# jweyn/DLWP-CS

Measured on AMD Instinct MI355X. Metric: cubed-sphere samples/sec (fwd+bwd), higher is better.
Workload: dtype bf16; 1 GPU; unet2 C48: x (32,6,48,48,14) per GPU, 14 out channels, base 32, MSE + Adam, fwd+bwd+update, bf16 activations + bf16 MFMA, fp32 master weights / gradients / Adam; global_batch=32, parallelism=dp1, hip_graphs=True

## Files before the change

### dlwp-cs_amd/DLWP/_native.py

```python
import ctypes
import os
import threading

import numpy as np
import torch

_HERE = os.path.dirname(os.path.abspath(__file__))
_TAG = os.environ.get('DLWPCS_LIB_TAG', '')
LIB_PATH = os.path.join(os.path.dirname(_HERE), 'lib', 'libdlwpcs%s.so' % ('_' + _TAG if _TAG else ''))

F32 = 0
BF16 = 1
I16 = 2
MAP_RENORMALIZE = 1
MSE_TARGET_F32 = 0x100
MSE_OVERWRITE = 0x200
ADAM_ZERO_GRAD = 1
HEAD_DEFER_STAGE2 = 2
LOSS_MSE, LOSS_MAE, LOSS_ACC = 0, 1, 2
REG_NONE, REG_MSE, REG_MAE, REG_GLOBAL = 0, 1, 2, 3
NORM_ALL, NORM_VALID = 0, 1
E_UNSUPPORTED = -2
ACT_NONE = 0
ACT_LEAKY_CLIP = 1
CONV_ACCUMULATE_WGRAD = 1
CONV_PREPACKED = 2
CONV_REUSE_DZ = 4
CONV_DEFER_REDUCE = 8
CONV_DEFER_RING0 = 16
CONV_OUT_PADDED = 32
CONV_DGRAD_GATHER = 64
CONSTRAINT_MAX_NORM, CONSTRAINT_NON_NEG, CONSTRAINT_UNIT_NORM, CONSTRAINT_MIN_MAX_NORM = 1, 2, 3, 4
PACK_FWD, PACK_BWD, PACK_BIAS = 0, 1, 2
WGRAD_BATCH_MAX = 24

c_void_p, c_int, c_float, c_size_t = ctypes.c_void_p, ctypes.c_int, ctypes.c_float, ctypes.c_size_t
c_i32p = ctypes.POINTER(ctypes.c_int32)


class ConvDesc(ctypes.Structure):
    _fields_ = [('B', ctypes.c_int32), ('N', ctypes.c_int32), ('C0', ctypes.c_int32), ('C1', ctypes.c_int32),
                ('Cout', ctypes.c_int32), ('ksize', ctypes.c_int32), ('halo', ctypes.c_int32),
                ('up0', ctypes.c_int32), ('flip_north_pole', ctypes.c_int32), ('act', ctypes.c_int32),
                ('alpha', ctypes.c_float), ('vmax', ctypes.c_float), ('dtype', ctypes.c_int32),
                ('flags', ctypes.c_int32), ('c0_valid', ctypes.c_int32)]


class PackItem(ctypes.Structure):
    _fields_ = [(n, ctypes.c_void_p) for n in ('w_eq', 'w_pol', 'w_np', 'b_eq', 'b_pol', 'b_np', 'wpk_fwd', 'wpk_bwd',
                                                'bias_pk')] + \
               [(n, ctypes.c_int32) for n in ('ksize', 'Cin', 'Cout', 'flip_north_pole', 'dtype', 'reserved')]


class ReduceItem(ctypes.Structure):
    _fields_ = [(n, ctypes.c_void_p) for n in ('partial', 'bpartial', 'dw_eq', 'dw_pol', 'dw_np', 'db_eq', 'db_pol',
                                                'db_np')] + \
               [(n, ctypes.c_int32) for n in ('ksize', 'Cin', 'Cout', 'CinP', 'CoutP', 'n_eq', 'n_4', 'n_5',
                                              'flip_north_pole', 'accumulate', 'vec', 'nblocks')] + \
               [('reserved', ctypes.c_int32 * 4)]


class WgradItem(ctypes.Structure):
    _fields_ = [('d', ConvDesc)] + [(n, ctypes.c_void_p) for n in ('src0', 'src1', 'dz', 'y', 'table_dev', 'dw_eq', 'dw_pol',
                                                                    'dw_np', 'db_eq', 'db_pol', 'db_np')]


class LossTail(ctypes.Structure):
    _fields_ = [('partial', ctypes.c_void_p), ('loss_out', ctypes.c_void_p), ('nblocks', ctypes.c_int32), ('inv_n', ctypes.c_float),
                ('weight', ctypes.c_float), ('overwrite', ctypes.c_int32)]


class LossDesc(ctypes.Structure):
    _fields_ = [('kind', ctypes.c_int32), ('loss_weight', ctypes.c_float), ('weight', ctypes.c_void_p),
                ('weight_div', ctypes.c_int32), ('weight_period', ctypes.c_int32), ('clim', ctypes.c_void_p),
                ('clim_div', ctypes.c_int32), ('clim_period', ctypes.c_int32), ('regularize', ctypes.c_int32),
                ('reverse', ctypes.c_int32), ('overwrite', ctypes.c_int32)]


class GConvDesc(ctypes.Structure):
    _fields_ = [(n, ctypes.c_int32) for n in
                ('B', 'H', 'W', 'Cin', 'Cout', 'kh', 'kw', 'sh', 'sw', 'dh', 'dw', 'pad_t', 'pad_l', 'Ho', 'Wo',
                 'flip_north_pole', 'dtype')]


SCORE_MSE, SCORE_RMSE, SCORE_MAE, SCORE_ACC, SCORE_COS, SCORE_MEAN = 0, 1, 2, 3, 4, 5
SCORE_MAX_DIMS = 8


class ScoreDesc(ctypes.Structure):
    _fields_ = [(n, ctypes.c_int32) for n in ('method', 'n_lead', 't_len', 't_cap', 't_slope', 'n_keep', 'n_red', 'kc')] + \
               [('keep_ext', ctypes.c_int64 * SCORE_MAX_DIMS), ('red_ext', ctypes.c_int64 * SCORE_MAX_DIMS),
                ('lead_stride', ctypes.c_int64 * 4), ('t_stride', ctypes.c_int64 * 4), ('kc_stride', ctypes.c_int64 * 4),
                ('keep_stride', (ctypes.c_int64 * SCORE_MAX_DIMS) * 4), ('red_stride', (ctypes.c_int64 * SCORE_MAX_DIMS) * 4)]


class OverlapDesc(ctypes.Structure):
    _fields_ = [('N', ctypes.c_int32), ('n_lat', ctypes.c_int32), ('n_lon', ctypes.c_int32), ('reserved', ctypes.c_int32),
                ('frames', ((ctypes.c_double * 3) * 3) * 6), ('dust', ctypes.c_double)]


class CubeBilinearDesc(ctypes.Structure):
    _fields_ = [('N', ctypes.c_int32), ('reserved', ctypes.c_int32), ('n_points', ctypes.c_int64),
                ('frames', ((ctypes.c_double * 3) * 3) * 6), ('edge', ((ctypes.c_int32 * 3) * 4) * 6)]


class SparseMapDesc(ctypes.Structure):
    _fields_ = [('n_a', ctypes.c_int64), ('n_b', ctypes.c_int64), ('nnz', ctypes.c_int64), ('x_dtype', ctypes.c_int32),
                ('n_outer', ctypes.c_int32), ('outer_ext', ctypes.c_int64 * 3), ('x_outer_stride', ctypes.c_int64 * 3),
                ('y_outer_stride', ctypes.c_int64 * 3), ('x_space_stride', ctypes.c_int64), ('y_space_stride', ctypes.c_int64),
                ('inner_ext', ctypes.c_int64), ('x_inner_stride', ctypes.c_int64), ('y_inner_stride', ctypes.c_int64)]


GROUP_SLAB_ROWS = 512


class RowsDesc(ctypes.Structure):
    _fields_ = [('n_inner', ctypes.c_int32), ('reserved', ctypes.c_int32), ('src_row_stride', ctypes.c_int64),
                ('out_row_stride', ctypes.c_int64), ('inner_ext', ctypes.c_int64 * SCORE_MAX_DIMS),
                ('src_stride', ctypes.c_int64 * SCORE_MAX_DIMS), ('out_stride', ctypes.c_int64 * SCORE_MAX_DIMS)]


class ZonalSpectrumDesc(ctypes.Structure):
    _fields_ = [(n, ctypes.c_int32) for n in ('L', 'n_wave', 'n_dims', 'remove_mean')] + \
               [('ext', ctypes.c_int64 * SCORE_MAX_DIMS), ('kept', ctypes.c_int32 * SCORE_MAX_DIMS),
                ('stride', (ctypes.c_int64 * SCORE_MAX_DIMS) * 3)]


class ShtSpectrumDesc(ctypes.Structure):
    _fields_ = [(n, ctypes.c_int32) for n in ('nlat', 'L', 'T', 'n_dims')] + \
               [('lat_stride', ctypes.c_int64 * 2), ('ext', ctypes.c_int64 * SCORE_MAX_DIMS),
                ('stride', (ctypes.c_int64 * SCORE_MAX_DIMS) * 2)]


class ShtSynthesisDesc(ctypes.Structure):
    _fields_ = [(n, ctypes.c_int32) for n in ('nlat', 'L', 'T', 'n_dims')] + \
               [('lat_stride', ctypes.c_int64), ('ext', ctypes.c_int64 * SCORE_MAX_DIMS), ('stride', ctypes.c_int64 * SCORE_MAX_DIMS)]


SHT_MAX_NLAT = 8192
ENSEMBLE_MAX_M = 128


class EnsembleDesc(ctypes.Structure):
    _fields_ = [(n, ctypes.c_int32) for n in ('M', 'n_dims', 'fair', 'ddof', 'variance', 'reserved')] + \
               [('member_stride', ctypes.c_int64), ('ext', ctypes.c_int64 * SCORE_MAX_DIMS),
                ('stride', (ctypes.c_int64 * SCORE_MAX_DIMS) * 2)]


QUANTILE_MAX_PROBS = 16
TIME_FILTER_MAX_TAPS = 4096
REGRESSION_MAX_TERMS = 16
REGRESSION_SLAB_ROWS = 512
TIME_SPECTRUM_MAX_M = 1728
TIME_SPECTRUM_SLAB_SEGMENTS = 8
ROW_GRAM_SLAB_COLS = 512
ROW_GRAM_GROUP_SLABS = 16
TIME_LAG_MAX_LAGS = 1024
TIME_LAG_SLAB_ROWS = 512
LAG_AUTO, LAG_PAIR, LAG_INDEX = 0, 1, 2
RESAMPLE_STAGED_ROWS = 1280
RESAMPLE_MAX_ROWS = 2147483647
RESAMPLE_CHOOSE, RESAMPLE_STAGED, RESAMPLE_DIRECT = -1, 0, 1
CATEGORY_MAX_M = 1024
CATEGORY_MAX_Q = 16


class CategoryDesc(ctypes.Structure):
    _fields_ = [(n, ctypes.c_int32) for n in ('M', 'Q', 'n_dims', 'fair')] + \
               [('member_stride', ctypes.c_int64), ('thr_stride', ctypes.c_int64), ('ext', ctypes.c_int64 * SCORE_MAX_DIMS),
                ('stride', (ctypes.c_int64 * SCORE_MAX_DIMS) * 3), ('ref_prob', ctypes.c_float * CATEGORY_MAX_Q)]


AFFINE_MUL_ADD, AFFINE_SUB_DIV = 0, 1
AFFINE_MAX_CHANNELS = 1024


class ChanDesc(ctypes.Structure):
    _fields_ = [(n, ctypes.c_int64) for n in ('R', 'C', 'S', 'row_stride', 'chan_stride', 'inner_stride', 'dst_row_stride',
                                              'dst_chan_stride', 'dst_inner_stride')]


PROTOTYPES = {
    'dlwpcs_version': (c_int, []),
    'dlwpcs_last_error': (ctypes.c_char_p, []),
    'dlwpcs_halo_table': (c_int, [c_int, c_int, c_void_p]),
    'dlwpcs_halo_inverse_table': (c_int, [c_int, c_int, c_void_p]),
    'dlwpcs_dgrad_gather_plan_ints': (c_size_t, [c_int]),
    'dlwpcs_dgrad_gather_plan': (c_int, [c_int, c_void_p]),
    'dlwpcs_pad_fwd': (c_int, [c_void_p, c_void_p, c_int, c_int, c_int, c_int, c_int, c_void_p, c_void_p]),
    'dlwpcs_pad_bwd': (c_int, [c_void_p, c_void_p, c_int, c_int, c_int, c_int, c_int, c_void_p, c_void_p]),
    'dlwpcs_conv_workspace_bytes': (c_size_t, [ctypes.POINTER(ConvDesc)]),
    'dlwpcs_conv_packed_bytes': (c_size_t, [ctypes.POINTER(ConvDesc), c_int]),
    'dlwpcs_pack_batch': (c_int, [c_void_p, c_int, c_void_p]),
    'dlwpcs_conv_fwd': (c_int, [ctypes.POINTER(ConvDesc)] + [c_void_p] * 8 + [c_void_p, c_void_p, c_void_p, c_size_t,
                                                                                 c_void_p]),
    'dlwpcs_conv_fwd_pool': (c_int, [ctypes.POINTER(ConvDesc)] + [c_void_p] * 8 + [c_void_p, c_void_p, c_void_p, c_void_p, c_size_t,
                                                                                      c_void_p]),
    'dlwpcs_conv_fwd_head': (c_int, [ctypes.POINTER(ConvDesc)] + [c_void_p] * 4 + [ctypes.POINTER(ConvDesc)] + [c_void_p] * 6 +
                             [c_size_t, ctypes.POINTER(c_int), c_void_p]),
    'dlwpcs_conv_bwd_data': (c_int, [ctypes.POINTER(ConvDesc)] + [c_void_p] * 5 + [c_void_p, c_void_p, c_void_p,
                                                                                      c_void_p, c_size_t, c_void_p]),
    'dlwpcs_conv_bwd_data_masked': (c_int, [ctypes.POINTER(ConvDesc)] + [c_void_p] * 4 + [c_void_p] * 4 + [c_float, c_float] +
                                    [c_void_p, c_void_p, c_size_t, c_void_p]),
    'dlwpcs_conv_small_fwd': (c_int, [ctypes.POINTER(ConvDesc)] + [c_void_p] * 8 + [c_void_p, c_void_p, c_void_p, c_size_t,
                                                                                       c_void_p]),
    'dlwpcs_conv_small_bwd_data': (c_int, [ctypes.POINTER(ConvDesc)] + [c_void_p] * 4 + [c_void_p] * 4 + [c_float, c_float] +
                                   [c_void_p, c_void_p, c_size_t, c_void_p]),
    'dlwpcs_conv_bwd_weights': (c_int, [ctypes.POINTER(ConvDesc)] + [c_void_p] * 4 + [c_void_p] * 6 +
                                [c_void_p, c_void_p, c_size_t, c_void_p]),
    'dlwpcs_conv_wgrad_reduce_item': (c_int, [ctypes.POINTER(ConvDesc)] + [c_void_p] * 6 +
                                      [c_void_p, c_size_t, ctypes.POINTER(ReduceItem)]),
    'dlwpcs_wgrad_reduce_batch': (c_int, [c_void_p, c_void_p, c_int, c_void_p]),
    'dlwpcs_wgrad_batch_supported': (c_int, [ctypes.POINTER(ConvDesc)]),
    'dlwpcs_wgrad_batch_sizes': (c_int, [c_void_p, c_int, ctypes.POINTER(c_size_t), ctypes.POINTER(c_size_t)]),
    'dlwpcs_wgrad_batch_plan': (c_int, [c_void_p, c_int, c_void_p, c_size_t]),
    'dlwpcs_wgrad_batch': (c_int, [c_void_p, c_int, c_void_p, c_void_p, c_void_p, c_size_t, c_void_p]),
    'dlwpcs_wgrad_batch_adam': (c_int, [c_void_p, c_int, c_void_p, c_void_p, c_void_p, c_size_t, c_void_p, c_void_p, c_void_p,
                                        c_void_p, c_size_t, c_void_p, c_void_p, c_void_p]),
    'dlwpcs_wgrad_batch_adam_tail': (c_int, [c_void_p, c_int, c_void_p, c_void_p, c_void_p, c_size_t, c_void_p, c_void_p, c_void_p,
                                             c_void_p, c_size_t, c_void_p, c_void_p, c_void_p, c_void_p, c_void_p]),
    'dlwpcs_wgrad_batch_apply': (c_int, [c_void_p, c_int, c_void_p, c_void_p, c_void_p, c_void_p, c_void_p, c_void_p, c_size_t,
                                         c_void_p, c_void_p, c_void_p, c_void_p, c_void_p]),
    'dlwpcs_gconv_fwd': (c_int, [ctypes.POINTER(GConvDesc)] + [c_void_p] * 9),
    'dlwpcs_gconv_bwd_data': (c_int, [ctypes.POINTER(GConvDesc)] + [c_void_p] * 6),
    'dlwpcs_gconv_bwd_weights': (c_int, [ctypes.POINTER(GConvDesc)] + [c_void_p] * 9),
    'dlwpcs_act_fwd': (c_int, [c_void_p, c_void_p, c_size_t, c_int, c_float, c_float, c_int, c_void_p]),
    'dlwpcs_act_bwd': (c_int, [c_void_p, c_void_p, c_void_p, c_size_t, c_int, c_float, c_float, c_int, c_void_p]),
    'dlwpcs_avgpool2_fwd': (c_int, [c_void_p, c_void_p, c_int, c_int, c_int, c_int, c_void_p]),
    'dlwpcs_avgpool2_bwd': (c_int, [c_void_p, c_void_p, c_int, c_int, c_int, c_int, c_void_p]),
    'dlwpcs_avgpool2_bwd_add': (c_int, [c_void_p, c_void_p, c_void_p, c_int, c_int, c_int, c_int, c_void_p]),
    'dlwpcs_avgpool2_bwd_masked': (c_int, [c_void_p, c_void_p, c_void_p, c_void_p, c_int, c_int, c_int, c_float, c_float, c_int,
                                           c_void_p]),
    'dlwpcs_avgpool2_bwd_ring': (c_int, [c_void_p, c_void_p, c_void_p, c_void_p, c_int, c_int, c_int, c_float, c_float, c_int,
                                         c_void_p, c_void_p, c_int, c_int, c_void_p]),
    'dlwpcs_conv_ring_info': (c_int, [ctypes.POINTER(ConvDesc), ctypes.POINTER(c_size_t), ctypes.POINTER(c_int)]),
    'dlwpcs_upsample2_fwd': (c_int, [c_void_p, c_void_p, c_int, c_int, c_int, c_int, c_void_p]),
    'dlwpcs_upsample2_bwd': (c_int, [c_void_p, c_void_p, c_int, c_int, c_int, c_int, c_void_p]),
    'dlwpcs_concat2': (c_int, [c_void_p, c_void_p, c_void_p, c_size_t, c_int, c_int, c_int, c_void_p]),
    'dlwpcs_split2': (c_int, [c_void_p, c_void_p, c_void_p, c_size_t, c_int, c_int, c_int, c_void_p]),
    'dlwpcs_cf_to_cl': (c_int, [c_void_p, c_void_p, c_int, c_int, c_size_t, c_int, c_void_p]),
    'dlwpcs_cl_to_cf': (c_int, [c_void_p, c_void_p, c_int, c_int, c_size_t, c_int, c_void_p]),
    'dlwpcs_add': (c_int, [c_void_p, c_void_p, c_void_p, c_size_t, c_int, c_void_p]),
    'dlwpcs_l1l2_regularize': (c_int, [c_void_p, c_void_p, c_size_t, c_float, c_float, c_float, c_void_p, c_void_p]),
    'dlwpcs_weight_constraint': (c_int, [c_void_p, c_int, c_int, c_int, c_float, c_float, c_float, c_void_p]),
    'dlwpcs_mse_scratch_bytes': (c_size_t, []),
    'dlwpcs_mse_fwd_bwd': (c_int, [c_void_p, c_void_p, c_void_p, c_void_p, c_size_t, c_float, c_int, c_void_p,
                                   c_void_p]),
    'dlwpcs_loss_scratch_bytes': (c_size_t, []),
    'dlwpcs_loss_fwd_bwd': (c_int, [c_void_p, c_void_p, c_void_p, c_void_p, c_void_p, c_size_t, c_int, c_void_p, c_void_p]),
    'dlwpcs_loss_masked_fwd_bwd': (c_int, [c_void_p, c_void_p, c_void_p, c_int, c_void_p, c_void_p, c_void_p, c_size_t, c_int,
                                           c_void_p, c_void_p]),
    'dlwpcs_head_loss_step': (c_int, [c_void_p, c_void_p, c_void_p, c_void_p, c_void_p, c_void_p, c_void_p, c_void_p, c_void_p,
                                      c_void_p, c_void_p, c_int, c_float, c_float, c_void_p]),
    'dlwpcs_score_scratch_bytes': (c_size_t, [c_void_p]),
    'dlwpcs_score': (c_int, [c_void_p, c_void_p, c_void_p, c_void_p, c_void_p, c_void_p, c_int, c_void_p, c_size_t, c_void_p]),
    'dlwpcs_score_indexed': (c_int, [c_void_p, c_void_p, c_void_p, c_void_p, c_void_p, c_void_p, ctypes.c_int64, c_void_p, c_int,
                                     c_void_p, c_size_t, c_void_p]),
    'dlwpcs_score_plan_info': (c_int, [c_void_p, c_void_p, c_void_p, c_void_p, c_void_p, c_int, ctypes.c_int64, c_void_p]),
    'dlwpcs_group_mean_scratch_bytes': (c_size_t, [c_void_p, c_int, ctypes.c_int64, c_int]),
    'dlwpcs_group_mean': (c_int, [c_void_p, c_void_p, c_void_p, c_void_p, c_int, ctypes.c_int64, c_int, c_void_p, c_void_p,
                                  c_void_p, c_size_t, c_void_p]),
    'dlwpcs_rows_gather': (c_int, [c_void_p, c_void_p, c_void_p, ctypes.c_int64, c_void_p, c_void_p]),
    'dlwpcs_group_quantile': (c_int, [c_void_p, c_void_p, c_void_p, c_void_p, c_int, ctypes.c_int64, c_void_p, c_int, c_void_p,
                                      ctypes.c_int64, c_void_p, c_void_p]),
    'dlwpcs_group_quantile_plan_info': (c_int, [c_void_p, c_void_p, c_int, ctypes.c_int64, c_int, c_void_p]),
    'dlwpcs_time_filter': (c_int, [c_void_p, c_void_p, ctypes.c_int64, c_void_p, c_int, ctypes.c_int64, ctypes.c_int64, ctypes.c_int64,
                                   c_int, c_float, c_int, ctypes.c_int64, c_void_p, c_void_p, c_void_p]),
    'dlwpcs_time_filter_plan_info': (c_int, [c_void_p, c_void_p, c_void_p, ctypes.c_int64, c_int, ctypes.c_int64, ctypes.c_int64, c_int,
                                             c_int, ctypes.c_int64, c_void_p]),
    'dlwpcs_time_regression_scratch_bytes': (c_size_t, [c_void_p, ctypes.c_int64, c_int, ctypes.c_int64, c_int]),
    'dlwpcs_time_regression': (c_int, [c_void_p, c_void_p, ctypes.c_int64, c_void_p, c_int, c_int, ctypes.c_int64, ctypes.c_double,
                                       ctypes.c_int64, c_int, c_int, c_void_p, ctypes.c_int64, c_void_p, c_void_p, c_size_t, c_void_p]),
    'dlwpcs_time_regression_plan_info': (c_int, [c_void_p, c_void_p, c_void_p, ctypes.c_int64, c_int, c_int, ctypes.c_int64,
                                                 ctypes.c_int64, c_int, c_int, ctypes.c_int64, c_void_p]),
    'dlwpcs_time_regression_apply': (c_int, [c_void_p, c_void_p, ctypes.c_int64, c_void_p, c_int, c_void_p, ctypes.c_int64, c_void_p,
                                             c_int, c_void_p, c_void_p]),
    'dlwpcs_time_spectrum_scratch_bytes': (c_size_t, [c_void_p, ctypes.c_int64, c_int, ctypes.c_int64, c_int, c_int, c_int]),
    'dlwpcs_time_spectrum': (c_int, [c_void_p, c_void_p, c_void_p, ctypes.c_int64, c_int, ctypes.c_int64, c_void_p, c_void_p,
                                     ctypes.c_double, c_int, c_int, c_int, c_int, c_int, ctypes.c_int64, ctypes.c_int64, c_void_p,
                                     c_void_p, c_void_p, c_size_t, c_void_p]),
    'dlwpcs_time_spectrum_plan_info': (c_int, [c_void_p, c_void_p, c_void_p, ctypes.c_int64, c_int, ctypes.c_int64, c_int, c_int,
                                               c_int, c_void_p]),
    'dlwpcs_row_gram_scratch_bytes': (c_size_t, [c_void_p, ctypes.c_int64, c_void_p, ctypes.c_int64, c_int]),
    'dlwpcs_row_gram': (c_int, [c_void_p, c_void_p, ctypes.c_int64, c_void_p, c_void_p, ctypes.c_int64, c_void_p, c_int, c_void_p,
                                c_int, c_void_p, c_int, c_void_p, ctypes.c_int64, c_void_p, c_void_p, c_void_p, c_size_t, c_void_p]),
    'dlwpcs_row_gram_plan_info': (c_int, [c_void_p, c_void_p, ctypes.c_int64, c_void_p, c_void_p, ctypes.c_int64, c_int, c_void_p]),
    'dlwpcs_time_lag_scratch_bytes': (c_size_t, [c_void_p, c_int, ctypes.c_int64, ctypes.c_int64, c_int, c_int, c_int]),
    'dlwpcs_time_lag': (c_int, [c_void_p, c_void_p, c_void_p, c_int, ctypes.c_int64, ctypes.c_int64, ctypes.c_int64, c_int, c_void_p,
                                c_void_p, c_void_p, c_int, c_int, c_int, c_int, c_void_p, c_void_p, c_void_p, c_size_t, c_void_p]),
    'dlwpcs_time_lag_plan_info': (c_int, [c_void_p, c_void_p, c_void_p, c_int, ctypes.c_int64, ctypes.c_int64, c_int, c_int, c_int,
# ... 220 lines not shown
```

### dlwp-cs_amd/DLWP/custom.py

```python


import numpy as np

from . import ops
from ._native import ACT_LEAKY_CLIP, ACT_NONE
from .keras import constraints, engine, regularizers
from .keras.callbacks import Callback, EarlyStopping
from .keras.engine import Layer
from .keras.losses import LossSpec, mean_absolute_error, mean_squared_error, spec_of



def _normalize_tuple(value, n, name):
    if isinstance(value, int):
        return (value,) * n
    try:
        value_tuple = tuple(value)
    except TypeError:
        raise ValueError('The `' + name + '` argument must be a tuple of ' + str(n) + ' integers. Received: ' +
                         str(value))
    if len(value_tuple) != n:
        raise ValueError('The `' + name + '` argument must be a tuple of ' + str(n) + ' integers. Received: ' +
                         str(value))
    for single_value in value_tuple:
# ... 97 lines not shown
                 independent_north_pole=False,
                 kernel_initializer='glorot_uniform',
                 bias_initializer='zeros',
                 kernel_regularizer=None,
                 bias_regularizer=None,
                 activity_regularizer=None,
                 kernel_constraint=None,
                 bias_constraint=None,
                 **kwargs):
        super(CubeSphereConv2D, self).__init__(**kwargs)
        self.filters = filters
        self.kernel_size = _normalize_tuple(kernel_size, 2, 'kernel_size')
        self.strides = _normalize_tuple(strides, 2, 'strides')
        self.padding = _normalize_padding(padding)
        self.data_format = _normalize_data_format(data_format)
        self.dilation_rate = _normalize_tuple(dilation_rate, 2, 'dilation_rate')
        self.activation = engine.get_activation(activation)
        self.use_bias = use_bias
        self.flip_north_pole = flip_north_pole
        self.independent_north_pole = independent_north_pole
        self.kernel_initializer = engine.get_initializer(kernel_initializer)
        self.bias_initializer = engine.get_initializer(bias_initializer)
        self.kernel_regularizer = regularizers.get(kernel_regularizer)
        self.bias_regularizer = regularizers.get(bias_regularizer)
        self.activity_regularizer = engine._passthrough_get(activity_regularizer)
        self.kernel_constraint = constraints.get(kernel_constraint)
        self.bias_constraint = constraints.get(bias_constraint)
        self.rank = 3

        self.equatorial_kernel = None
        self.equatorial_bias = None
        self.polar_kernel = None
        self.polar_bias = None
        self.north_pole_kernel = None
        self.north_pole_bias = None

    def _weight_attr_names(self):
        return ['equatorial_kernel', 'polar_kernel', 'north_pole_kernel', 'equatorial_bias', 'polar_bias',
                'north_pole_bias']

    def build(self, input_shape):
        if self.data_format == 'channels_first':
            channel_axis = 1
        else:
            channel_axis = -1
        if input_shape[channel_axis] is None:
            raise ValueError('The channel dimension of the inputs should be defined. Found `None`.')
        input_dim = int(input_shape[channel_axis])
        kernel_shape = self.kernel_size + (input_dim, self.filters)

        self.equatorial_kernel = self.add_weight(shape=kernel_shape, initializer=self.kernel_initializer,
                                                 name='equatorial_kernel', regularizer=self.kernel_regularizer,
                                                 constraint=self.kernel_constraint)
        self.polar_kernel = self.add_weight(shape=kernel_shape, initializer=self.kernel_initializer,
                                            name='polar_kernel', regularizer=self.kernel_regularizer,
                                            constraint=self.kernel_constraint)
        if self.independent_north_pole:
            self.north_pole_kernel = self.add_weight(shape=kernel_shape, initializer=self.kernel_initializer,
                                                     name='north_pole_kernel', regularizer=self.kernel_regularizer,
                                                     constraint=self.kernel_constraint)
        if self.use_bias:
            self.equatorial_bias = self.add_weight(shape=(self.filters,), initializer=self.bias_initializer,
                                                   name='equatorial_bias', regularizer=self.bias_regularizer,
                                                   constraint=self.bias_constraint)
            self.polar_bias = self.add_weight(shape=(self.filters,), initializer=self.bias_initializer,
                                              name='polar_bias', regularizer=self.bias_regularizer,
                                              constraint=self.bias_constraint)
            if self.independent_north_pole:
                self.north_pole_bias = self.add_weight(shape=(self.filters,), initializer=self.bias_initializer,
                                                       name='north_pole_bias', regularizer=self.bias_regularizer,
                                                       constraint=self.bias_constraint)
        self.input_dim = input_dim
        self.built = True

    def _is_mfma_config(self):
        k = self.kernel_size
        return (k[0] == k[1] and k[0] in (1, 3) and self.strides == (1, 1) and self.dilation_rate == (1, 1)
                and self.padding == 'valid')

    def can_fuse_halo(self, pad_width):
        return (self._is_mfma_config() and self.kernel_size[0] == 3 and pad_width == 1 and self.activation is None)

    def fused_call(self, src0, src1=None, up0=False, halo=True, act=ACT_NONE, alpha=0.0, vmax=0.0, premask0=None,
                   premask1=None, dy_premasked=False, defer_ring0=False, want_pool=False, out_padded=False, small=False):
        return ops.cs_conv(src0, self.equatorial_kernel, self.polar_kernel, self.north_pole_kernel,
                           self.equatorial_bias, self.polar_bias, self.north_pole_bias, src1=src1,
                           ksize=self.kernel_size[0], halo=halo, up0=up0, flip_north_pole=self.flip_north_pole,
                           act=act, alpha=alpha, vmax=vmax, premask0=premask0, premask1=premask1,
                           dy_premasked=dy_premasked, defer_ring0=defer_ring0, want_pool=want_pool, out_padded=out_padded,
                           small=small)

    def call(self, inputs, channels_last_io=False, **kwargs):
        channels_first = self.data_format == 'channels_first' and not channels_last_io
        x = ops.channels_first_to_last(inputs) if channels_first else inputs
        if self._is_mfma_config():
            outputs = ops.cs_conv(x, self.equatorial_kernel, self.polar_kernel, self.north_pole_kernel,
                                  self.equatorial_bias, self.polar_bias, self.north_pole_bias,
                                  ksize=self.kernel_size[0], halo=False, flip_north_pole=self.flip_north_pole)
        else:
            outputs = ops.cs_gconv(x, self.equatorial_kernel, self.polar_kernel, self.north_pole_kernel,
                                   self.equatorial_bias, self.polar_bias, self.north_pole_bias,
                                   strides=self.strides, padding=self.padding, dilation=self.dilation_rate,
                                   flip_north_pole=self.flip_north_pole)
        if channels_first:
            outputs = ops.channels_last_to_first(outputs)
        if self.activation is not None:
            return self.activation(outputs)
        return outputs

    def compute_output_shape(self, input_shape):
        if self.data_format == 'channels_last':
            space = input_shape[2:4]
        else:
            space = input_shape[-2:]
        new_space = []
        for i in range(len(space)):
            new_space.append(_conv_output_length(space[i], self.kernel_size[i], padding=self.padding,
                                                 stride=self.strides[i], dilation=self.dilation_rate[i]))
        if self.data_format == 'channels_last':
            return (input_shape[0], 6) + tuple(new_space) + (self.filters,)
        return (input_shape[0], self.filters, 6) + tuple(new_space)

    def get_config(self):
        config = {
            'filters': self.filters,
            'kernel_size': self.kernel_size,
            'strides': self.strides,
            'padding': self.padding,
            'data_format': self.data_format,
            'dilation_rate': self.dilation_rate,
            'activation': engine.serialize_activation(self.activation),
            'use_bias': self.use_bias,
            'flip_north_pole': self.flip_north_pole,
            'independent_north_pole': self.independent_north_pole,
            'kernel_initializer': engine.serialize_initializer(self.kernel_initializer),
            'bias_initializer': engine.serialize_initializer(self.bias_initializer),
            'kernel_regularizer': regularizers.serialize(self.kernel_regularizer),
            'bias_regularizer': regularizers.serialize(self.bias_regularizer),
            'activity_regularizer': self.activity_regularizer,
            'kernel_constraint': constraints.serialize(self.kernel_constraint),
            'bias_constraint': constraints.serialize(self.bias_constraint)
        }
        base_config = super(CubeSphereConv2D, self).get_config()
        return dict(list(base_config.items()) + list(config.items()))



def _adam_effective_lr(optimizer, beta_1, beta_2, with_bias_correction):
    it = float(optimizer.iterations)
    lr = float(optimizer.lr) / (1. + float(getattr(optimizer, 'decay', 0.)) * it)
    if with_bias_correction:
        t = it + 1.
        lr = lr * np.sqrt(1. - np.power(beta_2, t)) / (1. - np.power(beta_1, t))
    return lr


class AdamLearningRateTracker(Callback):

    def on_epoch_end(self, epoch, logs=None, beta_1=0.9, beta_2=0.999, ):
        print(' - LR: {:.6f}'.format(_adam_effective_lr(self.model.optimizer, beta_1, beta_2, True)))


class SGDLearningRateTracker(Callback):

    def on_epoch_end(self, epoch, logs=None):
        print(' - LR: {:.6f}'.format(_adam_effective_lr(self.model.optimizer, 0., 0., False)))


class BatchHistory(Callback):

    def on_train_begin(self, logs=None):
        self.history, self.epoch = [], 0

# ... 239 lines not shown
```

### dlwp-cs_amd/DLWP/keras/models.py

```python
import gc
import json
import os
import sys
import time

import numpy as np
import torch

from .. import ops, parallel
from ..options import option
from .. import _native as _nat
from .._native import ACT_LEAKY_CLIP, ACT_NONE
from . import backend, callbacks as cbks, losses as klosses, optimizers, staging
from .engine import KTensor, Layer
from .layers import AveragePooling3D, Concatenate, InputLayer, ReLU, UpSampling3D


def _new_graph():
    if os.environ.get('DLWPCS_KEEP_GRAPH', '0') == '1':
        return torch.cuda.CUDAGraph(keep_graph=True)
    return torch.cuda.CUDAGraph()


def _as_list(x):
    if isinstance(x, (list, tuple)):
        return list(x)
    return [x]


class Model(object):
    def __init__(self, inputs=None, outputs=None, name=None):
        if inputs is None or outputs is None:
            raise ValueError('Model needs `inputs` and `outputs`')
        self._single_input = not isinstance(inputs, (list, tuple))
        self.inputs = _as_list(inputs)
        self.outputs = _as_list(outputs)
        self._single_output = len(self.outputs) == 1
        for t in self.inputs + self.outputs:
            if not isinstance(t, KTensor):
                raise ValueError('Model inputs/outputs must be symbolic tensors created by Input() and layer calls')
        self.name = name or 'model'
        self.stop_training = False
        self.optimizer = None
        self.loss = None
        self._dev_losses = None
        self.loss_weights = None
        self.metrics = []
        self.history = None
        self.use_graphs = option('graphs')
        self.compute_dtype = backend.compute_dtype()
        self.prepack_weights = True
        self.wgrad_side_stream = False
        self.defer_wgrad_reduce = True
        self.batch_wgrad = option('wgrad_batch')
        self.check_finite = option('check_finite')
        self.fuse_adam = option('fuse_adam')
        self.fold_ring = option('fold_ring')
        self.fuse_pool = option('fuse_pool')
        self.fold_loss_tail = option('fold_loss_tail')
        self.fuse_pack = option('fuse_pack')
        self._packed_ok = False
        self.exchange_buckets = int(os.environ.get('DLWPCS_EXCHANGE_BUCKETS', '1'))
        self._stager = None
        self.fuse_head_loss = option('fuse_head')
        self.fold_head = option('fold_head')
        self.small_conv = option('small_conv')
        self.static_batch_buffers = False
        self._ones = {}
        self._compiled = False
        self._flat_params = self._flat_grads = None
        self._grads_clean = False
        self._graphs = {}
        self._infer_graphs = {}
        self._rollout_series = {}
        self.rollout_keep_bytes = 4 << 30
        self._seen_batch = {}
        self._toposort()
        self._build_plan()

    def _toposort(self):
        order, seen = [], set()

        def visit(t):
            if t.uid in seen:
                return
            seen.add(t.uid)
            for i in t.node_inputs:
                visit(i)
            order.append(t)
        for o in self.outputs:
            visit(o)
        input_uids = {t.uid for t in self.inputs}
        for t in order:
            if isinstance(t.layer, InputLayer) and t.uid not in input_uids:
                raise ValueError('Graph disconnected: cannot obtain value for tensor %r' % (t,))
        self._nodes = order
        layers, seen_l = [], set()
        for t in self.inputs + order:
            if t.layer is not None and id(t.layer) not in seen_l:
                seen_l.add(id(t.layer))
                layers.append(t.layer)
        self.layers = layers

    def _build_plan(self):
        consumers = {}
        for t in self._nodes:
            for i in t.node_inputs:
                consumers.setdefault(i.uid, []).append(t)
        out_uids = {o.uid for o in self.outputs}

        def sole_consumer(t):
            c = consumers.get(t.uid, [])
            return c[0] if (len(c) == 1 and t.uid not in out_uids) else None

        from ..custom import CubeSphereConv2D, CubeSpherePadding2D
        def cf_layer(t):
            lay = t.layer
            if isinstance(lay, InputLayer):
                return len(t.shape) == 5
            if isinstance(lay, CubeSphereConv2D) and lay.activation is not None \
                    and getattr(lay.activation, '_dlwp_name', None) != 'relu':
                return False
            if isinstance(lay, (CubeSpherePadding2D, CubeSphereConv2D, AveragePooling3D, UpSampling3D)):
                return lay.data_format == 'channels_first'
            if isinstance(lay, Concatenate):
                return lay._axis(len(t.shape)) == 1
            return isinstance(lay, ReLU)
        self._cf_model = (option('cf_model') and all(cf_layer(t) for t in self._nodes)
                          and any(isinstance(t.layer, (CubeSphereConv2D, CubeSpherePadding2D)) for t in self._nodes))
        fmt = 'channels_first' if self._cf_model else 'channels_last'
        virtual = set()
        fused = {}
        for t in self._nodes:
            lay = t.layer
            if not isinstance(lay, CubeSphereConv2D) or len(t.node_inputs) != 1:
                continue
            padt = t.node_inputs[0]
            if not isinstance(padt.layer, CubeSpherePadding2D) or sole_consumer(padt) is not t:
                continue
            if padt.layer.data_format != fmt or lay.data_format != fmt or not lay.can_fuse_halo(padt.layer.padding[1][0]):
                continue
            if padt.layer.padding[1] != padt.layer.padding[2] or padt.layer.padding[1][0] != padt.layer.padding[1][1]:
                continue
            x = padt.node_inputs[0]
            src0, src1, up0 = x, None, False
            chain = [padt]
            if isinstance(x.layer, Concatenate) and len(x.node_inputs) == 2 and sole_consumer(x) is padt \
                    and x.layer._axis(len(x.shape)) == (1 if self._cf_model else len(x.shape) - 1):
                src0, src1 = x.node_inputs
# ... 28 lines not shown
                              isinstance(t.layer, Concatenate)))
        self._plan = steps
        self.n_fused = len(fused)
        self._padded_io_ok = False
        if len(self.inputs) == 1:
            u = self.inputs[0].uid
            rd = [st for st in steps
                  if (st[0] == 'fused_conv' and u in (st[3], st[4])) or (st[0] == 'pool_skip' and st[3] == u)
                  or (st[0] == 'layer' and u in st[3])]
            self._padded_io_ok = (len(rd) == 1 and rd[0][0] == 'fused_conv' and rd[0][3] == u and rd[0][4] is None
                                  and not rd[0][5] and u not in out_uids and not self._cf_model)
        self._plan_premask(steps, out_uids)
        self._head_fold = {}
        for i, st in enumerate(steps):
            if st[0] != 'fused_conv' or st[1] in out_uids:
                continue
            rd = [j for j, s2 in enumerate(steps)
                  if (s2[0] == 'fused_conv' and st[1] in (s2[3], s2[4])) or (s2[0] == 'pool_skip' and s2[3] == st[1])
                  or (s2[0] == 'layer' and st[1] in s2[3])]
            if len(rd) != 1 or steps[rd[0]][0] != 'layer':
                continue
            hl = steps[rd[0]][2]
            if (isinstance(hl, CubeSphereConv2D) and len(steps[rd[0]][3]) == 1 and tuple(hl.kernel_size) == (1, 1)
                    and hl.activation is None and not hl.independent_north_pole and not st[2].independent_north_pole
                    and st[2].filters == 32 and self._runs_channels_last(hl) and not self._cf_model):
                self._head_fold[i] = rd[0]
        uids = [o.uid for o in self.outputs]
        self._sole_outputs = {u for u in uids if not consumers.get(u) and uids.count(u) == 1}

    def _plan_premask(self, steps, out_uids):
        from ..custom import CubeSphereConv2D
        produced = {}
        for st in steps:
            if st[0] == 'fused_conv' and st[6] == ACT_LEAKY_CLIP:
                produced[st[1]] = (float(st[7]), float(st[8]))
        capable = {u: (u not in out_uids) for u in produced}
        in_uids_model = {t.uid for t in self.inputs}
        for st in steps:
            if st[0] == 'fused_conv' and st[1] in capable and st[3] in in_uids_model and (st[4] is None or st[4] in in_uids_model):
                capable[st[1]] = False
        aliased = set()
        src_mask = {}
        for i, st in enumerate(steps):
            if st[0] == 'fused_conv':
                s0, s1 = st[3], st[4]
                src_mask[i] = (s0 in produced and s0 not in aliased, s1 is not None and s1 in produced and s1 not in aliased)
                if s0 == s1 and s0 in produced:
                    capable[s0] = False
            elif st[0] == 'pool_skip':
                u = st[3]
                src_mask[i] = u in produced and u not in aliased
                aliased.add(u)
            else:
                _, out_uid, lay, in_uids, _ = st
                head = (isinstance(lay, CubeSphereConv2D) and len(in_uids) == 1 and lay._is_mfma_config()
                        and self._runs_channels_last(lay) and lay.activation is None)
                src_mask[i] = bool(head and in_uids[0] in produced and in_uids[0] not in aliased)
                for u in in_uids:
                    if u in produced and u not in aliased and not head:
                        capable[u] = False
        self._premask = {u: produced[u] for u in produced if capable[u]}
        self._src_mask = src_mask
        readers = {}
        for i, st in enumerate(steps):
            ins = [st[3], st[4]] if st[0] == 'fused_conv' else ([st[3]] if st[0] == 'pool_skip' else list(st[3]))
            for u in ins:
                if u is not None:
                    readers.setdefault(u, []).append(i)
        self._pool_producers = set()
        for i, st in enumerate(steps):
            if st[0] == 'fused_conv':
                r = readers.get(st[1], [])
                if r and steps[r[0]][0] == 'pool_skip' and steps[r[0]][3] == st[1]:
                    self._pool_producers.add(i)
        self._defer_ring = set()
        for i, st in enumerate(steps):
            if st[0] != 'pool_skip' or not (src_mask.get(i) and st[3] in self._premask):
                continue
            r = readers.get(st[1], [])
            if len(r) == 1 and st[1] not in out_uids and steps[r[0]][0] == 'fused_conv' and steps[r[0]][3] == st[1] \
                    and steps[r[0]][4] != st[1] and not steps[r[0]][5]:
                self._defer_ring.add(r[0])

    def _runs_channels_last(self, lay):
        return lay.data_format == 'channels_last' or self._cf_model

    def _plan_exchange(self):
        if self._exchange_cut is not None:
            return self._exchange_cut or None
        self._exchange_cut = False
        if self._flat_grads is None:
            return None
        base = self._flat_grads.data_ptr()
        spans = []
        for st in self._plan:
            ws = [w for w in getattr(st[2], '_weights', []) if w.requires_grad and w.grad is not None]
            if ws:
                lo = min((w.grad.data_ptr() - base) // 4 for w in ws)
                hi = max((w.grad.data_ptr() - base) // 4 + w.numel() for w in ws)
                spans.append((lo, hi))
            else:
                spans.append(None)
        total = sum(hi - lo for sp in spans if sp for lo, hi in [sp])
        if total == 0:
            return None
        acc, cut = 0, None
        for i in range(len(spans) - 1, 0, -1):
            if spans[i]:
                acc += spans[i][1] - spans[i][0]
                if acc >= 0.4 * total:
                    cut = i
                    break
        if cut is None or not any(spans[:cut]):
            return None
        lo_a = min(sp[0] for sp in spans[cut:] if sp)
        if any(sp and sp[1] > lo_a for sp in spans[:cut]):
            return None
        self._exchange_cut = (cut, int(lo_a) // 64 * 64)
        return self._exchange_cut

    def _premask_on(self):
        return (self.compute_dtype == 'bfloat16' and torch.is_grad_enabled()
                and option('premask'))

    def _pack_state(self, device):
        from ..custom import CubeSphereConv2D
        from .. import _native as nat
        tag = nat.BF16 if self.compute_dtype == 'bfloat16' else nat.F32
        key = (str(device), tag, self._flat_params.data_ptr() if self._flat_params is not None else 0)
        st = getattr(self, '_pack_cache', None)
        if st is not None and st['key'] == key:
            return st
        entries, table, by_grad = [], {}, {}
        for lay in self.layers:
            if not isinstance(lay, CubeSphereConv2D) or not lay.built or not lay._is_mfma_config():
                continue
            we = lay.equatorial_kernel
            if we.device != device or id(we) in table:
                continue
            bufs = ops.conv_packed_buffers(lay.kernel_size[0], we.shape[2], we.shape[3], tag, device,
                                           bias=lay.equatorial_bias is not None)
            entries.append((we, lay.polar_kernel, lay.north_pole_kernel, lay.equatorial_bias, lay.polar_bias,
                            lay.north_pole_bias, bufs, lay.kernel_size[0], lay.flip_north_pole, tag))
            table[id(we)] = (tag, bufs[0], bufs[1], bufs[2])
            if we.grad is not None:
                by_grad[we.grad.data_ptr()] = entries[-1]
        st = {'key': key, 'items': ops.make_pack_items(entries, device) if entries else None, 'n': len(entries),
              'table': table, 'keep': entries, 'by_grad': by_grad}
        self._pack_cache = st
        return st

    def _forward(self, inputs, repack=True, fuse_targets=None):
        want = backend.torch_dtype(self.compute_dtype)
        inputs = [v if v.dtype == want else v.to(want) for v in inputs]
        if inputs and inputs[0].is_cuda and self.prepack_weights:
            st = self._pack_state(inputs[0].device)
            if st['n'] and (repack or not st.get('packed')):
                ops.pack_batch(st['items'], st['n'])
                st['packed'] = True
                st['packed_version'] = self._flat_params._version if self._flat_params is not None else None
                self._packed_ok = True
            ops.PREPACKED = st['table']
            try:
                return self._run_plan(inputs, fuse_targets)
            finally:
                ops.PREPACKED = {}
        return self._run_plan(inputs, fuse_targets)

    def _run_plan(self, inputs, fuse_targets=None):
        from ..custom import CubeSphereConv2D, CubeSpherePadding2D
        cf = self._cf_model
        if cf:
            inputs = [ops.channels_first_to_last(v) for v in inputs]
        values = {t.uid: v for t, v in zip(self.inputs, inputs)}
        self._fused_outputs = set()
        pm = self._premask if self._premask_on() else {}
        cut = getattr(self, '_record_cut', None)
        self._cut_tensors = []
        ops._POOLED.clear()
        folded = set()
        for i, st in enumerate(self._plan):
            if i in folded:
                continue
            if cut is not None and i == cut:
                need, seen = set(), set()
                for s2 in self._plan[cut:]:
                    ins = [s2[3], s2[4]] if s2[0] == 'fused_conv' else ([s2[3]] if s2[0] == 'pool_skip' else list(s2[3]))
                    need.update(u for u in ins if u is not None)
                for u, v in values.items():
                    if u in need and isinstance(v, torch.Tensor) and v.requires_grad and id(v) not in seen:
                        seen.add(id(v))
                        self._cut_tensors.append(v)
            if st[0] == 'fused_conv':
                _, out_uid, lay, s0, s1, up0, act, alpha, vmax = st
                j = self._head_fold.get(i) if self.fold_head else None
                if j is not None and fuse_targets is None and not torch.is_grad_enabled():
                    hl, h_uid = self._plan[j][2], self._plan[j][1]
                    padded = bool(getattr(self, '_padded_io', False) and h_uid in self._sole_outputs and hl.filters % 8 != 0)
                    if (lay._is_mfma_config() and hl._is_mfma_config() and hl.built and lay.built and ops.cs_conv_head_applicable(
                            values[s0], None if s1 is None else values[s1], lay.equatorial_kernel, hl.equatorial_kernel, padded)):
                        values[h_uid] = ops.cs_conv_head(values[s0], lay.equatorial_kernel, lay.equatorial_bias,
                                                         hl.equatorial_kernel, hl.equatorial_bias,
                                                         src1=None if s1 is None else values[s1], up0=up0,
                                                         flip_north_pole=lay.flip_north_pole, act=act, alpha=alpha, vmax=vmax,
                                                         out_padded=padded)
                        folded.add(j)
                        continue
                m0, m1 = self._src_mask[i]
                values[out_uid] = lay.fused_call(values[s0], None if s1 is None else values[s1], up0=up0, halo=True,
                                                 act=act, alpha=alpha, vmax=vmax,
                                                 premask0=pm.get(s0) if m0 else None, premask1=pm.get(s1) if m1 else None,
                                                 dy_premasked=out_uid in pm,
                                                 defer_ring0=bool(pm) and self.fold_ring and i in self._defer_ring,
                                                 want_pool=self.fuse_pool and i in self._pool_producers,
                                                 small=self.small_conv)
            elif st[0] == 'pool_skip':
                _, out_uid, lay, in_uid = st
                values[out_uid], values[in_uid] = ops.avgpool2_skip(values[in_uid],
                                                                     pm.get(in_uid) if self._src_mask[i] else None)
                if cut is not None and i < cut:
                    values[in_uid] = ops.detour(values[in_uid])
            else:
                _, out_uid, lay, in_uids, takes_list = st
                args = [values[u] for u in in_uids]
                head_pm = pm.get(in_uids[0]) if (self._src_mask[i] and in_uids) else None
                if (fuse_targets is not None and out_uid in fuse_targets and out_uid in self._sole_outputs
                        and isinstance(lay, CubeSphereConv2D) and len(args) == 1 and lay._is_mfma_config()
                        and self._runs_channels_last(lay) and lay.activation is None and lay.north_pole_kernel is None
                        and ops.head_mse_applicable(args[0], lay.equatorial_kernel, lay.kernel_size[0], ACT_NONE,
                                                    fuse_targets[out_uid][0], fuse_targets[out_uid][2])):
                    tgt, wgt, dl = fuse_targets[out_uid]
                    values[out_uid] = ops.head_mse(args[0], tgt, lay.equatorial_kernel, lay.polar_kernel, lay.equatorial_bias,
                                                   lay.polar_bias, wgt, lay.flip_north_pole, premask=head_pm, loss=dl)
                    self._fused_outputs.add(out_uid)
                    continue
                if head_pm is not None:
                    values[out_uid] = lay.fused_call(args[0], halo=False, premask0=head_pm)
                    continue
                if (getattr(self, '_padded_io', False) and out_uid in self._sole_outputs and isinstance(lay, CubeSphereConv2D)
                        and len(args) == 1 and lay._is_mfma_config() and self._runs_channels_last(lay)
                        and lay.activation is None and lay.kernel_size[0] == 1 and args[0].dtype == torch.bfloat16
                        and args[0].shape[-1] == 32 and 8 <= lay.filters <= 32 and lay.filters % 2 == 0
                        and (args[0].shape[2] * args[0].shape[3]) % 16 == 0):
                    values[out_uid] = lay.fused_call(args[0], halo=False, out_padded=True)
                    continue
                if cf:
                    if isinstance(lay, CubeSphereConv2D):
                        values[out_uid] = lay.call(args[0], channels_last_io=True)
                    elif isinstance(lay, CubeSpherePadding2D):
                        values[out_uid] = ops.cs_pad(args[0], lay.padding[1][0])
                    elif isinstance(lay, AveragePooling3D):
                        values[out_uid] = ops.avgpool2(args[0])
                    elif isinstance(lay, UpSampling3D):
                        values[out_uid] = ops.upsample2(args[0])
                    elif isinstance(lay, Concatenate):
                        values[out_uid] = ops.concat_channels(list(args))
                    else:
                        values[out_uid] = lay.call(args[0])
                    continue
                values[out_uid] = lay.call(args if (takes_list or len(args) > 1) else args[0])
        if cf and not getattr(self, '_loss_in_cl', False):
            return [values[o.uid] if o.uid in self._fused_outputs else ops.channels_last_to_first(values[o.uid])
                    for o in self.outputs]
        return [values[o.uid] for o in self.outputs]

    def __call__(self, inputs):
        self._grads_clean = False
        outs = self._forward(_as_list(inputs))
        return outs[0] if self._single_output else outs

    def _weight_layers(self):
        return [l for l in self.layers if l._weights]

    @property
    def weights(self):
        return [w for l in self._weight_layers() for w in l._weights]

    @property
    def trainable_weights(self):
        return [w for w in self.weights if w.requires_grad]

    def count_params(self):
        return int(sum(w.numel() for w in self.weights))

    def get_weights(self):
        return [a for l in self._weight_layers() for a in l.get_weights()]

    def set_weights(self, weights):
        weights = list(weights)
        n = sum(len(l._weights) for l in self._weight_layers())
        if len(weights) != n:
            raise ValueError('You called `set_weights(weights)` on model "%s" with a weight list of length %d, but the '
                             'model was expecting %d weights.' % (self.name, len(weights), n))
        k = 0
        for l in self._weight_layers():
            l.set_weights(weights[k:k + len(l._weights)])
            k += len(l._weights)

# ... 167 lines not shown

    def _loss_and_backward_gen(self, inputs, targets, train=True, fuse_update=None, split=False, skip_pack=False, exchange=False):
        self._update_done = False
        self._did_split = False
        if train and self.batch_wgrad and inputs and inputs[0].is_cuda and not _nat.lds_oob_reads_zero(inputs[0].device):
            self.batch_wgrad = False
        if len(targets) != len(self.outputs):
            raise ValueError('Error when checking model target: expected %d target arrays, got %d'
                             % (len(self.outputs), len(targets)))
        if self._cf_model:
            targets = [ops.channels_first_to_last(t) if t.dim() == 5 else t for t in targets]
        fuse = None
        if train and self.fuse_head_loss:
            fuse = {o.uid: (t, w, dl) for o, t, w, dl in zip(self.outputs, targets, self.loss_weights, self._losses_per_output())}
            ops.DIRECT_PARAM_GRADS = True
        cutplan = self._plan_exchange() if (train and split) else None
        self._record_cut = cutplan[0] if cutplan else None
        ops.finish_loss_tail()
        dp_fused = bool(train and exchange and fuse_update is not None and not cutplan)
        ops.DEFER_LOSS_TAIL = bool(train and fuse_update is not None and self.fuse_adam and self.batch_wgrad and self.fold_loss_tail
                                   and self.optimizer is not None and (self._world == 1 or dp_fused) and not cutplan)
        self._pack_done = False
        self._loss_in_cl = self._cf_model
        try:
            outs = self._forward(inputs, repack=not skip_pack, fuse_targets=fuse)
        finally:
            self._loss_in_cl = False
            self._record_cut = None
            ops.DEFER_LOSS_TAIL = False
            if not train:
                ops.finish_loss_tail()
            if fuse is not None:
                ops.DIRECT_PARAM_GRADS = False
        fused = getattr(self, '_fused_outputs', set()) if fuse is not None else set()
        stats = [o if out.uid in fused else (ops.mse_mae(o, t, w) if dl is None else ops.loss_stats(o, t, dl, w))
                 for out, o, t, w, dl in zip(self.outputs, outs, targets, self.loss_weights, self._losses_per_output())]
        if train:
            dev = stats[0].device
            ones = [ops.unit_seed(dev) for _ in stats]
            ops.DIRECT_PARAM_GRADS = True
            ops.WGRAD_SIDE_STREAM = self.wgrad_side_stream
            ops.DEFER_WGRAD_REDUCE = self.defer_wgrad_reduce
            ops.WGRAD_BATCH = self.batch_wgrad and not self.wgrad_side_stream
            ops.drop_deferred_reduce()
            ops.drop_wgrad_batch()
            ops.drop_pending_rings()
            try:
                cut = [t for t in self._cut_tensors] if cutplan else []
                self._cut_tensors = []
                if cut:
                    gcut = torch.autograd.grad(stats, cut, ones, allow_unused=True)
                    ops.flush_wgrad_batch(None)
                    ops.flush_deferred_reduce(dev)
                    self._did_split = True
                    yield None
                    pairs = [(t, g) for t, g in zip(cut, gcut) if g is not None]
                    if pairs:
                        torch.autograd.backward([t for t, _ in pairs], [g for _, g in pairs])
                else:
                    torch.autograd.backward(stats, ones)
                if dp_fused:
                    ops.flush_wgrad_batch(None)
                    ops.flush_deferred_reduce(dev)
                    self._wb_done = ops.flushed_wgrad_entries()
                    parallel.allreduce_gradients(self._flat_grads)
                    self._update_done = True
                    self._apply_update(fuse_update, dev)
                else:
                    adam = lookup = None
                    if (fuse_update is not None and self.fuse_adam and not ops._deferred and self.optimizer is not None
                            and self._world == 1 and not cut):
                        adam, lookup = self._adam_args(dev, fuse_update)
                    self._update_done = ops.flush_wgrad_batch(adam, lookup)
                    self._pack_done = bool(self._update_done and ops.PACK_FUSED)
                    ops.flush_deferred_reduce(dev)
                    self._wb_done = ops.flushed_wgrad_entries()
            finally:
                ops.DIRECT_PARAM_GRADS = False
                ops.WGRAD_SIDE_STREAM = False
                ops.DEFER_WGRAD_REDUCE = False
                ops.WGRAD_BATCH = False
                ops.drop_deferred_reduce()
                ops.drop_wgrad_batch()
                if ops._pending_ring:
                    ops.drop_pending_rings()
                    if sys.exc_info()[0] is None:
                        raise RuntimeError('a deferred ring fix-up was not consumed by its pooling node (plan error)')
                ops.finish_loss_tail()
                ops.join_side_stream(stats[0].device)
        if len(stats) == 1:
            return stats[0].detach().view(1, 2)
        return torch.stack([s.detach() for s in stats])

    def _exchange_slices(self):
        lo = self._plan_exchange()[1]
        return self._flat_grads[lo:], self._flat_grads[:lo]

    def _weight_rules(self):
        rules = getattr(self, '_wrules', None)
        if rules is None:
            rules = []
            for lay in self._weight_layers():
                for w, (reg, con) in zip(lay._weights, getattr(lay, '_weight_rules', [])):
                    if w.requires_grad and (reg is not None or con is not None):
                        rules.append((w, reg, con))
            self._wrules = rules
        return rules

    def _grad_view(self, w):
        off = (w.data_ptr() - self._flat_params.data_ptr()) // 4
        return self._flat_grads[off:off + w.numel()]

    def _penalty_row(self, add_grads, grad_scale=1.0):
        from .._native import check, lib, ptr, stream_ptr
        pen = torch.zeros((1, 2), dtype=torch.float32, device=self._flat_params.device)
        for w, reg, _ in self._weight_rules():
            if reg is None or (reg.l1 == 0.0 and reg.l2 == 0.0):
                continue
            g = self._grad_view(w) if add_grads else None
            check(lib().dlwpcs_l1l2_regularize(ptr(w), ptr(g), w.numel(), reg.l1, reg.l2, 1.0 / float(grad_scale), ptr(pen), stream_ptr()),
                  'dlwpcs_l1l2_regularize')
        return pen

    def _apply_constraints(self):
        for w, _, con in self._weight_rules():
            if con is not None:
                con.apply(w)

    def _update_with_rules(self, scale):
        pen = self._penalty_row(True, scale) if self._weight_rules() else None
        self.optimizer.apply(self._flat_params, self._flat_grads, grad_scale=scale)
        if pen is not None:
            self._apply_constraints()
        self._packed_ok = False
        return pen

    def _apply_gradients(self):
        scale = parallel.allreduce_gradients(self._flat_grads)
        return self._update_with_rules(scale)

    def _train_step_eager(self, inputs, targets):
        self._flat_grads.zero_()
        self._grads_clean = False
        if self._split_wanted():
            gen = self._loss_and_backward_gen(inputs, targets, True, None, split=True)
            ha = None
            try:
                next(gen)
                ha = parallel.allreduce_start(self._exchange_slices()[0])
                next(gen)
                raise RuntimeError('the split step yielded twice')
            except StopIteration as e:
                stats = e.value
            finally:
                gen.close()
            if self._did_split:
                hb = parallel.allreduce_start(self._exchange_slices()[1])
                parallel.allreduce_wait(ha)
                parallel.allreduce_wait(hb)
                pen = self._update_with_rules(1.0 / self._world)
                return stats if pen is None else torch.cat([stats, pen], dim=0)
            pen = self._apply_gradients()
            return stats if pen is None else torch.cat([stats, pen], dim=0)
        stats = self._loss_and_backward(inputs, targets, True)
        pen = self._apply_gradients()
        return stats if pen is None else torch.cat([stats, pen], dim=0)

    def train_on_device_batch(self, inputs, targets):
        if not self._compiled:
            raise RuntimeError('You must compile your model before training/testing. Use `model.compile(...)`.')
# ... 1040 lines not shown
```

### dlwp-cs_amd/DLWP/ops.py

```python
import ctypes
import os

import numpy as np
import torch

from . import _native as nat
from .layout import element_layout, member_split, merge_dims
from .options import option
from ._native import ConvDesc, GConvDesc, check, lib, ptr, require_device, stream_ptr

DIRECT_PARAM_GRADS = False

PREPACKED = {}

WGRAD_SIDE_STREAM = False
_side_streams = {}


def side_stream(device):
    key = str(device)
    st = _side_streams.get(key)
    if st is None:
        st = torch.cuda.Stream(device=device)
        _side_streams[key] = st
# ... 171 lines not shown
def prepare_wgrad_plan(entries, n_elems):
    entries = list(entries)
    if not entries or len(entries) > nat.WGRAD_BATCH_MAX or not _wb_covers(entries, n_elems):
        return
    dev = entries[0][3].device
    arr, key = _wb_items(entries)
    _wb_plan(arr, len(entries), (str(dev), key), dev)


def _pack_array(packs):
    pk_arr = (nat.PackItem * len(packs))()
    for it, (we, wp, wn, be, bp, bn, bufs, ksize, flip, tag) in zip(pk_arr, packs):
        it.w_eq, it.w_pol, it.w_np = ptr(we), ptr(wp), ptr(wn)
        it.b_eq, it.b_pol, it.b_np = ptr(be), ptr(bp), ptr(bn)
        it.wpk_fwd, it.bias_pk, it.wpk_bwd = ptr(bufs[0]), ptr(bufs[1]), ptr(bufs[2])
        it.ksize, it.Cin, it.Cout = int(ksize), int(we.shape[2]), int(we.shape[3])
        it.flip_north_pole, it.dtype, it.reserved = int(flip), int(tag), 0
    return pk_arr


def _wb_plan(arr, n, key, dev):
    hit = _wb_plans.get(key)
    if hit is None:
        if torch.cuda.is_current_stream_capturing():
            raise nat.NativeError('the weight-gradient plan would have to be uploaded during graph capture; run one eager '
                                  'step first')
        pb, wb = ctypes.c_size_t(), ctypes.c_size_t()
        check(lib().dlwpcs_wgrad_batch_sizes(arr, n, ctypes.byref(pb), ctypes.byref(wb)), 'dlwpcs_wgrad_batch_sizes')
        host = (ctypes.c_char * pb.value)()
        check(lib().dlwpcs_wgrad_batch_plan(arr, n, host, pb.value), 'dlwpcs_wgrad_batch_plan')
        plan_dev = torch.frombuffer(bytearray(bytes(host)), dtype=torch.uint8).to(dev)
        hit = (host, plan_dev, wb.value)
        _wb_plans[key] = hit
    return hit


def _wb_items(entries):
    arr = (nat.WgradItem * len(entries))()
    key = []
    for it, ent in zip(arr, entries):
        d, src0, src1, dz, table, grads = ent[:6]
        y = ent[6] if len(ent) > 6 else None
        it.d = d
        it.src0, it.src1, it.dz, it.y, it.table_dev = ptr(src0), ptr(src1), ptr(dz), ptr(y), ptr(table)
        it.dw_eq, it.dw_pol, it.dw_np, it.db_eq, it.db_pol, it.db_np = [ptr(g) for g in grads]
        key.append((d.B, d.N, d.C0, d.C1, d.Cout, d.ksize, d.halo, d.up0, d.flip_north_pole, d.dtype, d.c0_valid,
                    tuple(g is not None for g in grads), None if y is None else (d.act, d.alpha, d.vmax)))
    return arr, tuple(key)


def wgrad_batch(entries, adam=None, packs=None):
    if not entries:
        return
    dev = entries[0][3].device
    for lo in range(0, len(entries), nat.WGRAD_BATCH_MAX):
        chunk = entries[lo:lo + nat.WGRAD_BATCH_MAX]
        arr, key = _wb_items(chunk)
        host, plan_dev, ws_bytes = _wb_plan(arr, len(chunk), (str(dev), key), dev)
        ws = _workspace(ws_bytes, dev, 'wgrad_batch')
        if adam is not None:
            p, g, m, v, state, hyper = adam
            tail = None
            if len(_pending_tail) == 1:
                tail, keep = _pending_tail.pop()
            if tail is not None or packs is not None:
                pk_arr = _pack_array(packs[lo:lo + len(chunk)]) if packs is not None else None
                check(lib().dlwpcs_wgrad_batch_adam_tail(arr, len(chunk), host, ptr(plan_dev), ptr(ws), ws.numel(), ptr(p), ptr(g),
                                                         ptr(m), ptr(v), g.numel(), ptr(state), ptr(hyper),
                                                         ctypes.byref(tail) if tail is not None else None, pk_arr, stream_ptr()),
                      'dlwpcs_wgrad_batch_adam_tail')
                continue
            check(lib().dlwpcs_wgrad_batch_adam(arr, len(chunk), host, ptr(plan_dev), ptr(ws), ws.numel(), ptr(p), ptr(g), ptr(m),
                                                ptr(v), g.numel(), ptr(state), ptr(hyper), stream_ptr()),
                  'dlwpcs_wgrad_batch_adam')
            continue
        check(lib().dlwpcs_wgrad_batch(arr, len(chunk), host, ptr(plan_dev), ptr(ws), ws.numel(), stream_ptr()),
              'dlwpcs_wgrad_batch')


_pending_ring = {}
_POOLED = {}


def drop_pending_rings():
    _pending_ring.clear()


def _c(t):
    return t if t.is_contiguous() else t.contiguous()



class _CSPad(torch.autograd.Function):
    @staticmethod
    def forward(ctx, x, p):
        require_device(x, 'cs_pad')
        x = _c(x)
        B, F6, N, N2, C = x.shape
        if F6 != 6 or N != N2:
            raise ValueError('cs_pad: expected (B, 6, N, N, C), got %s' % (tuple(x.shape),))
        table, inv = nat.halo_tables(N, p, x.device)
        y = torch.empty((B, 6, N + 2 * p, N + 2 * p, C), dtype=x.dtype, device=x.device)
        check(lib().dlwpcs_pad_fwd(ptr(x), ptr(y), B, N, C, p, nat.dtype_tag(x), ptr(table), stream_ptr()),
              'dlwpcs_pad_fwd')
        ctx.p, ctx.shape = p, (B, N, C)
        ctx.inv = inv
        return y

    @staticmethod
    def backward(ctx, dy):
        B, N, C = ctx.shape
        dy = _c(dy)
        dx = torch.empty((B, 6, N, N, C), dtype=dy.dtype, device=dy.device)
        check(lib().dlwpcs_pad_bwd(ptr(dy), ptr(dx), B, N, C, ctx.p, nat.dtype_tag(dy), ptr(ctx.inv), stream_ptr()),
              'dlwpcs_pad_bwd')
        return dx, None


def cs_pad(x, p):
    return _CSPad.apply(x, int(p))



def _make_desc(B, N, C0, C1, Cout, ksize, halo, up0, flip, act, alpha, vmax, dtype=nat.F32, c0_valid=0):
    return ConvDesc(B=B, N=N, C0=C0, C1=C1, Cout=Cout, ksize=ksize, halo=int(halo), up0=int(up0),
                    flip_north_pole=int(flip), act=int(act), alpha=float(alpha), vmax=float(vmax), dtype=int(dtype),
                    flags=0, c0_valid=int(c0_valid))


class _PadChannels(torch.autograd.Function):

    @staticmethod
    def forward(ctx, x, cp):
        require_device(x, 'pad_channels')
        x = _c(x)
        C = x.shape[-1]
        rows = x.numel() // C if C else 0
        y = torch.empty(tuple(x.shape[:-1]) + (cp,), dtype=x.dtype, device=x.device)
        check(lib().dlwpcs_pad_channels(ptr(x), ptr(y), rows, C, cp, nat.dtype_tag(x), stream_ptr()), 'dlwpcs_pad_channels')
        ctx.c = C
        return y

    @staticmethod
    def backward(ctx, dy):
        dy = _c(dy)
        cp = dy.shape[-1]
        rows = dy.numel() // cp
        dx = torch.empty(tuple(dy.shape[:-1]) + (ctx.c,), dtype=dy.dtype, device=dy.device)
        check(lib().dlwpcs_slice_channels(ptr(dy), ptr(dx), rows, cp, ctx.c, nat.dtype_tag(dy), stream_ptr()),
              'dlwpcs_slice_channels')
        return dx, None


def pad_channels(x, cp):
    if x.shape[-1] == cp:
        return x
    if x.shape[-1] > cp:
        raise ValueError('pad_channels: tensor has %d channels, asked for %d' % (x.shape[-1], cp))
    return _PadChannels.apply(x, int(cp))


def channel_vector(dtype):
    return 8 if dtype == torch.bfloat16 else 4


def padded_channels(c, dtype, even_too=None):
    v = channel_vector(dtype)
    if c % v == 0:
        return c
    if c % 2 == 1 or even_too:
        return (c + v - 1) // v * v
    return c


def _f32_param(t, what):
    if t is not None and t.dtype != torch.float32:
        raise TypeError('%s: parameters must be float32 master copies, got %s' % (what, t.dtype))


def _weight_gradients(d, src0, src1, dy, y, params, table, ws, nbytes, direct, defer, need, has_np, has_bias, has_bnp,
                      batch_mask_ok=False):
    dev = dy.device
    w_eq, w_pol, w_np = params[0], params[1], params[2]
    dw_eq = dw_pol = dw_np = db_eq = db_pol = db_np = None
    if (direct and WGRAD_BATCH and d.B > 0 and not WGRAD_SIDE_STREAM and wgrad_batch_supported(d)
            and (d.act == nat.ACT_NONE or (batch_mask_ok and d.ksize == 3 and y is not None))):
        pe, pp, pn, be, bp, bn = params
        d2 = ConvDesc.from_buffer_copy(d)
        _wb_pending.append((d2, src0, src1, dy, table,
                            (pe.grad, pp.grad, None if pn is None else pn.grad, None if be is None else be.grad,
                             None if bp is None else bp.grad, None if bn is None else bn.grad),
                            None if d.act == nat.ACT_NONE else y))
        return dw_eq, dw_pol, dw_np, db_eq, db_pol, db_np
    if direct:
        pe, pp, pn, be, bp, bn = params
        d2 = ConvDesc.from_buffer_copy(d)
        d2.flags = d.flags | nat.CONV_ACCUMULATE_WGRAD | (nat.CONV_DEFER_REDUCE if defer else 0)
        grads = (ptr(pe.grad), ptr(pp.grad), ptr(None if pn is None else pn.grad),
                 ptr(None if be is None else be.grad), ptr(None if bp is None else bp.grad),
                 ptr(None if bn is None else bn.grad))

        def launch(wsx):
            check(lib().dlwpcs_conv_bwd_weights(ctypes.byref(d2), ptr(src0), ptr(src1), ptr(dy), ptr(y), *grads,
                                                ptr(table), ptr(wsx), wsx.numel(), stream_ptr()),
                  'dlwpcs_conv_bwd_weights')
            if defer:
                item = nat.ReduceItem()
                check(lib().dlwpcs_conv_wgrad_reduce_item(ctypes.byref(d2), *grads, ptr(wsx), wsx.numel(),
                                                          ctypes.byref(item)), 'dlwpcs_conv_wgrad_reduce_item')
                _deferred.append((item, wsx))
        if WGRAD_SIDE_STREAM:
            side = side_stream(dev)
            side.wait_stream(torch.cuda.current_stream(dev))
            ws2 = _workspace(nbytes, dev, 'side')
            with torch.cuda.stream(side):
                launch(ws2)
            for t in (src0, src1, dy, y):
                if t is not None:
                    t.record_stream(side)
        else:
            launch(ws)
    elif any(need):
        dw_eq, dw_pol = torch.empty_like(w_eq), torch.empty_like(w_pol)
        dw_np = torch.empty_like(w_np) if has_np else None
        if has_bias:
            db_eq = torch.empty(d.Cout, dtype=torch.float32, device=dev)
            db_pol = torch.empty(d.Cout, dtype=torch.float32, device=dev)
            db_np = torch.empty(d.Cout, dtype=torch.float32, device=dev) if has_bnp else None
        check(lib().dlwpcs_conv_bwd_weights(ctypes.byref(d), ptr(src0), ptr(src1), ptr(dy), ptr(y), ptr(dw_eq),
                                            ptr(dw_pol), ptr(dw_np), ptr(db_eq), ptr(db_pol), ptr(db_np),
                                            ptr(table), ptr(ws), ws.numel(), stream_ptr()),
              'dlwpcs_conv_bwd_weights')
    return dw_eq, dw_pol, dw_np, db_eq, db_pol, db_np


class _CSConv(torch.autograd.Function):

    @staticmethod
    def forward(ctx, src0, src1, w_eq, w_pol, w_np, b_eq, b_pol, b_np, ksize, halo, up0, flip, act, alpha, vmax,
                c0_valid=0, premask0=None, premask1=None, dy_premasked=False, defer_ring0=False, want_pool=False,
                out_padded=False, small=False):
        require_device(src0, 'cs_conv')
        src0 = _c(src0)
        B = src0.shape[0]
        if src0.dim() != 5 or src0.shape[1] != 6 or src0.shape[2] != src0.shape[3]:
            raise ValueError('cs_conv: expected (B, 6, N, N, C), got %s' % (tuple(src0.shape),))
        N = src0.shape[2] * (2 if up0 else 1)
        C0 = src0.shape[4]
        C1 = 0
        if src1 is not None:
            require_device(src1, 'cs_conv')
            src1 = _c(src1)
            if tuple(src1.shape[:4]) != (B, 6, N, N):
                raise ValueError('cs_conv: src1 shape %s does not match (B,6,%d,%d,*)' % (tuple(src1.shape), N, N))
            C1 = src1.shape[4]
            if src1.dtype != src0.dtype:
                raise TypeError('cs_conv: src0 is %s but src1 is %s' % (src0.dtype, src1.dtype))
        for prm in (w_eq, w_pol, w_np, b_eq, b_pol, b_np):
            _f32_param(prm, 'cs_conv')
        kh, kw, cin, Cout = w_eq.shape
        if kh != ksize or kw != ksize or cin != (c0_valid or C0) + C1:
            raise ValueError('cs_conv: kernel shape %s does not match ksize=%d, C_in=%d' % (tuple(w_eq.shape), ksize,
                                                                                          (c0_valid or C0) + C1))
        w_eq, w_pol = _c(w_eq), _c(w_pol)
        w_np = _c(w_np) if w_np is not None else None
        d = _make_desc(B, N, C0, C1, Cout, ksize, halo, up0, flip, act, alpha, vmax, nat.dtype_tag(src0), c0_valid)
        No = N if halo else N - ksize + 1
        if out_padded:
            if torch.is_grad_enabled() and any(t is not None and t.requires_grad for t in (src0, src1, w_eq)):
                raise RuntimeError('cs_conv: out_padded is an inference-only layout')
            d.flags |= nat.CONV_OUT_PADDED
        y = torch.empty((B, 6, No, No, (Cout + 7) // 8 * 8 if out_padded else Cout), dtype=src0.dtype, device=src0.device)
        table = inv = None
        if halo:
            table, inv = nat.halo_tables(N, (ksize - 1) // 2, src0.device)
        nbytes = lib().dlwpcs_conv_workspace_bytes(ctypes.byref(d))
        ws = _workspace(nbytes, src0.device)
        packed = PREPACKED.get(id(w_eq))
        if packed is not None and packed[0] != d.dtype:
            packed = None
        yp = None
        if want_pool and halo and No % 2 == 0:
            yp = torch.empty((B, 6, No // 2, No // 2, Cout), dtype=src0.dtype, device=src0.device)
        wargs = ((ptr(packed[1]), 0, 0, ptr(packed[2]) if b_eq is not None else 0, 0, 0) if packed is not None else
                 (ptr(w_eq), ptr(w_pol), ptr(w_np), ptr(b_eq), ptr(b_pol), ptr(b_np)))
        if packed is not None:
            d.flags |= nat.CONV_PREPACKED
        small = bool(small) and _small_conv_ok(d)
        if yp is not None:
            check(lib().dlwpcs_conv_fwd_pool(ctypes.byref(d), ptr(src0), ptr(src1), *wargs, ptr(y), ptr(yp), ptr(table), ptr(ws),
                                             ws.numel(), stream_ptr()), 'dlwpcs_conv_fwd_pool')
            _POOLED[y.data_ptr()] = yp
        else:
            rc = nat.E_UNSUPPORTED
            if small:
                rc = lib().dlwpcs_conv_small_fwd(ctypes.byref(d), ptr(src0), ptr(src1), *wargs, ptr(y), ptr(table), ptr(ws),
                                                 ws.numel(), stream_ptr())
            if rc == nat.E_UNSUPPORTED:
                rc = lib().dlwpcs_conv_fwd(ctypes.byref(d), ptr(src0), ptr(src1), *wargs, ptr(y), ptr(table), ptr(ws),
                                           ws.numel(), stream_ptr())
            check(rc, 'dlwpcs_conv_fwd')
        ctx.small = small
        if premask0 is not None and premask1 is not None and tuple(premask0) != tuple(premask1):
            raise ValueError('cs_conv: both sources must share the activation parameters of their masks')
        ctx.premask = (premask0, premask1)
        ctx.dy_premasked = bool(dy_premasked) and act != nat.ACT_NONE
        ctx.defer_ring0 = bool(defer_ring0)
        ctx.packed = packed
        ctx.desc = d
        ctx.tables = (table, inv)
        ctx.has = (src1 is not None, w_np is not None, b_eq is not None, b_np is not None)
        ctx.params = (w_eq, w_pol, w_np, b_eq, b_pol, b_np)
        ctx.save_for_backward(src0, src1, w_eq, w_pol, w_np, y if act != nat.ACT_NONE else None)
        return y

    @staticmethod
    def backward(ctx, dy):
        src0, src1, w_eq, w_pol, w_np, y = ctx.saved_tensors
        d = ctx.desc
        table, inv = ctx.tables
        has_src1, has_np, has_bias, has_bnp = ctx.has
        dy = _c(dy)
        dev = dy.device
        nbytes = lib().dlwpcs_conv_workspace_bytes(ctypes.byref(d))
        need = ctx.needs_input_grad
        dsrc0 = torch.empty_like(src0) if need[0] else None
        dsrc1 = torch.empty_like(src1) if (has_src1 and need[1]) else None
        want_w = any(need[2:8])
        direct = DIRECT_PARAM_GRADS and (need[2] or need[3]) and all(
            p is None or (p.is_leaf and p.grad is not None and p.grad.is_contiguous()) for p in ctx.params)
        pm0, pm1 = ctx.premask
        if dsrc0 is None:
            pm0 = None
        if dsrc1 is None:
            pm1 = None
        masked_io = ctx.dy_premasked or pm0 is not None or pm1 is not None
        if masked_io:
            if ctx.dy_premasked or d.act == nat.ACT_NONE:
                dz = dy
            else:
                dz = torch.empty_like(dy)
                check(lib().dlwpcs_act_bwd(ptr(dy), ptr(y), ptr(dz), dy.numel(), nat.ACT_LEAKY_CLIP, d.alpha, d.vmax,
                                           nat.dtype_tag(dy), stream_ptr()), 'dlwpcs_act_bwd')
            dn = ConvDesc.from_buffer_copy(d)
            dn.act = nat.ACT_NONE
            dn.flags = (d.flags & nat.CONV_PREPACKED) | _gather_flag(d, dev)
            batching = (direct and WGRAD_BATCH and d.B > 0 and not WGRAD_SIDE_STREAM and wgrad_batch_supported(dn))
            defer = direct and DEFER_WGRAD_REDUCE and not WGRAD_SIDE_STREAM and d.B > 0 and not batching
            ws = _workspace(nbytes, dev, 'defer%d' % len(_deferred)) if defer else _workspace(nbytes, dev)
            ring = None
            if ctx.defer_ring0 and dsrc0 is not None and pm0 is None and halo_ring_info(dn) is not None:
                ring = halo_ring_info(dn)
                dn.flags |= nat.CONV_DEFER_RING0
                if not defer:
                    ws = _workspace(nbytes, dev, 'ring%d' % len(_pending_ring))
            if dsrc0 is not None or dsrc1 is not None:
                wq = ctx.packed[3] if ctx.packed is not None else w_eq
                pm = pm0 if pm0 is not None else pm1
                ma, mv = (float(pm[0]), float(pm[1])) if pm is not None else (0.0, 0.0)
                bargs = (ctypes.byref(dn), ptr(dz), ptr(wq), ptr(w_pol), ptr(w_np), ptr(dsrc0), ptr(dsrc1),
                         ptr(src0 if pm0 is not None else None), ptr(src1 if pm1 is not None else None), ma, mv, ptr(inv), ptr(ws),
                         ws.numel(), stream_ptr())
                rc = nat.E_UNSUPPORTED
                if ctx.small and dsrc0 is not None and dsrc1 is None:
                    rc = lib().dlwpcs_conv_small_bwd_data(*bargs)
                if rc == nat.E_UNSUPPORTED:
                    rc = lib().dlwpcs_conv_bwd_data_masked(*bargs)
                check(rc, 'dlwpcs_conv_bwd_data_masked')
                if ring is not None:
                    _pending_ring[dsrc0.data_ptr()] = (ws, ring[0], ring[1], nat.halo_tables(d.N, 1, dev)[1])
                    dn.flags &= ~nat.CONV_DEFER_RING0
            dw_eq, dw_pol, dw_np, db_eq, db_pol, db_np = _weight_gradients(
                dn, src0, src1, dz, None, ctx.params, table, ws, nbytes, direct, defer, need[2:8], has_np, has_bias, has_bnp)
            return (dsrc0, dsrc1, dw_eq, dw_pol, dw_np, db_eq, db_pol, db_np) + (None,) * 15
        no_dgrad = dsrc0 is None and dsrc1 is None
        mask_on_load = d.ksize == 3 and (no_dgrad or d.dtype == nat.F32)
        batching = (direct and WGRAD_BATCH and d.B > 0 and not WGRAD_SIDE_STREAM and wgrad_batch_supported(d)
                    and (d.act == nat.ACT_NONE or mask_on_load))
        defer = direct and DEFER_WGRAD_REDUCE and not WGRAD_SIDE_STREAM and d.B > 0 and not batching
        ws = _workspace(nbytes, dev, 'defer%d' % len(_deferred)) if defer else _workspace(nbytes, dev)
        reuse_dz = ((dsrc0 is not None or dsrc1 is not None) and want_w and d.act != nat.ACT_NONE
                    and not WGRAD_SIDE_STREAM and not batching)
        if reuse_dz:
            d.flags |= nat.CONV_REUSE_DZ

        def run_bwd_data():
            if dsrc0 is not None or dsrc1 is not None:
                wq = ctx.packed[3] if ctx.packed is not None else w_eq
                d.flags |= _gather_flag(d, dev)
                check(lib().dlwpcs_conv_bwd_data(ctypes.byref(d), ptr(dy), ptr(y), ptr(wq), ptr(w_pol), ptr(w_np),
                                                 ptr(dsrc0), ptr(dsrc1), ptr(inv), ptr(ws), ws.numel(), stream_ptr()),
                      'dlwpcs_conv_bwd_data')
                d.flags &= ~nat.CONV_DGRAD_GATHER
        if not reuse_dz:
            run_bwd_data()
        dw_eq, dw_pol, dw_np, db_eq, db_pol, db_np = _weight_gradients(
            d, src0, src1, dy, y, ctx.params, table, ws, nbytes, direct, defer, need[2:8], has_np, has_bias, has_bnp,
            batch_mask_ok=mask_on_load)
        if reuse_dz:
            run_bwd_data()
        return (dsrc0, dsrc1, dw_eq, dw_pol, dw_np, db_eq, db_pol, db_np) + (None,) * 15


def _small_conv_ok(d):
    return (d.dtype == nat.BF16 and d.ksize == 3 and d.halo and d.C1 == 0 and not d.up0 and d.c0_valid == 0
            and d.N * d.N <= 320 and d.C0 % 32 == 0 and d.Cout % 32 == 0 and d.B > 0)


_ring_info_cache = {}



def _gather_flag(d, dev):
    if option('dgrad_gather') and d.halo and d.ksize == 3 and d.dtype == nat.BF16 and nat.dgrad_gather_ready(d.N, 1, dev):
        return nat.CONV_DGRAD_GATHER
    return 0


def halo_ring_info(d):
    key = (d.B, d.N, d.C0, d.C1, d.Cout, d.ksize, d.halo, d.up0, d.dtype, d.c0_valid, d.flags & nat.CONV_DGRAD_GATHER)
    if key not in _ring_info_cache:
        off, ch = ctypes.c_size_t(), ctypes.c_int()
        ok = lib().dlwpcs_conv_ring_info(ctypes.byref(d), ctypes.byref(off), ctypes.byref(ch))
        _ring_info_cache[key] = (off.value, ch.value) if ok else None
    return _ring_info_cache[key]


def conv_packed_buffers(ksize, cin, cout, dtype_tag, device, bias=True):
    d = _make_desc(1, max(ksize, 2), cin, 0, cout, ksize, False, False, True, nat.ACT_NONE, 0.0, 0.0, dtype_tag)
    out = []
    for which in (nat.PACK_FWD, nat.PACK_BIAS, nat.PACK_BWD):
        n = lib().dlwpcs_conv_packed_bytes(ctypes.byref(d), which)
        if n == 0:
            check(-1, 'dlwpcs_conv_packed_bytes')
        out.append(torch.empty(n, dtype=torch.uint8, device=device))
    if not bias:
        out[1] = None
    return tuple(out)


def make_pack_items(entries, device):
    arr = (nat.PackItem * len(entries))()
    for it, (we, wp, wn, be, bp, bn, bufs, ksize, flip, tag) in zip(arr, entries):
        it.w_eq, it.w_pol, it.w_np = ptr(we), ptr(wp), ptr(wn)
        it.b_eq, it.b_pol, it.b_np = ptr(be), ptr(bp), ptr(bn)
        it.wpk_fwd, it.bias_pk, it.wpk_bwd = ptr(bufs[0]), ptr(bufs[1]), ptr(bufs[2])
        it.ksize, it.Cin, it.Cout = int(ksize), int(we.shape[2]), int(we.shape[3])
        it.flip_north_pole, it.dtype, it.reserved = int(flip), int(tag), 0
    raw = bytes(arr)
    host = torch.frombuffer(bytearray(raw), dtype=torch.uint8) if raw else torch.empty(0, dtype=torch.uint8)
    return host.to(device)


def pack_batch(items_dev, n_items):
    check(lib().dlwpcs_pack_batch(ptr(items_dev), int(n_items), stream_ptr()), 'dlwpcs_pack_batch')


def cs_conv(src0, w_eq, w_pol, w_np=None, b_eq=None, b_pol=None, b_np=None, src1=None, ksize=3, halo=True, up0=False,
            flip_north_pole=True, act=nat.ACT_NONE, alpha=0.0, vmax=0.0, premask0=None, premask1=None, dy_premasked=False,
            defer_ring0=False, want_pool=False, out_padded=False, small=False):
    if (w_np is None) != (b_np is None) and b_eq is not None:
        raise ValueError('cs_conv: north-pole kernel and bias must be given together')
    c0_valid = 0
    cin_w = w_eq.shape[2]
    if src1 is None and not up0:
        c_phys = src0.shape[-1]
        if c_phys == cin_w:
            cp = padded_channels(c_phys, src0.dtype)
            if cp != c_phys:
                src0 = pad_channels(src0, cp)
                c0_valid = cin_w
        elif cin_w < c_phys <= (cin_w + channel_vector(src0.dtype) - 1) // channel_vector(src0.dtype) * channel_vector(src0.dtype):
            c0_valid = cin_w
    return _CSConv.apply(src0, src1, w_eq, w_pol, w_np, b_eq, b_pol, b_np, int(ksize), bool(halo), bool(up0),
                         bool(flip_north_pole), int(act), float(alpha), float(vmax), int(c0_valid), premask0, premask1,
                         bool(dy_premasked), bool(defer_ring0), bool(want_pool), bool(out_padded), bool(small))


def cs_conv_head_applicable(src0, src1, w_eq, head_w_eq, out_padded):
    if torch.is_grad_enabled() or not src0.is_cuda or src0.dtype != torch.bfloat16:
        return False
    pk, hk = PREPACKED.get(id(w_eq)), PREPACKED.get(id(head_w_eq))
    if pk is None or hk is None or pk[0] != nat.BF16 or hk[0] != nat.BF16:
        return False
    cout2 = head_w_eq.shape[3]
    rows = (cout2 + 7) // 8 * 8 if out_padded else cout2
    c0, c1 = src0.shape[-1], (src1.shape[-1] if src1 is not None else 0)
    if c0 % 8 or c1 % 8 or c0 + c1 != w_eq.shape[2]:
        return False
    return (tuple(w_eq.shape[:2]) == (3, 3) and w_eq.shape[3] == 32 and tuple(head_w_eq.shape[:3]) == (1, 1, 32) and rows == 32
            and cout2 % 2 == 0 and cout2 >= 8)


def cs_conv_head(src0, w_eq, b_eq, head_w_eq, head_b_eq, src1=None, up0=False, flip_north_pole=True, act=nat.ACT_NONE,
                 alpha=0.0, vmax=0.0, out_padded=False):
    require_device(src0, 'cs_conv_head')
    src0 = _c(src0)
    B = src0.shape[0]
    N = src0.shape[2] * (2 if up0 else 1)
    C0, C1 = src0.shape[4], 0
    if src1 is not None:
        src1 = _c(src1)
        C1 = src1.shape[4]
    Cout, cout2 = w_eq.shape[3], head_w_eq.shape[3]
    pk, hk = PREPACKED[id(w_eq)], PREPACKED[id(head_w_eq)]
    d = _make_desc(B, N, C0, C1, Cout, 3, True, up0, flip_north_pole, act, alpha, vmax, nat.BF16, 0)
    d.flags |= nat.CONV_PREPACKED
    dh = _make_desc(B, N, Cout, 0, cout2, 1, False, False, flip_north_pole, nat.ACT_NONE, 0.0, 0.0, nat.BF16, 0)
    dh.flags |= nat.CONV_PREPACKED | (nat.CONV_OUT_PADDED if out_padded else 0)
    rows = (cout2 + 7) // 8 * 8 if out_padded else cout2
    y = torch.empty((B, 6, N, N, Cout), dtype=src0.dtype, device=src0.device)
    yh = torch.empty((B, 6, N, N, rows), dtype=src0.dtype, device=src0.device)
    table = nat.halo_tables(N, 1, src0.device)[0]
    nbytes = max(lib().dlwpcs_conv_workspace_bytes(ctypes.byref(d)), lib().dlwpcs_conv_workspace_bytes(ctypes.byref(dh)))
    ws = _workspace(nbytes, src0.device)
    fused = ctypes.c_int(0)
    check(lib().dlwpcs_conv_fwd_head(ctypes.byref(d), ptr(src0), ptr(src1), ptr(pk[1]), ptr(pk[2]) if b_eq is not None else 0,
                                     ctypes.byref(dh), ptr(hk[1]), ptr(hk[2]) if head_b_eq is not None else 0, ptr(y), ptr(yh),
                                     ptr(table), ptr(ws), ws.numel(), ctypes.byref(fused), stream_ptr()), 'dlwpcs_conv_fwd_head')
    global HEAD_FOLDED
    HEAD_FOLDED = bool(fused.value)
    return yh


HEAD_FOLDED = False



def _same_pads(n, k, s, dil):
    out = -(-n // s)
    total = max((out - 1) * s + (k - 1) * dil + 1 - n, 0)
    return total // 2, out


def _valid_len(n, k, s, dil):
    return (n - (k - 1) * dil - 1) // s + 1


class _GConv(torch.autograd.Function):
    @staticmethod
    def forward(ctx, x, w_eq, w_pol, w_np, b_eq, b_pol, b_np, strides, padding, dilation, flip):
        require_device(x, 'cs_gconv')
        for prm in (w_eq, w_pol, w_np, b_eq, b_pol, b_np):
            _f32_param(prm, 'cs_gconv')
        x, w_eq, w_pol = _c(x), _c(w_eq), _c(w_pol)
        w_np = _c(w_np) if w_np is not None else None
        B, F6, H, W, Cin = x.shape
        kh, kw, cin, Cout = w_eq.shape
        if F6 != 6 or cin != Cin:
            raise ValueError('cs_gconv: bad shapes x=%s kernel=%s' % (tuple(x.shape), tuple(w_eq.shape)))
        sh, sw = strides
        dh, dw = dilation
        if padding == 'same':
            pad_t, Ho = _same_pads(H, kh, sh, dh)
            pad_l, Wo = _same_pads(W, kw, sw, dw)
        elif padding == 'valid':
            pad_t = pad_l = 0
            Ho = _valid_len(H, kh, sh, dh)
            Wo = _valid_len(W, kw, sw, dw)
# ... 2637 lines not shown
```

### dlwp-cs_amd/DLWP/options.py

```python
import os

DEFAULTS = {
    'graphs': True, 'premask': True, 'wgrad_batch': True, 'fuse_adam': True, 'fuse_pack': True, 'fuse_head': True,
    'fold_loss_tail': True, 'fuse_pool': True, 'fold_ring': True, 'cf_model': True, 'padded_io': True, 'host_staging': True, 'resident_data': True,
    'dgrad_gather': True, 'fold_head': True, 'small_conv': True, 'check_finite': False,
}


_parsed = {}


def _parse(env):
    hit = _parsed.get(env)
    if hit is None:
        hit = {}
        for item in env.split(','):
            item = item.strip()
            if not item:
                continue
            k, _, v = item.partition('=')
            k = k.strip()
            if k not in DEFAULTS:
                raise KeyError('DLWPCS_OPTIONS: unknown engine option %r (known: %s)' % (k, ', '.join(sorted(DEFAULTS))))
            hit[k] = v.strip() not in ('0', 'false', 'False', 'off', '')
        if len(_parsed) > 64:
            _parsed.clear()
        _parsed[env] = hit
    return hit


def option(name):
    if name not in DEFAULTS:
        raise KeyError('unknown engine option %r (known: %s)' % (name, ', '.join(sorted(DEFAULTS))))
    return _parse(os.environ.get('DLWPCS_OPTIONS', '')).get(name, DEFAULTS[name])


def snapshot():
    over = _parse(os.environ.get('DLWPCS_OPTIONS', ''))
    return {k: over.get(k, v) for k, v in DEFAULTS.items()}
```

### dlwp-cs_amd/csrc/conv_mfma.hip

```cpp
#include <stdlib.h>
#include <type_traits>
#include "common.h"
#include "mfma_common.h"
#include "conv_ws.h"
#include "conv_launch.h"

namespace dlwpcs {

template <typename T>
__device__ __forceinline__ void pack_weights_range(const float *__restrict__ w_eq, const float *__restrict__ w_pol,
                                                   const float *__restrict__ w_np, T *__restrict__ out,
                                                   int KS, int Cin, int Cout, int K, int Ncol, int CG, int NTtot,
                                                   int flip, int transposed, size_t total, size_t first, size_t stride) {
    constexpr int J = 16 / (int)sizeof(T);
    const int TAPS = KS * KS;
    const size_t entries = total / J;
    for (size_t e = first; e < entries; e += stride) {
        unsigned r = (unsigned)e;
        const int n = r % 32; r /= 32;
        const int hf = r % 2; r /= 2;
        const int tap = r % TAPS; r /= TAPS;
        const int cg = r % CG; r /= CG;
        const int nt = r % NTtot; r /= NTtot;
        const int v = (int)r;
// ... 1104 lines not shown

__global__ void __launch_bounds__(256) head_stage2_kernel(const float *__restrict__ partial, float *__restrict__ loss_out,
                                                          int nblocks, float inv_n, float weight, int overwrite) {
    loss_stage2_body(partial, loss_out, nblocks, inv_n, weight, overwrite);
}

static bool pw_applies(const dlwpcs_conv_desc *d) {
    return d->dtype == DLWPCS_BF16 && d->ksize == 1 && !d->halo && !d->up0 && d->C1 == 0 && d->C0 == 32 && d->Cout % 2 == 0 &&
           d->Cout >= 8 && d->Cout <= 32 && ((long)d->N * d->N) % 16 == 0 && d->B > 0 &&
           (long)d->B * 6 * d->N * d->N * 32 < (1l << 31);
}
static unsigned pw_grid(long ngroups) {
    long blocks = (ngroups + 4 * PW_U - 1) / (4 * PW_U);
    return (unsigned)(blocks > 2048 ? 2048 : blocks);
}

static inline int cin_logical(const dlwpcs_conv_desc *d);

thread_local ConvEdgeArgs g_edge_args{};

struct WgradBf16Name { static const char *str() { return "wgrad_bf16_kernel"; } };
struct WgradMfmaName { static const char *str() { return "wgrad_mfma_kernel"; } };
struct PwHeadName { static const char *str() { return "pw_head_train_kernel"; } };
struct PwFwdName { static const char *str() { return "pw_fwd_kernel"; } };
static const int g_plain_tags[] = {prof_register_tag("pw_dgrad_kernel<false>"), prof_register_tag("pw_dgrad_kernel<true>"),
                                   prof_register_tag("wgrad_reduce_batch_kernel")};

static int dispatch_conv(int dtype, int KS, int vw, const ConvKParams &P, const Work &W, hipStream_t s) {
    if (KS == 3 && P.mode == MODE_HALO && P.edge) {
        if (dtype == DLWPCS_BF16 && vw == 8) return dispatch_conv_edge(P, W, s);
        return fail(DLWPCS_E_UNSUPPORTED, "conv: gather-form data gradient serves bf16 with 16-B channel vectors");
    }
    return dtype == DLWPCS_BF16 ? dispatch_conv_bf16(KS, vw, P, W, s) : dispatch_conv_f32(KS, vw, P, W, s);
}

static inline int vec_width(int c0, int c1, int dtype) {
    if (dtype == DLWPCS_BF16 && c0 % 8 == 0 && c1 % 8 == 0) return 8;
    if (c0 % 4 == 0 && c1 % 4 == 0) return 4;
    if (c0 % 2 == 0 && c1 % 2 == 0) return 2;
    return 1;
}
static inline int cgw_of(int dtype) { return dtype == DLWPCS_BF16 ? 16 : 8; }

static Work conv_work(const dlwpcs_conv_desc *d) {
    const double No = d->halo ? d->N : d->N - d->ksize + 1;
    const double Cin = cin_logical(d), taps = (double)d->ksize * d->ksize;
    const double n0 = d->up0 ? d->N / 2 : d->N;
    Work w;
    w.flops = 2.0 * d->B * 6 * No * No * taps * Cin * d->Cout;
    w.bytes = (double)dtype_size(d->dtype) * d->B * 6.0 * (n0 * n0 * d->C0 + (double)d->N * d->N * d->C1 + No * No * d->Cout) +
              4.0 * 2.0 * taps * Cin * d->Cout;
    return w;
}

struct Geometry {
    int Cin, CinP8, CG, NT_f, CoutP, NT_b, CGb, No, TAPS;
};

static int validate(const dlwpcs_conv_desc *d, const char *who) {
    if (!d) return fail(DLWPCS_E_INVALID, "%s: null descriptor", who);
    if (!dtype_ok(d->dtype)) return fail(DLWPCS_E_UNSUPPORTED, "%s: dtype %d not built", who, d->dtype);
    if (d->ksize != 1 && d->ksize != 3) return fail(DLWPCS_E_UNSUPPORTED, "%s: kernel size %d (MFMA path serves 1 and 3)", who, d->ksize);
    if (d->B < 0 || d->N < 1 || d->C0 < 1 || d->C1 < 0 || d->Cout < 1) return fail(DLWPCS_E_INVALID, "%s: bad shape B=%d N=%d C0=%d C1=%d Cout=%d", who, d->B, d->N, d->C0, d->C1, d->Cout);
    if (d->up0 && (d->N % 2)) return fail(DLWPCS_E_INVALID, "%s: up0 needs even N", who);
    if (d->halo && d->ksize == 1) return fail(DLWPCS_E_INVALID, "%s: halo with a 1x1 kernel", who);
    if (!d->halo && d->N < d->ksize) return fail(DLWPCS_E_INVALID, "%s: N < kernel size", who);
    if (d->act != DLWPCS_ACT_NONE && d->act != DLWPCS_ACT_LEAKY_CLIP) return fail(DLWPCS_E_INVALID, "%s: unknown activation %d", who, d->act);
    if (d->act == DLWPCS_ACT_LEAKY_CLIP && (!(d->alpha >= 0.f) || !(d->vmax >= 0.f)))
        return fail(DLWPCS_E_INVALID, "%s: activation needs negative_slope >= 0 and max_value >= 0, got %g / %g", who, d->alpha, d->vmax);
    if (d->N > 1024) return fail(DLWPCS_E_UNSUPPORTED, "%s: N > 1024", who);
    if (d->c0_valid != 0) {
        if (d->c0_valid < 1 || d->c0_valid > d->C0) return fail(DLWPCS_E_INVALID, "%s: c0_valid %d outside [1, C0 = %d]", who, d->c0_valid, d->C0);
        if (d->C1 != 0) return fail(DLWPCS_E_INVALID, "%s: c0_valid needs a single source (C1 = 0)", who);
        if (ceil_div(d->c0_valid, 32) != ceil_div(d->C0, 32))
            return fail(DLWPCS_E_INVALID, "%s: c0_valid %d and C0 %d must share their last 32-channel tile", who, d->c0_valid, d->C0);
    }
    return DLWPCS_OK;
}

static inline int out_size(const dlwpcs_conv_desc *d) { return d->halo ? d->N : d->N - d->ksize + 1; }
static inline int cin_logical(const dlwpcs_conv_desc *d) { return (d->c0_valid > 0 ? d->c0_valid : d->C0) + d->C1; }

bool conv_small_serves(int B, int N, int Cin, int Cout);
int launch_conv_small(const ConvKParams &K, hipStream_t s);
static bool conv_small_layer_ok(const dlwpcs_conv_desc *d) {
    return d->dtype == DLWPCS_BF16 && d->ksize == 3 && d->halo && d->C1 == 0 && !d->up0 && d->c0_valid == 0 &&
           !(d->flags & DLWPCS_CONV_OUT_PADDED) && conv_small_serves(d->B, d->N, d->C0, d->Cout);
}

struct WsLayout {
    size_t wpk_f, bias, wpk_b, dxv, dz, partial, bpartial, total;
    int n_eq, n_4, n_5, wg_pix, wg_nblk;
};

static bool wgrad_bf16_eligible(const dlwpcs_conv_desc *d) {
    const bool dz_ok = d->Cout % 8 == 0 || (d->ksize == 1 && d->Cout % 2 == 0 && d->Cout <= 16);
    if (d->Cout % 8 != 0 && (d->C0 % 8 != 0 || d->C1 % 8 != 0)) return false;
    return d->dtype == DLWPCS_BF16 && d->C0 % 2 == 0 && d->C1 % 2 == 0 && dz_ok;
}
static void wgrad_bf16_xcfg(const dlwpcs_conv_desc *d, int &xv, int &qx, int &cap_px, int &ct) {
    ct = 1;
    if (d->C0 % 8 == 0 && d->C1 % 8 == 0) {
        xv = 8; qx = 4; cap_px = 512;
        if ((d->C0 + d->C1) % 64 == 0 && d->Cout % 8 == 0) { ct = 2; cap_px = 320; }
    }
    else if (d->C0 + d->C1 <= 16) { xv = 2; qx = 8; cap_px = 512; }
    else { xv = 2; qx = 16; cap_px = 256; }
}

static bool dz_handover(const dlwpcs_conv_desc *d);

static void wgrad_tiling(const dlwpcs_conv_desc *d, int &pix, int &nblk, int &n_eq, int &n_4, int &n_5) {
    const int No = out_size(d);
    const int face_pix = No * No;
    int CAP = 192;
    int ci_tile = 32;
    if (wgrad_bf16_eligible(d)) {
        int xv, qx, cap_px, ct;
        wgrad_bf16_xcfg(d, xv, qx, cap_px, ct);
        CAP = ct == 2 ? 192 : 384;
        ci_tile = 32 * ct;
        while (CAP > 96 && (long)(tile_rows_for(No <= CAP ? (CAP / No) * No : CAP, No) + d->ksize - 1) * (No + d->ksize - 1) > cap_px)
            CAP -= 96;
    }
    pix = CAP;
    if (No <= CAP) pix = (CAP / No) * No;
    if (pix > face_pix) pix = face_pix;
    nblk = ceil_div(face_pix, pix);
    const int CinP = ceil_div(d->C0 + d->C1, 32) * 32, CoutP = ceil_div(d->Cout, 32) * 32;
    const int pairs = ceil_div(CinP, ci_tile) * (CoutP / 32);
    int wpp = 256 / pairs;
    if (wpp < 3) wpp = 3;
    const long items_per_face = (long)(d->B > 0 ? d->B : 1) * nblk;
    if (wpp > 6 * items_per_face) wpp = (int)(6 * items_per_face);
    if (wpp < 3) wpp = 3;
    n_4 = (wpp + 3) / 6; if (n_4 < 1) n_4 = 1;
    n_5 = n_4;
    n_eq = wpp - n_4 - n_5; if (n_eq < 1) n_eq = 1;
}

static WsLayout ws_layout(const dlwpcs_conv_desc *d);
static bool wgrad_bf16_fits(const dlwpcs_conv_desc *d, const struct WsLayout &L);

static WsLayout ws_layout(const dlwpcs_conv_desc *d) {
    WsLayout L{};
    const int Cin = d->C0 + d->C1, TAPS = d->ksize * d->ksize;
    const int cgw = cgw_of(d->dtype);
    const int CGf = ceil_div(Cin, cgw), NTf = ceil_div(d->Cout, 32);
    const int CGb = ceil_div(d->Cout, cgw), NTb = ceil_div(Cin, 32);
    const int No = out_size(d);
    size_t off = 0;
    L.wpk_f = off; off += align_up((size_t)3 * NTf * CGf * TAPS * 256 * 4, 256);
    L.bias = off;  off += align_up((size_t)3 * NTf * 32 * 4, 256);
    L.wpk_b = off; off += align_up((size_t)3 * NTb * CGb * TAPS * 256 * 4, 256);
    const int Nv = d->halo ? d->N + d->ksize - 1 : d->N;
    L.dxv = off;   off += align_up((size_t)d->B * 6 * Nv * Nv * Cin * dtype_size(d->dtype), 256);
    L.dz = off;    off += align_up((size_t)d->B * 6 * No * No * d->Cout * dtype_size(d->dtype), 256);
    int pix, nblk;
    wgrad_tiling(d, pix, nblk, L.n_eq, L.n_4, L.n_5);
    L.wg_pix = pix; L.wg_nblk = nblk;
    const int nworkers = L.n_eq + L.n_4 + L.n_5;
    const int CinP = ceil_div(Cin, 32) * 32, CoutP = ceil_div(d->Cout, 32) * 32;
    L.partial = off;  off += align_up((size_t)nworkers * TAPS * CinP * CoutP * 4, 256);
    L.bpartial = off; off += align_up((size_t)nworkers * CoutP * 4, 256);
    (void)No;
    L.total = off;
    return L;
// ... 238 lines not shown
                         workspace_bytes, stream, nullptr, nullptr);
}

static int conv_fwd_impl(const dlwpcs_conv_desc *d, const void *src0, const void *src1,
                         const void *w_eq, const void *w_pol, const void *w_np,
                         const void *b_eq, const void *b_pol, const void *b_np,
                         void *y, const int32_t *table_dev,
                         void *workspace, size_t workspace_bytes, dlwpcs_stream_t stream, void *y_pooled, int *pool_done,
                         const ConvHeadArgs *head, bool small) {
    int rc = validate(d, "conv_fwd");
    if (rc) return rc;
    if (small && !conv_small_layer_ok(d))
        return fail(DLWPCS_E_UNSUPPORTED, "conv_small_fwd: serves bf16 3x3 halo layers with one source on faces of <= 320 cells, channel counts multiples of 32");
    if (!src0 || !w_eq || (!w_pol && !(d->flags & DLWPCS_CONV_PREPACKED)) || !y || !workspace)
        return fail(DLWPCS_E_INVALID, "conv_fwd: null pointer");
    if (d->C1 > 0 && !src1) return fail(DLWPCS_E_INVALID, "conv_fwd: C1 > 0 but src1 is null");
    if (d->halo && !table_dev) return fail(DLWPCS_E_INVALID, "conv_fwd: halo requested without table");
    const bool prepacked = (d->flags & DLWPCS_CONV_PREPACKED) != 0;
    if (!prepacked && (b_eq == nullptr) != (b_pol == nullptr)) return fail(DLWPCS_E_INVALID, "conv_fwd: b_eq and b_pol must both be given or both be null");
    const WsLayout L = ws_layout(d);
    if (workspace_bytes < L.total) return fail(DLWPCS_E_WORKSPACE, "conv_fwd: workspace %zu < %zu bytes", workspace_bytes, L.total);
    if (d->B == 0) return DLWPCS_OK;
    hipStream_t s = (hipStream_t)stream;
    char *ws = (char *)workspace;
    const int Cin = d->C0 + d->C1;
    const void *wpk = prepacked ? w_eq : ws + L.wpk_f;
    const float *bpk = prepacked ? (const float *)b_eq : (const float *)(ws + L.bias);
    if (!prepacked) launch_pack(w_eq, w_pol, w_np, ws + L.wpk_f, d->ksize, cin_logical(d), d->Cout, 0, d->flip_north_pole, d->dtype, s);
    const int NTtot = ceil_div(d->Cout, 32);
    if (b_eq && !prepacked) {
        const int n = 3 * NTtot * 32;
        hipLaunchKernelGGL(pack_bias_kernel, dim3(ceil_div(n, 256)), dim3(256), 0, s, (const float *)b_eq,
                           (const float *)b_pol, (const float *)b_np, (float *)(ws + L.bias), d->Cout, NTtot * 32);
    }
    ConvKParams P{};
    P.src0 = src0; P.src1 = src1; P.ymask = nullptr;
    P.wpk = wpk; P.bias = b_eq ? bpk : nullptr; P.out = y; P.table = table_dev;
    P.B = d->B; P.Nin = d->N; P.No = out_size(d);
    P.C0 = d->C0; P.C1 = d->C1; P.Cin = Cin; P.Cout = d->Cout;
    P.CG = ceil_div(Cin, cgw_of(d->dtype)); P.NTtot = NTtot; P.up0 = d->up0;
    P.mode = d->halo ? MODE_HALO : MODE_DIRECT;
    P.act = d->act; P.alpha = d->alpha; P.vmax = d->vmax;
    P.pool_out = y_pooled; P.pool_done = pool_done;
    if (head) { P.head_w = head->wpk; P.head_b = head->bias; P.head_out = head->out; P.head_done = head->done; }
    if ((d->flags & DLWPCS_CONV_OUT_PADDED) && !pw_applies(d))
        return fail(DLWPCS_E_UNSUPPORTED, "conv_fwd: DLWPCS_CONV_OUT_PADDED serves the bf16 pointwise output layer only");
    if (small) return launch_conv_small(P, s);
    if (pw_applies(d)) {
        PwParams Q{};
        Q.in = (const bf16_t *)src0; Q.wpk = (const bf16_t *)wpk; Q.bias = b_eq ? bpk : nullptr; Q.out = (bf16_t *)y;
        Q.ngroups = (long)d->B * 6 * d->N * d->N / 16; Q.groups_per_face = d->N * d->N / 16; Q.Cout = d->Cout;
        if (d->flags & DLWPCS_CONV_OUT_PADDED) Q.Cout = (d->Cout + 7) / 8 * 8;
        Q.alpha = d->alpha; Q.vmax = d->vmax;
        int pidx = -1;
        const bool actv = d->act != DLWPCS_ACT_NONE;
        if (prof_enabled()) {
            const Work wk = conv_work(d);
            const char *tag = Q.Cout <= 16 ? (actv ? KTag<PwFwdName, void, true, 1>::tag() : KTag<PwFwdName, void, false, 1>::tag())
                                           : (actv ? KTag<PwFwdName, void, true, 2>::tag() : KTag<PwFwdName, void, false, 2>::tag());
            pidx = prof_begin(tag, wk.flops, wk.bytes, s);
        }
        const dim3 pgrid(pw_grid(Q.ngroups));
        if (Q.Cout <= 16) {
            if (actv) hipLaunchKernelGGL((pw_fwd_kernel<true, 1>), pgrid, dim3(256), 0, s, Q);
            else hipLaunchKernelGGL((pw_fwd_kernel<false, 1>), pgrid, dim3(256), 0, s, Q);
        } else {
            if (actv) hipLaunchKernelGGL((pw_fwd_kernel<true, 2>), pgrid, dim3(256), 0, s, Q);
            else hipLaunchKernelGGL((pw_fwd_kernel<false, 2>), pgrid, dim3(256), 0, s, Q);
        }
        if (pidx >= 0) prof_end(pidx, s);
        return check_launch("pw_fwd");
    }
    if (d->dtype == DLWPCS_BF16 && d->ksize == 3 && d->halo && d->C1 == 0 && d->C0 >= 8 && d->C0 % 2 == 0 && d->C0 % 8 != 0 &&
        NTtot <= 2) {
        return dispatch_conv_tail8(d->C0 <= 16 ? 16 : 32, NTtot, P, conv_work(d), s);
    }
    return dispatch_conv(d->dtype, d->ksize, vec_width(d->C0, d->C1, d->dtype), P, conv_work(d), s);
}

static int conv_bwd_data_impl(const dlwpcs_conv_desc *d, const void *dy, const void *y, bool dz_given,
                              const void *w_eq, const void *w_pol, const void *w_np,
                              void *dsrc0, void *dsrc1, const void *m0, const void *m1, float m_alpha, float m_vmax,
                              const int32_t *inv_table_dev, void *workspace, size_t workspace_bytes, dlwpcs_stream_t stream,
                              const char *who, int *ring_query = nullptr, bool small = false) {
    int rc = validate(d, who);
    if (rc) return rc;
    if (small && (!conv_small_layer_ok(d) || (d->act != DLWPCS_ACT_NONE && !dz_given) || dsrc1 || !dsrc0))
        return fail(DLWPCS_E_UNSUPPORTED, "%s: serves bf16 3x3 halo layers with one source on faces of <= 320 cells, channel counts multiples of 32, gradient given as dz", who);
    const bool prepacked = (d->flags & DLWPCS_CONV_PREPACKED) != 0;
    if (!dy || !w_eq || (!w_pol && !prepacked) || !workspace) return fail(DLWPCS_E_INVALID, "%s: null pointer", who);
    const bool has_act = d->act != DLWPCS_ACT_NONE && !dz_given;
    if (has_act && !y) return fail(DLWPCS_E_INVALID, "%s: activation needs the saved output y", who);
    if (d->halo && !inv_table_dev) return fail(DLWPCS_E_INVALID, "%s: halo requested without inverse table", who);
    if ((m0 || m1) && (!(m_alpha >= 0.f) || !(m_vmax >= 0.f)))
        return fail(DLWPCS_E_INVALID, "%s: mask activation needs negative_slope >= 0 and max_value >= 0, got %g / %g", who, m_alpha, m_vmax);
    if (!dsrc0 && !dsrc1) return DLWPCS_OK;
    if (!dsrc0) m0 = nullptr;
    if (!dsrc1 || d->C1 == 0) m1 = nullptr;
    const WsLayout L = ws_layout(d);
    if (workspace_bytes < L.total) return fail(DLWPCS_E_WORKSPACE, "%s: workspace %zu < %zu bytes", who, workspace_bytes, L.total);
    if (d->B == 0) return DLWPCS_OK;
    hipStream_t s = (hipStream_t)stream;
    char *ws = (char *)workspace;
    const int Cin = d->C0 + d->C1;
    const void *wpk = prepacked ? w_eq : ws + L.wpk_b;
    void *dxv = ws + L.dxv;
    if (!prepacked) launch_pack(w_eq, w_pol, w_np, ws + L.wpk_b, d->ksize, cin_logical(d), d->Cout, 1, d->flip_north_pole, d->dtype, s);
    const int No = out_size(d);
    const int n0 = d->up0 ? d->N / 2 : d->N;
    const size_t n_src0 = (size_t)d->B * 6 * n0 * n0 * d->C0, n_src1 = (size_t)d->B * 6 * d->N * d->N * d->C1;
    auto finish_masks = [&](bool todo0, bool todo1) -> int {
        int r = DLWPCS_OK;
        if (todo0 && m0) r = launch_mask_inplace(dsrc0, m0, n_src0, m_alpha, m_vmax, d->dtype, s);
        if (!r && todo1 && m1) r = launch_mask_inplace(dsrc1, m1, n_src1, m_alpha, m_vmax, d->dtype, s);
        return r;
    };
    if (pw_applies(d) && !has_act && dsrc0) {
        PwParams Q{};
        Q.in = (const bf16_t *)dy; Q.wpk = (const bf16_t *)wpk; Q.bias = nullptr; Q.out = (bf16_t *)dsrc0;
        Q.ngroups = (long)d->B * 6 * d->N * d->N / 16; Q.groups_per_face = d->N * d->N / 16; Q.Cout = d->Cout;
        int pidx = -1;
        const bool in_kernel_mask = m0 != nullptr;
        if (prof_enabled()) {
            const Work wk = conv_work(d);
            pidx = prof_begin(in_kernel_mask ? "pw_dgrad_kernel<true>" : "pw_dgrad_kernel<false>", wk.flops, wk.bytes, s);
        }
        Q.mask = (const bf16_t *)m0; Q.m_alpha = m_alpha; Q.m_vmax = mask_vmax_for(d->dtype, m_vmax);
        if (in_kernel_mask) hipLaunchKernelGGL(pw_dgrad_kernel<true>, dim3(pw_grid(Q.ngroups)), dim3(256), 0, s, Q);
        else hipLaunchKernelGGL(pw_dgrad_kernel<false>, dim3(pw_grid(Q.ngroups)), dim3(256), 0, s, Q);
        if (pidx >= 0) prof_end(pidx, s);
        rc = check_launch("pw_dgrad");
        return rc ? rc : finish_masks(!in_kernel_mask, false);
    }
    ConvKParams P{};
    const bool dz_ready = !dz_given && dz_handover(d);
    P.src0 = dz_ready ? (const void *)(ws + L.dz) : dy; P.src1 = nullptr;
    P.ymask = (has_act && !dz_ready) ? y : nullptr;
    P.wpk = wpk; P.bias = nullptr; P.out = dxv; P.table = nullptr;
    P.B = d->B; P.Nin = No; P.No = No + d->ksize - 1;
    P.C0 = d->Cout; P.C1 = 0; P.Cin = d->Cout; P.Cout = Cin;
    P.CG = ceil_div(d->Cout, cgw_of(d->dtype)); P.NTtot = ceil_div(Cin, 32); P.up0 = 0;
    P.mode = MODE_ZERO;
    P.act = DLWPCS_ACT_NONE; P.alpha = d->alpha; P.vmax = mask_vmax_for(d->dtype, d->vmax);
    int direct_done = 0, mask_done = 0;
    const bool can_direct = d->halo && d->ksize == 3;
    P.d0 = (can_direct && dsrc0 && !d->up0) ? dsrc0 : nullptr;
    P.d1 = (can_direct && dsrc1 && d->C1 > 0) ? dsrc1 : nullptr;
    P.dsplit = d->C0;
    P.direct_done = &direct_done;
    P.m0 = P.d0 ? m0 : nullptr; P.m1 = P.d1 ? m1 : nullptr;
    P.m_alpha = m_alpha; P.m_vmax = mask_vmax_for(d->dtype, m_vmax); P.m_thr1 = bf16_mask_threshold(m_vmax);
    P.mask_done = &mask_done;
    if ((d->flags & DLWPCS_CONV_DGRAD_GATHER) && d->halo && d->ksize == 3 && d->dtype == DLWPCS_BF16 && !P.ymask && d->N >= 8 &&
        vec_width(d->Cout, 0, d->dtype) == 8 && d->C0 % 8 == 0 && d->C1 % 8 == 0) {
        ConvKParams G = P;
        const int M = d->N + 2;
        const int32_t *plan = inv_table_dev + (size_t)6 * d->N * d->N * 4 + DGG_HEADER;
        G.table = plan; G.edge = 1;
        G.mode = MODE_HALO; G.Nin = d->N; G.No = d->N;
        ConvEdgeArgs EA{};
        EA.src = plan + (size_t)6 * M * M;
        int32_t wids[36];
        int grc = dgrad_gather_wids(d->N, wids);
        for (int k = 0; k < 36; ++k) EA.wids[k] = (int8_t)wids[k];
        g_edge_args = EA;
        G.d0 = (dsrc0 && !d->up0) ? dsrc0 : nullptr;
        G.d1 = (dsrc1 && d->C1 > 0) ? dsrc1 : nullptr;
        G.m0 = G.d0 ? m0 : nullptr; G.m1 = G.d1 ? m1 : nullptr;
        int g_usum = 0;
        G.pool_out = (dsrc0 && d->up0) ? dsrc0 : nullptr; G.pool_mask = G.pool_out ? m0 : nullptr; G.pool_done = &g_usum;
        int g_direct = 0, g_mask = 0;
        G.direct_done = &g_direct; G.mask_done = &g_mask;
        G.dry_run = 1;
        const bool need_direct = G.d0 || G.d1;
        if (!grc) grc = dispatch_conv(d->dtype, d->ksize, 8, G, conv_work(d), s);
        if (!grc && (g_direct || !need_direct)) {
            if (small) return fail(DLWPCS_E_UNSUPPORTED, "%s: this shape is served in gather form", who);
            if (ring_query) { *ring_query = 0; return DLWPCS_OK; }
            G.dry_run = 0;
            grc = dispatch_conv(d->dtype, d->ksize, 8, G, conv_work(d), s);
            if (grc) return grc;
            bool todo0 = m0 != nullptr && !(G.d0 && (g_mask & 1)) && !g_usum, todo1 = m1 != nullptr && !(G.d1 && (g_mask & 2));
            if (dsrc0 && !G.d0 && !g_usum) {
                int masked = 0;
                grc = launch_src_grad(dxv, dsrc0, nullptr, d->B, d->N, Cin, 0, d->C0, d->up0, 0, d->dtype, s, m0, m_alpha, m_vmax, &masked);
                if (grc) return grc;
                if (masked) todo0 = false;
            }
            if (dsrc1 && d->C1 > 0 && !G.d1) {
                int masked = 0;
                grc = launch_src_grad(dxv, dsrc1, nullptr, d->B, d->N, Cin, d->C0, d->C1, 0, 0, d->dtype, s, m1, m_alpha, m_vmax, &masked);
                if (grc) return grc;
                if (masked) todo1 = false;
            }
            return finish_masks(todo0, todo1);
        }
    }
    const bool whole = !d->halo && !d->up0 && d->C1 == 0 && dsrc0;
    if (whole) P.out = dsrc0;
    P.dry_run = ring_query ? 1 : 0;
    rc = small ? launch_conv_small(P, s) : dispatch_conv(d->dtype, d->ksize, vec_width(d->Cout, 0, d->dtype), P, conv_work(d), s);
    if (ring_query) { *ring_query = (!rc && direct_done && P.d0 && !m0) ? 1 : 0; return rc; }
    if (rc) return rc;
    if (whole) return finish_masks(true, false);
    bool todo0 = m0 != nullptr, todo1 = m1 != nullptr;
    const bool direct0 = direct_done && P.d0, direct1 = direct_done && P.d1;
    const void *rm0 = (direct0 && !(mask_done & 1)) ? nullptr : m0;
    const void *rm1 = (direct1 && !(mask_done & 2)) ? nullptr : m1;
    if (dsrc0 && dsrc1 && d->C1 > 0 && d->halo && direct_done && !P.d0 && P.d1) {
        rc = launch_src_pair(dxv, dsrc0, dsrc1, inv_table_dev, d->B, d->N, d->C0, d->C1, d->up0, d->dtype, s, m0, rm1, m_alpha, m_vmax);
        if (rc) return rc;
        return finish_masks(false, todo1 && !rm1);
    }
    if (dsrc0) {
        if (direct0 && !m0 && (d->flags & DLWPCS_CONV_DEFER_RING0)) {
        } else if (direct0) {
            rc = launch_ring_fix(dxv, dsrc0, inv_table_dev, d->B, d->N, Cin, 0, d->C0, d->dtype, s, rm0, m_alpha, m_vmax);
            if (rm0) todo0 = false;
        } else {
            int masked = 0;
            rc = launch_src_grad(dxv, dsrc0, inv_table_dev, d->B, d->N, Cin, 0, d->C0, d->up0, d->halo, d->dtype, s, m0, m_alpha, m_vmax, &masked);
            if (masked) todo0 = false;
        }
        if (rc) return rc;
    }
    if (dsrc1 && d->C1 > 0) {
        if (direct1) {
            rc = launch_ring_fix(dxv, dsrc1, inv_table_dev, d->B, d->N, Cin, d->C0, d->C1, d->dtype, s, rm1, m_alpha, m_vmax);
            if (rm1) todo1 = false;
        } else {
            int masked = 0;
            rc = launch_src_grad(dxv, dsrc1, inv_table_dev, d->B, d->N, Cin, d->C0, d->C1, 0, d->halo, d->dtype, s, m1, m_alpha, m_vmax, &masked);
            if (masked) todo1 = false;
        }
        if (rc) return rc;
    }
    return finish_masks(todo0, todo1);
}

extern "C" int dlwpcs_conv_bwd_data(const dlwpcs_conv_desc *d, const void *dy, const void *y,
                                    const void *w_eq, const void *w_pol, const void *w_np,
                                    void *dsrc0, void *dsrc1, const int32_t *inv_table_dev,
                                    void *workspace, size_t workspace_bytes, dlwpcs_stream_t stream) {
    return conv_bwd_data_impl(d, dy, y, false, w_eq, w_pol, w_np, dsrc0, dsrc1, nullptr, nullptr, 0.f, 0.f, inv_table_dev, workspace,
                              workspace_bytes, stream, "conv_bwd_data");
}

extern "C" int dlwpcs_conv_bwd_data_masked(const dlwpcs_conv_desc *d, const void *dz,
                                           const void *w_eq, const void *w_pol, const void *w_np,
                                           void *dsrc0, void *dsrc1, const void *m0, const void *m1, float m_alpha, float m_vmax,
                                           const int32_t *inv_table_dev,
                                           void *workspace, size_t workspace_bytes, dlwpcs_stream_t stream) {
    return conv_bwd_data_impl(d, dz, nullptr, true, w_eq, w_pol, w_np, dsrc0, dsrc1, m0, m1, m_alpha, m_vmax, inv_table_dev, workspace,
                              workspace_bytes, stream, "conv_bwd_data_masked");
}

extern "C" int dlwpcs_conv_small_fwd(const dlwpcs_conv_desc *d, const void *src0, const void *src1,
                                     const void *w_eq, const void *w_pol, const void *w_np,
                                     const void *b_eq, const void *b_pol, const void *b_np,
                                     void *y, const int32_t *table_dev,
                                     void *workspace, size_t workspace_bytes, dlwpcs_stream_t stream) {
    return conv_fwd_impl(d, src0, src1, w_eq, w_pol, w_np, b_eq, b_pol, b_np, y, table_dev, workspace, workspace_bytes, stream,
                         nullptr, nullptr, nullptr, true);
}

extern "C" int dlwpcs_conv_small_bwd_data(const dlwpcs_conv_desc *d, const void *dz,
                                          const void *w_eq, const void *w_pol, const void *w_np,
                                          void *dsrc0, void *dsrc1, const void *m0, const void *m1, float m_alpha, float m_vmax,
                                          const int32_t *inv_table_dev,
                                          void *workspace, size_t workspace_bytes, dlwpcs_stream_t stream) {
    return conv_bwd_data_impl(d, dz, nullptr, true, w_eq, w_pol, w_np, dsrc0, dsrc1, m0, m1, m_alpha, m_vmax, inv_table_dev, workspace,
                              workspace_bytes, stream, "conv_small_bwd_data", nullptr, true);
}

extern "C" int dlwpcs_conv_ring_info(const dlwpcs_conv_desc *d, size_t *dxv_offset, int *channels) {
    if (validate(d, "conv_ring_info") != DLWPCS_OK || !dxv_offset || !channels) return 0;
    if (!d->halo || d->ksize != 3 || d->up0 || d->B < 1) return 0;
    const WsLayout L = ws_layout(d);
    int q = 0;
    char dummy = 0;
    dlwpcs_conv_desc dd = *d;
    dd.act = DLWPCS_ACT_NONE;
    dd.flags |= DLWPCS_CONV_PREPACKED;
    const int rc = conv_bwd_data_impl(&dd, &dummy, nullptr, true, &dummy, nullptr, nullptr, &dummy, d->C1 > 0 ? &dummy : nullptr, nullptr,
                                      nullptr, 0.f, 0.f, (const int32_t *)&dummy, &dummy, L.total, nullptr, "conv_ring_info", &q);
    if (rc || !q) return 0;
    *dxv_offset = L.dxv;
    *channels = d->C0 + d->C1;
    return 1;
}

extern "C" int dlwpcs_conv_bwd_weights(const dlwpcs_conv_desc *d, const void *src0, const void *src1, const void *dy,
                                       const void *y, void *dw_eq, void *dw_pol, void *dw_np,
                                       void *db_eq, void *db_pol, void *db_np, const int32_t *table_dev,
                                       void *workspace, size_t workspace_bytes, dlwpcs_stream_t stream) {
    int rc = validate(d, "conv_bwd_weights");
    if (rc) return rc;
    if (!src0 || !dy || !dw_eq || !dw_pol || !workspace) return fail(DLWPCS_E_INVALID, "conv_bwd_weights: null pointer");
    if (d->C1 > 0 && !src1) return fail(DLWPCS_E_INVALID, "conv_bwd_weights: C1 > 0 but src1 is null");
    if (d->act != DLWPCS_ACT_NONE && !y) return fail(DLWPCS_E_INVALID, "conv_bwd_weights: activation needs the saved output y");
    if (d->halo && !table_dev) return fail(DLWPCS_E_INVALID, "conv_bwd_weights: halo requested without table");
    if ((db_np != nullptr) != (dw_np != nullptr) && db_eq) return fail(DLWPCS_E_INVALID, "conv_bwd_weights: dw_np/db_np must match");
    const WsLayout L = ws_layout(d);
    if (workspace_bytes < L.total) return fail(DLWPCS_E_WORKSPACE, "conv_bwd_weights: workspace %zu < %zu bytes", workspace_bytes, L.total);
    hipStream_t s = (hipStream_t)stream;
    char *ws = (char *)workspace;
    const int Cin = d->C0 + d->C1, KS = d->ksize, TAPS = KS * KS;
    const int CinP = ceil_div(Cin, 32) * 32, CoutP = ceil_div(d->Cout, 32) * 32;
    if (d->B == 0 && (d->flags & DLWPCS_CONV_ACCUMULATE_WGRAD)) return DLWPCS_OK;
    if (d->B == 0) {
        const size_t wbytes = (size_t)TAPS * cin_logical(d) * d->Cout * 4;
        (void)hipMemsetAsync(dw_eq, 0, wbytes, s);
        (void)hipMemsetAsync(dw_pol, 0, wbytes, s);
        if (dw_np) (void)hipMemsetAsync(dw_np, 0, wbytes, s);
        if (db_eq) (void)hipMemsetAsync(db_eq, 0, (size_t)d->Cout * 4, s);
        if (db_pol) (void)hipMemsetAsync(db_pol, 0, (size_t)d->Cout * 4, s);
        if (db_np) (void)hipMemsetAsync(db_np, 0, (size_t)d->Cout * 4, s);
        return DLWPCS_OK;
    }
    WgradKParams W{};
    ConvKParams &P = W.c;
    P.src0 = src0; P.src1 = src1; P.ymask = nullptr; P.table = table_dev;
    P.B = d->B; P.Nin = d->N; P.No = out_size(d);
    P.C0 = d->C0; P.C1 = d->C1; P.Cin = Cin; P.Cout = d->Cout; P.up0 = d->up0;
    P.mode = d->halo ? MODE_HALO : MODE_DIRECT;
    P.alpha = d->alpha; P.vmax = mask_vmax_for(d->dtype, d->vmax);
    P.pix_per_block = L.wg_pix; P.nblk_face = L.wg_nblk;
    P.W2 = P.No + KS - 1; P.magicW2 = div_magic(P.W2); P.magicNo = div_magic(P.No);
    P.tile_rows_max = tile_rows_for(L.wg_pix, P.No) + (KS - 1);
    W.dy = dy; W.y = y;
    W.dz_out = dz_handover(d) ? ws + L.dz : nullptr;
    W.partial = (float *)(ws + L.partial);
    const bool want_bias = db_eq || db_pol || db_np;
    W.bpartial = want_bias ? (float *)(ws + L.bpartial) : nullptr;
    W.CinP = CinP; W.CoutP = CoutP;
    W.n_eq = L.n_eq; W.n_4 = L.n_4; W.n_5 = L.n_5;
    P.magicN = div_magic(P.Nin);
    P.tune = tune_bits();
    W.magicB = P.B > 1 ? div_magic(P.B) : 0; W.magicNb = P.nblk_face > 1 ? div_magic(P.nblk_face) : 0;
    if (P.C1 == 0) P.src1 = P.src0;
    const bool mask = d->act != DLWPCS_ACT_NONE;
    dim3 grid((unsigned)(L.n_eq + L.n_4 + L.n_5), (unsigned)(CinP / 32), (unsigned)(CoutP / 32));
    int xv = 0, qx = 0, cap_px = 0, ct = 1;
    if (wgrad_bf16_eligible(d)) wgrad_bf16_xcfg(d, xv, qx, cap_px, ct);
    if (wgrad_bf16_fits(d, L)) {
        const int pcap = (L.wg_pix + 15) & ~15;
        size_t lds = 2 * ((size_t)ct * P.tile_rows_max * P.W2 * 64 + (size_t)pcap * 64);
        grid.y = (unsigned)(CinP / (32 * ct));
        {
            const int nph = 4 / ct, rslots = TAPS - TAPS / nph;
            const size_t need = ((size_t)4 * rslots * 1024 + 2048) * 4;
            if (lds < need) lds = need;
        }
        if (lds > 160 * 1024) return fail(DLWPCS_E_UNSUPPORTED, "conv_bwd_weights: LDS tile of %zu bytes exceeds 160 KiB", lds);
        if ((long)P.Nin * P.Nin >= (1l << 16))
            return fail(DLWPCS_E_UNSUPPORTED, "conv_bwd_weights: face size %d too large for the 16-bit index arithmetic", P.Nin);
#define WGB_LAUNCH(KSV, MASKV, XVV, QXV, CTV, DVV)                                                                        \
    do {                                                                                                                  \
        auto kern = wgrad_bf16_kernel<KSV, MASKV, XVV, QXV, CTV, DVV>;                                                    \
        if (lds > 64 * 1024) {                                                                                            \
            hipError_t e = hipFuncSetAttribute((const void *)kern, hipFuncAttributeMaxDynamicSharedMemorySize, (int)lds); \
            if (e != hipSuccess) return fail(DLWPCS_E_LAUNCH, "wgrad: hipFuncSetAttribute: %s", hipGetErrorString(e));    \
        }                                                                                                                 \
        int pidx = -1;                                                                                                    \
        if (prof_enabled()) {                                                                                             \
            const Work wk = conv_work(d);                                                                                 \
            pidx = prof_begin(KTag<WgradBf16Name, void, KSV, MASKV, XVV, QXV, CTV, DVV>::tag(), wk.flops, wk.bytes, s);   \
        }                                                                                                                 \
        hipLaunchKernelGGL(kern, grid, dim3(512), lds, s, W);                                                             \
// ... 132 lines not shown
```

### dlwp-cs_amd/csrc/conv_small.hip

```cpp
#include "conv_ws.h"

namespace dlwpcs {

struct SmallParams {
    const void *src;
    const void *wpk;
    const float *bias;
    const int32_t *table;
    void *out;
    void *d0;
    const void *m0;
    int B, Ns, No, W2;
    int Cin, Cout, CG, NT;
    int Q;
    uint32_t magicQ, magicW2, magicNo, magicNT, magicB;
    int act;
    float alpha, vmax;
    float m_alpha;
    uint32_t m_thr1;
    int patch_base;
};

constexpr int SM_THREADS = 256, SM_WAVES = 4;
constexpr int SM_PROW = 32 * 2 + 16;
constexpr int SM_U = 16;

template <bool BWD, int MTW>
__global__ void __launch_bounds__(SM_THREADS, 2) conv_small_kernel(const SmallParams P) {
    extern __shared__ __attribute__((aligned(16))) char smem[];
    const int tid = threadIdx.x;
    const int lane = tid & 63, wave = __builtin_amdgcn_readfirstlane(tid >> 6);
    const int half = lane >> 5, l31 = lane & 31;
    const uint32_t t = xcd_remap(blockIdx.x, gridDim.x);
    const int bf = P.magicNT ? __umulhi(t, P.magicNT) : (int)t;
    const int nt = (int)t - bf * P.NT;
    const int f = P.magicB ? __umulhi((uint32_t)bf, P.magicB) : bf;
    const int b = bf - f * P.B;
    const int v = f < 4 ? 0 : (f == 4 ? 1 : 2);
    const int RB = P.Cin * 2 + 16;
    const int face_pix = P.No * P.No;
    const int ncells = P.W2 * P.W2;
    const int nitems = ncells * P.Q;

    const uint4 *wsrc = reinterpret_cast<const uint4 *>(P.wpk) + ((size_t)v * P.NT + nt) * P.CG * 576 + lane;
    auto load_w = [&](int cg, uint4 (&w)[9]) __attribute__((always_inline)) {
        const uint4 *p = wsrc + (size_t)min(cg, P.CG - 1) * 576;
#pragma unroll
        for (int tap = 0; tap < 9; ++tap) w[tap] = p[tap * 64];
    };
    uint4 wa[9], wb[9];
    load_w(0, wa);

    {
        const int spix = 6 * P.Ns * P.Ns;
        const rsrc_t rs = make_rsrc(reinterpret_cast<const bf16_t *>(P.src) + (size_t)b * spix * P.Cin, (uint32_t)(spix * P.Cin * 2));
#pragma unroll 1
        for (int e0 = 0; e0 < nitems; e0 += SM_THREADS * SM_U) {
            int sp[SM_U];
#pragma unroll
            for (int u = 0; u < SM_U; ++u) {
                const int e = e0 + tid + u * SM_THREADS;
                const bool live = e < nitems;
                const int cell = __umulhi((uint32_t)e, P.magicQ);
                if constexpr (!BWD) {
                    sp[u] = P.table[live ? f * ncells + cell : 0];
                    if (!live) sp[u] = -1;
                } else {
                    const int ty = __umulhi((uint32_t)cell, P.magicW2), tx = cell - ty * P.W2;
                    const int vy = ty - 2, vx = tx - 2;
                    const bool ok = live & ((uint32_t)vy < (uint32_t)P.Ns) & ((uint32_t)vx < (uint32_t)P.Ns);
                    sp[u] = ok ? (f * P.Ns + vy) * P.Ns + vx : -1;
                }
            }
            u32x4 val[SM_U];
#pragma unroll
            for (int u = 0; u < SM_U; ++u) {
                const int e = e0 + tid + u * SM_THREADS;
                const int cell = __umulhi((uint32_t)e, P.magicQ), qv = e - cell * P.Q;
                const uint32_t off = sp[u] >= 0 ? (uint32_t)(sp[u] * P.Cin + qv * 8) * 2u : ST_SKIP;
                val[u] = __builtin_amdgcn_raw_buffer_load_b128(rs, off, 0, 0);
            }
#pragma unroll
            for (int u = 0; u < SM_U; ++u) {
                const int e = e0 + tid + u * SM_THREADS;
                const int cell = __umulhi((uint32_t)e, P.magicQ), qv = e - cell * P.Q;
                if (e < nitems) *reinterpret_cast<uint4 *>(smem + cell * RB + qv * 16) = make_uint4(val[u].x, val[u].y, val[u].z, val[u].w);
            }
        }
    }

    const int nmt = (face_pix + 31) >> 5;
    const int wv = (wave + (int)(blockIdx.x >> 3) + (int)(blockIdx.x >> 8)) & (SM_WAVES - 1);
    const int my_mt = max(0, min(MTW, (nmt - wv + SM_WAVES - 1) / SM_WAVES));
    int abase[MTW];
#pragma unroll
    for (int i = 0; i < MTW; ++i) {
        const int m = (wv + SM_WAVES * i) * 32 + l31;
        int base = 0;
        if (m < face_pix) {
            const int oy = __umulhi((uint32_t)m, P.magicNo), ox = m - oy * P.No;
            base = (oy * P.W2 + ox) * RB;
        }
        abase[i] = base + half * 16;
    }
    float4 bq[4];
#pragma unroll
    for (int jq = 0; jq < 4; ++jq)
        bq[jq] = P.bias ? *reinterpret_cast<const float4 *>(P.bias + (size_t)v * P.NT * 32 + nt * 32 + 8 * jq + 4 * half)
                        : make_float4(0.f, 0.f, 0.f, 0.f);
    f32x16 acc[MTW];

    load_w(1, wb);
    __syncthreads();
    if (my_mt == 0) return;

    auto matrix = [&](auto mta_tag) __attribute__((always_inline)) {
        constexpr int MTA = decltype(mta_tag)::value;
        constexpr int SM_R = MTA == 1 ? 6 : 3, SM_D = SM_R - 1;
        uint4 fa[SM_R][MTA];
#pragma unroll
        for (int i = 0; i < MTA; ++i)
#pragma unroll
            for (int jq = 0; jq < 4; ++jq) {
                acc[i][4 * jq] = bq[jq].x; acc[i][4 * jq + 1] = bq[jq].y; acc[i][4 * jq + 2] = bq[jq].z; acc[i][4 * jq + 3] = bq[jq].w;
            }
        auto rd = [&](int cg, int tap, uint4 (&a)[MTA]) __attribute__((always_inline)) {
            const char *lds = smem + cg * 32 + ((tap / 3) * P.W2 + tap % 3) * RB;
#pragma unroll
            for (int i = 0; i < MTA; ++i) a[i] = *reinterpret_cast<const uint4 *>(lds + abase[i]);
        };
#pragma unroll
        for (int st = 0; st < SM_D; ++st) rd(0, st, fa[st % SM_R]);
        __builtin_amdgcn_sched_group_barrier(0x100, SM_D * MTA, 0);
#pragma unroll 1
        for (int cg = 0; cg < P.CG; cg += 2) {
#pragma unroll
            for (int st = 0; st < 18; ++st) {
                rd(cg + (st + SM_D) / 9, (st + SM_D) % 9, fa[(st + SM_D) % SM_R]);
#pragma unroll
                for (int i = 0; i < MTA; ++i) frag_mma<bf16_t>(acc[i], st < 9 ? wa[st] : wb[st - 9], fa[st % SM_R][i]);
                __builtin_amdgcn_sched_group_barrier(0x100, MTA, 0);
                __builtin_amdgcn_sched_group_barrier(0x008, MTA, 0);
                if (st == 8) { asm volatile("" ::: "memory"); load_w(cg + 2, wa); }
                if (st == 17) { asm volatile("" ::: "memory"); load_w(cg + 3, wb); }
            }
        }
    };
    if (MTW >= 3 && my_mt >= 3) matrix(std::integral_constant<int, (MTW >= 3 ? 3 : 1)>{});
    else if (MTW >= 2 && my_mt == 2) matrix(std::integral_constant<int, (MTW >= 2 ? 2 : 1)>{});
    else matrix(std::integral_constant<int, 1>{});

    constexpr int NPS = 2;
    uint32_t soff[MTW][NPS];
    uint32_t ssel = 0;
    const int c = nt * 32 + (lane & 3) * 8;
#pragma unroll
    for (int i = 0; i < MTW; ++i)
#pragma unroll
        for (int ps = 0; ps < NPS; ++ps) {
            const int m = (wv + SM_WAVES * i) * 32 + ps * 16 + (lane >> 2);
            const int oy = __umulhi((uint32_t)m, P.magicNo), ox = m - oy * P.No;
            int off = ((f * face_pix + m) * P.Cout + c) * 2;
            if constexpr (BWD) {
                const int Nd = P.No - 2;
                const bool interior = ((uint32_t)(oy - 1) < (uint32_t)Nd) & ((uint32_t)(ox - 1) < (uint32_t)Nd);
                if (interior && P.d0 != nullptr) {
                    off = (((f * Nd + (oy - 1)) * Nd + (ox - 1)) * P.Cout + c) * 2;
                    ssel |= 1u << (i * NPS + ps);
                }
// ... 1 lines not shown
            soff[i][ps] = m < face_pix ? (uint32_t)off : ST_SKIP;
        }
    uint4 ymq[BWD ? MTW : 1][NPS];
    if constexpr (BWD) {
        const int dpix = 6 * (P.No - 2) * (P.No - 2);
        const rsrc_t rm = make_rsrc(P.m0 ? reinterpret_cast<const bf16_t *>(P.m0) + (size_t)b * dpix * P.Cout : nullptr, (uint32_t)(dpix * P.Cout * 2));
#pragma unroll
        for (int i = 0; i < MTW; ++i)
#pragma unroll
            for (int ps = 0; ps < NPS; ++ps) {
                const u32x4 a = __builtin_amdgcn_raw_buffer_load_b128(rm, ((ssel >> (i * NPS + ps)) & 1u) ? soff[i][ps] : ST_SKIP, 0, 0);
                ymq[i][ps] = make_uint4(a.x, a.y, a.z, a.w);
            }
    }
    const float e_alpha = P.act == DLWPCS_ACT_LEAKY_CLIP ? P.alpha : 1.f;
    const float e_vmax = P.act == DLWPCS_ACT_LEAKY_CLIP ? P.vmax : __builtin_inff();
    const bool fast_act = e_alpha >= 0.f && e_alpha <= 1.f && e_vmax >= 0.f;
    const int amode = (BWD || P.act != DLWPCS_ACT_LEAKY_CLIP) ? 2 : (fast_act ? 1 : 0);
    auto quad = [&](const f32x16 &a, int jq) __attribute__((always_inline)) {
        float4 v4 = make_float4(a[4 * jq], a[4 * jq + 1], a[4 * jq + 2], a[4 * jq + 3]);
        if (amode == 2) return v4;
        if (amode == 1) {
            typedef float f32x2 __attribute__((ext_vector_type(2)));
            auto lc = [&](float x, float ax) {
                float tt, y;
                asm("v_max_f32 %0, %1, %2" : "=v"(tt) : "v"(x), "v"(ax));
                asm("v_minimum3_f32 %0, %1, %2, %2" : "=v"(y) : "v"(tt), "v"(e_vmax));
                return y;
            };
            const f32x2 a01 = f32x2{v4.x, v4.y} * e_alpha, a23 = f32x2{v4.z, v4.w} * e_alpha;
            v4.x = lc(v4.x, a01.x); v4.y = lc(v4.y, a01.y); v4.z = lc(v4.z, a23.x); v4.w = lc(v4.w, a23.y);
        } else {
            v4.x = act_leaky_clip(v4.x, e_alpha, e_vmax); v4.y = act_leaky_clip(v4.y, e_alpha, e_vmax);
            v4.z = act_leaky_clip(v4.z, e_alpha, e_vmax); v4.w = act_leaky_clip(v4.w, e_alpha, e_vmax);
        }
        return v4;
    };
    const rsrc_t d_out = make_rsrc(reinterpret_cast<bf16_t *>(P.out) + (size_t)b * 6 * face_pix * P.Cout, (uint32_t)(6 * face_pix * P.Cout * 2));
    const int dpix = 6 * (P.No - 2) * (P.No - 2);
    const rsrc_t d_0 = BWD ? make_rsrc(P.d0 ? reinterpret_cast<bf16_t *>(P.d0) + (size_t)b * dpix * P.Cout : nullptr, (uint32_t)(dpix * P.Cout * 2))
                           : d_out;
    char *const patch = smem + P.patch_base + wave * (32 * SM_PROW);
    if constexpr (BWD) {
#pragma unroll
        for (int i = 0; i < MTW; ++i)
#pragma unroll
            for (int ps = 0; ps < NPS; ++ps) asm volatile("" : "+v"(ymq[i][ps].x), "+v"(ymq[i][ps].y), "+v"(ymq[i][ps].z), "+v"(ymq[i][ps].w));
    }
#pragma unroll
    for (int i = 0; i < MTW; ++i) {
        if (i < my_mt) {
#pragma unroll
            for (int k = 0; k < 4; ++k) {
                const float4 v4 = quad(acc[i], k);
                *reinterpret_cast<uint2 *>(patch + l31 * SM_PROW + (8 * k + 4 * half) * 2) = make_uint2(f2bf2(v4.x, v4.y), f2bf2(v4.z, v4.w));
            }
            __builtin_amdgcn_wave_barrier();
#pragma unroll
            for (int ps = 0; ps < NPS; ++ps) {
                uint4 o = *reinterpret_cast<const uint4 *>(patch + (ps * 16 + (lane >> 2)) * SM_PROW + (lane & 3) * 16);
                if constexpr (BWD) {
                    const bool to0 = ((ssel >> (i * NPS + ps)) & 1u) != 0;
                    uint4 om = o;
                    vmask_pk(om, ymq[i][ps], P.m_alpha, P.m_thr1);
                    const bool on = to0 && P.m0 != nullptr;
                    o.x = on ? om.x : o.x; o.y = on ? om.y : o.y; o.z = on ? om.z : o.z; o.w = on ? om.w : o.w;
                    bst128(o, d_out, to0 ? ST_SKIP : soff[i][ps]);
                    bst128(o, d_0, to0 ? soff[i][ps] : ST_SKIP);
                } else {
                    bst128(o, d_out, soff[i][ps]);
                }
            }
            __builtin_amdgcn_wave_barrier();
        }
    }
}

bool conv_small_serves(int B, int N, int Cin, int Cout) {
    const int cmax = Cin > Cout ? Cin : Cout;
    return N >= 2 && N * N <= 320 && Cin >= 32 && Cout >= 32 && Cin % 32 == 0 && Cout % 32 == 0 &&
           (size_t)(N + 4) * (N + 4) * (cmax * 2 + 16) + (size_t)SM_WAVES * 32 * SM_PROW <= 160 * 1024 && (long)B * 6 * (cmax / 32) < (1l << 16);
}

template <bool BWD>
static int launch_small_t(const SmallParams &P, int mtw, size_t lds, unsigned grid, hipStream_t s) {
    auto go = [&](auto kern) -> int {
        if (lds > 64 * 1024) {
            hipError_t e = hipFuncSetAttribute((const void *)kern, hipFuncAttributeMaxDynamicSharedMemorySize, (int)lds);
            if (e != hipSuccess) return fail(DLWPCS_E_LAUNCH, "conv_small: hipFuncSetAttribute: %s", hipGetErrorString(e));
        }
        hipLaunchKernelGGL(kern, dim3(grid), dim3(SM_THREADS), lds, s, P);
        return check_launch("conv_small");
    };
    if (mtw == 1) return go(conv_small_kernel<BWD, 1>);
    if (mtw == 2) return go(conv_small_kernel<BWD, 2>);
    return go(conv_small_kernel<BWD, 3>);
}

int launch_conv_small(const ConvKParams &K, hipStream_t s) {
    const bool bwd = K.mode == MODE_ZERO;
    if (K.mode != MODE_HALO && !bwd) return fail(DLWPCS_E_UNSUPPORTED, "conv_small: serves halo convolutions and their data gradients");
    const int N = K.Nin;
    if (K.C1 != 0 || K.up0 || K.ymask || K.pool_out || K.head_w || K.edge)
        return fail(DLWPCS_E_UNSUPPORTED, "conv_small: one source, no upsampling, no mask on load, no pooled or folded second output");
    if (K.No != (bwd ? N + 2 : N) || !conv_small_serves(K.B, N, K.Cin, K.Cout))
        return fail(DLWPCS_E_UNSUPPORTED, "conv_small: N=%d Cin=%d Cout=%d outside faces of <= 320 cells with channel counts that are multiples of 32",
                    N, K.Cin, K.Cout);
    if (bwd && K.d1) return fail(DLWPCS_E_UNSUPPORTED, "conv_small: one source");
    if (bwd && K.d0 && K.dsplit != K.Cout) return fail(DLWPCS_E_UNSUPPORTED, "conv_small: one source");
    SmallParams P{};
    P.src = K.src0; P.wpk = K.wpk; P.bias = K.bias; P.table = K.table; P.out = K.out;
    P.d0 = bwd ? K.d0 : nullptr;
    P.m0 = (bwd && K.d0) ? K.m0 : nullptr;
    P.B = K.B; P.Ns = N; P.No = K.No; P.W2 = K.No + 2;
    P.Cin = K.Cin; P.Cout = K.Cout; P.CG = K.Cin / 16; P.NT = K.Cout / 32; P.Q = K.Cin / 8;
    P.magicQ = div_magic(P.Q); P.magicW2 = div_magic(P.W2); P.magicNo = div_magic(P.No);
    P.magicNT = P.NT > 1 ? div_magic(P.NT) : 0; P.magicB = P.B > 1 ? div_magic(P.B) : 0;
    P.act = K.act; P.alpha = K.alpha; P.vmax = K.vmax;
    P.m_alpha = K.m_alpha; P.m_thr1 = K.m_thr1;
    const size_t in_b = (size_t)P.W2 * P.W2 * (P.Cin * 2 + 16);
    P.patch_base = (int)in_b;
    const size_t lds = in_b + (size_t)SM_WAVES * 32 * SM_PROW;
    const int nmt = ceil_div(P.No * P.No, 32), mtw = ceil_div(nmt, SM_WAVES);
    const long nwg = (long)P.B * 6 * P.NT;
    if (lds > 160 * 1024 || mtw > 3 || nwg >= (1l << 16) || P.W2 * P.W2 * P.Q >= (1 << 16))
        return fail(DLWPCS_E_UNSUPPORTED, "conv_small: B=%d N=%d Cin=%d beyond the kernel's LDS tile or index range", P.B, N, P.Cin);
    if (K.direct_done) *K.direct_done = (bwd && P.d0) ? 1 : 0;
    if (K.mask_done) *K.mask_done = P.m0 ? 1 : 0;
    if (K.pool_done) *K.pool_done = 0;
    if (K.head_done) *K.head_done = 0;
    if (K.dry_run || K.B == 0) return DLWPCS_OK;
    return bwd ? launch_small_t<true>(P, mtw, lds, (unsigned)nwg, s) : launch_small_t<false>(P, mtw, lds, (unsigned)nwg, s);
}

}
```

### dlwp-cs_amd/csrc/elementwise.hip

```cpp
#include "common.h"

namespace dlwpcs {

static inline dim3 stream_grid(size_t work_items, int block = 256) {
    size_t g = (work_items + block - 1) / block;
    if (g > 2048) g = 2048;
    if (g < 1) g = 1;
    return dim3((unsigned)g);
}

struct H2 { uint32_t u; };
struct alignas(16) H8 { uint4 u; };
template <int N> struct Acc { float v[N]; };
template <int N> __device__ __forceinline__ Acc<N> vadd(Acc<N> a, const Acc<N> &b) {
#pragma unroll
    for (int i = 0; i < N; ++i) a.v[i] += b.v[i];
    return a;
}
template <int N> __device__ __forceinline__ Acc<N> vscale(Acc<N> a, float s) {
#pragma unroll
    for (int i = 0; i < N; ++i) a.v[i] *= s;
    return a;
}
template <int N> __device__ __forceinline__ Acc<N> vmaskacc(Acc<N> a, const Acc<N> &y, float alpha, float vmax) {
// ... 830 lines not shown
        hipLaunchKernelGGL(pad_bwd_kernel<V>, stream_grid(total), dim3(256), 0, s, (const V *)dy, (V *)dx, inv_table_dev,
                           total, C / w, N, p);
    });
    return check_launch("pad_bwd");
}

namespace dlwpcs {
int launch_mask_inplace(void *dx, const void *m, size_t n, float alpha, float vmax, int dtype, hipStream_t s);

int launch_src_grad(const void *dxv, void *dsrc, const int32_t *inv, int B, int N, int CT, int choff, int CS, int up,
                    int halo, int dtype, hipStream_t s, const void *msrc, float m_alpha, float m_vmax, int *masked) {
    if (masked) *masked = msrc ? 1 : 0;
    m_vmax = mask_vmax_for(dtype, m_vmax);
    const int No = up ? N / 2 : N;
    int g = 8;
    while (g > 1 && (CT % g || choff % g || CS % g)) g >>= 1;
    dispatch_vec(dtype, g, [&](auto tag, int w) {
        using V = decltype(tag);
        const size_t total = (size_t)B * 6 * No * No * (CS / w);
        if (halo)
            hipLaunchKernelGGL(pad_bwd_src_kernel<V>, stream_grid(total), dim3(256), 0, s, (const V *)dxv, (V *)dsrc, inv,
                               total, CS / w, CT / w, choff / w, N, up, (const V *)msrc, m_alpha, m_vmax);
        else
            hipLaunchKernelGGL(window_src_kernel<V>, stream_grid(total), dim3(256), 0, s, (const V *)dxv, (V *)dsrc, total,
                               CS / w, CT / w, choff / w, N, up, (const V *)msrc, m_alpha, m_vmax);
    });
    return check_launch("src_grad");
}

int launch_src_pair(const void *dxv, void *dsrc0, void *dsrc1, const int32_t *inv, int B, int N, int C0, int C1, int up0,
                    int dtype, hipStream_t s, const void *m0, const void *m1, float m_alpha, float m_vmax) {
    const int CT = C0 + C1;
    m_vmax = mask_vmax_for(dtype, m_vmax);
    int g = 8;
    while (g > 1 && (C0 % g || C1 % g)) g >>= 1;
    const int No = up0 ? N / 2 : N;
    const int nb = N > 1 ? 4 * N - 4 : 1;
    dispatch_vec(dtype, g, [&](auto tag, int w) {
        using V = decltype(tag);
        const size_t total0 = (size_t)B * 6 * No * No * (C0 / w), total1 = (size_t)B * 6 * nb * (C1 / w);
        const unsigned nb0 = stream_grid(total0).x, nb1 = stream_grid(total1).x;
        hipLaunchKernelGGL(src_pair_kernel<V>, dim3(nb0 + nb1), dim3(256), 0, s, (const V *)dxv, (V *)dsrc0, (V *)dsrc1, inv,
                           total0, total1, C0 / w, C1 / w, CT / w, N, up0, nb0, (const V *)m0, (const V *)m1, m_alpha, m_vmax);
    });
    return check_launch("src_pair");
}

int launch_ring_fix(const void *dxv, void *dsrc, const int32_t *inv, int B, int N, int CT, int choff, int CS, int dtype,
                    hipStream_t s, const void *msrc, float m_alpha, float m_vmax) {
    m_vmax = mask_vmax_for(dtype, m_vmax);
    int g = 8;
    while (g > 1 && (CT % g || choff % g || CS % g)) g >>= 1;
    const int nb = N > 1 ? 4 * N - 4 : 1;
    dispatch_vec(dtype, g, [&](auto tag, int w) {
        using V = decltype(tag);
        const size_t total = (size_t)B * 6 * nb * (CS / w);
        hipLaunchKernelGGL(pad_ring_fix_kernel<V>, stream_grid(total), dim3(256), 0, s, (const V *)dxv, (V *)dsrc, inv, total,
                           CS / w, CT / w, choff / w, N, (const V *)msrc, m_alpha, m_vmax);
    });
    return check_launch("ring_fix");
}

int launch_mask_inplace(void *dx, const void *m, size_t n, float alpha, float vmax, int dtype, hipStream_t s) {
    if (n == 0) return DLWPCS_OK;
    vmax = mask_vmax_for(dtype, vmax);
    const bool vec = aligned16(dx, m);
    if (dtype == DLWPCS_BF16) {
        if (vec)
            hipLaunchKernelGGL((act_bwd_kernel<H8, bf16_t>), stream_grid(n / 8 + 1), dim3(256), 0, s, (const bf16_t *)dx,
                               (const bf16_t *)m, (bf16_t *)dx, n, alpha, vmax);
        else
            hipLaunchKernelGGL((act_bwd_kernel<bf16_t, bf16_t>), stream_grid(n), dim3(256), 0, s, (const bf16_t *)dx,
                               (const bf16_t *)m, (bf16_t *)dx, n, alpha, vmax);
    } else {
        if (vec)
            hipLaunchKernelGGL((act_bwd_kernel<float4, float>), stream_grid(n / 4 + 1), dim3(256), 0, s, (const float *)dx,
                               (const float *)m, (float *)dx, n, alpha, vmax);
        else
            hipLaunchKernelGGL((act_bwd_kernel<float, float>), stream_grid(n), dim3(256), 0, s, (const float *)dx,
                               (const float *)m, (float *)dx, n, alpha, vmax);
    }
    return check_launch("mask_inplace");
}
}

extern "C" int dlwpcs_act_fwd(const void *x, void *y, size_t n, int act, float alpha, float vmax, int dtype,
                              dlwpcs_stream_t stream) {
    REQUIRE_DTYPE(dtype, "act_fwd");
    REQUIRE(x && y, "act_fwd: null pointer");
    REQUIRE(act == DLWPCS_ACT_LEAKY_CLIP, "act_fwd: unknown activation %d", act);
    if (n == 0) return DLWPCS_OK;
    const bool vec = aligned16(x, y);
    if (dtype == DLWPCS_BF16) {
        if (vec)
            hipLaunchKernelGGL((act_fwd_kernel<H8, bf16_t>), stream_grid(n / 8 + 1), dim3(256), 0, (hipStream_t)stream,
                               (const bf16_t *)x, (bf16_t *)y, n, alpha, vmax);
        else
            hipLaunchKernelGGL((act_fwd_kernel<bf16_t, bf16_t>), stream_grid(n), dim3(256), 0, (hipStream_t)stream,
                               (const bf16_t *)x, (bf16_t *)y, n, alpha, vmax);
    } else {
        if (vec)
            hipLaunchKernelGGL((act_fwd_kernel<float4, float>), stream_grid(n / 4 + 1), dim3(256), 0, (hipStream_t)stream,
                               (const float *)x, (float *)y, n, alpha, vmax);
        else
            hipLaunchKernelGGL((act_fwd_kernel<float, float>), stream_grid(n), dim3(256), 0, (hipStream_t)stream,
                               (const float *)x, (float *)y, n, alpha, vmax);
    }
    return check_launch("act_fwd");
}

extern "C" int dlwpcs_act_bwd(const void *dy, const void *y, void *dx, size_t n, int act, float alpha, float vmax,
                              int dtype, dlwpcs_stream_t stream) {
    REQUIRE_DTYPE(dtype, "act_bwd");
    REQUIRE(dy && y && dx, "act_bwd: null pointer");
    REQUIRE(act == DLWPCS_ACT_LEAKY_CLIP, "act_bwd: unknown activation %d", act);
    if (n == 0) return DLWPCS_OK;
    vmax = mask_vmax_for(dtype, vmax);
    const bool vec = aligned16(dy, y, dx);
    if (dtype == DLWPCS_BF16) {
        if (vec)
            hipLaunchKernelGGL((act_bwd_kernel<H8, bf16_t>), stream_grid(n / 8 + 1), dim3(256), 0, (hipStream_t)stream,
                               (const bf16_t *)dy, (const bf16_t *)y, (bf16_t *)dx, n, alpha, vmax);
        else
            hipLaunchKernelGGL((act_bwd_kernel<bf16_t, bf16_t>), stream_grid(n), dim3(256), 0, (hipStream_t)stream,
                               (const bf16_t *)dy, (const bf16_t *)y, (bf16_t *)dx, n, alpha, vmax);
    } else {
        if (vec)
            hipLaunchKernelGGL((act_bwd_kernel<float4, float>), stream_grid(n / 4 + 1), dim3(256), 0, (hipStream_t)stream,
                               (const float *)dy, (const float *)y, (float *)dx, n, alpha, vmax);
        else
            hipLaunchKernelGGL((act_bwd_kernel<float, float>), stream_grid(n), dim3(256), 0, (hipStream_t)stream,
                               (const float *)dy, (const float *)y, (float *)dx, n, alpha, vmax);
    }
    return check_launch("act_bwd");
}

#define POOL_LAUNCH(KERNEL, IN, OUT, TOTAL_PIX, NARG)                                                                  \
    dispatch_vec(dtype, C, [&](auto tag, int w) {                                                                      \
        using V = decltype(tag);                                                                                       \
        const size_t total = (size_t)(TOTAL_PIX) * (C / w);                                                            \
        hipLaunchKernelGGL(KERNEL<V>, stream_grid(total), dim3(256), 0, (hipStream_t)stream, (const V *)(IN),          \
                           (V *)(OUT), total, C / w, NARG);                                                            \
    });

extern "C" int dlwpcs_avgpool2_fwd(const void *x, void *y, int B, int N, int C, int dtype, dlwpcs_stream_t stream) {
    REQUIRE_DTYPE(dtype, "avgpool2_fwd");
    REQUIRE(x && y, "avgpool2_fwd: null pointer");
    REQUIRE(B >= 0 && N >= 2 && N % 2 == 0 && C >= 1, "avgpool2_fwd: bad shape B=%d N=%d C=%d", B, N, C);
    if (B == 0) return DLWPCS_OK;
    POOL_LAUNCH(avgpool2_fwd_kernel, x, y, (size_t)B * 6 * (N / 2) * (N / 2), N)
    return check_launch("avgpool2_fwd");
}
extern "C" int dlwpcs_avgpool2_bwd(const void *dy, void *dx, int B, int N, int C, int dtype, dlwpcs_stream_t stream) {
    REQUIRE_DTYPE(dtype, "avgpool2_bwd");
    REQUIRE(dy && dx, "avgpool2_bwd: null pointer");
    REQUIRE(B >= 0 && N >= 2 && N % 2 == 0 && C >= 1, "avgpool2_bwd: bad shape B=%d N=%d C=%d", B, N, C);
    if (B == 0) return DLWPCS_OK;
    POOL_LAUNCH(avgpool2_bwd_kernel, dy, dx, (size_t)B * 6 * N * N, N)
    return check_launch("avgpool2_bwd");
}
extern "C" int dlwpcs_avgpool2_bwd_add(const void *dy, const void *dskip, void *dx, int B, int N, int C, int dtype,
                                       dlwpcs_stream_t stream) {
    REQUIRE_DTYPE(dtype, "avgpool2_bwd_add");
    REQUIRE(dy && dskip && dx, "avgpool2_bwd_add: null pointer");
    REQUIRE(B >= 0 && N >= 2 && N % 2 == 0 && C >= 1, "avgpool2_bwd_add: bad shape B=%d N=%d C=%d", B, N, C);
    if (B == 0) return DLWPCS_OK;
// ... 488 lines not shown
```

### include/dlwpcs.h

```cpp
#ifndef DLWPCS_H
#define DLWPCS_H

#include <stddef.h>
#include <stdint.h>

#ifdef __cplusplus
extern "C" {
#endif

#define DLWPCS_VERSION 105

#define DLWPCS_OK             0
#define DLWPCS_E_INVALID     -1
#define DLWPCS_E_UNSUPPORTED -2
#define DLWPCS_E_WORKSPACE   -3
#define DLWPCS_E_LAUNCH      -4

#define DLWPCS_F32  0
#define DLWPCS_BF16 1

#define DLWPCS_ACT_NONE        0
#define DLWPCS_ACT_LEAKY_CLIP  1

typedef void *dlwpcs_stream_t;

int dlwpcs_version(void);
const char *dlwpcs_last_error(void);


int dlwpcs_halo_table(int N, int p, int32_t *out);

int dlwpcs_halo_inverse_table(int N, int p, int32_t *inv);

size_t dlwpcs_dgrad_gather_plan_ints(int N);
int dlwpcs_dgrad_gather_plan(int N, int32_t *out);

int dlwpcs_pad_fwd(const void *x, void *y, int B, int N, int C, int p, int dtype,
                   const int32_t *table_dev, dlwpcs_stream_t stream);
int dlwpcs_pad_bwd(const void *dy, void *dx, int B, int N, int C, int p, int dtype,
                   const int32_t *inv_table_dev, dlwpcs_stream_t stream);

#define DLWPCS_CONV_ACCUMULATE_WGRAD 1
#define DLWPCS_CONV_PREPACKED        2
#define DLWPCS_CONV_REUSE_DZ         4
#define DLWPCS_CONV_DEFER_RING0     16
#define DLWPCS_CONV_DGRAD_GATHER    64
#define DLWPCS_CONV_OUT_PADDED      32
#define DLWPCS_CONV_DEFER_REDUCE     8

typedef struct dlwpcs_conv_desc {
    int32_t B;
    int32_t N;
    int32_t C0, C1;
    int32_t Cout;
    int32_t ksize;
    int32_t halo;
    int32_t up0;
    int32_t flip_north_pole;
    int32_t act;
    float   alpha, vmax;
    int32_t dtype;
    int32_t flags;
    int32_t c0_valid;
} dlwpcs_conv_desc;

size_t dlwpcs_conv_workspace_bytes(const dlwpcs_conv_desc *d);

#define DLWPCS_PACK_FWD  0
#define DLWPCS_PACK_BWD  1
#define DLWPCS_PACK_BIAS 2
typedef struct dlwpcs_pack_item {
    const void *w_eq, *w_pol, *w_np;
    const void *b_eq, *b_pol, *b_np;
    void *wpk_fwd, *wpk_bwd, *bias_pk;
    int32_t ksize, Cin, Cout, flip_north_pole, dtype, reserved;
} dlwpcs_pack_item;
size_t dlwpcs_conv_packed_bytes(const dlwpcs_conv_desc *d, int which);
int dlwpcs_pack_batch(const dlwpcs_pack_item *items_dev, int n_items, dlwpcs_stream_t stream);

int dlwpcs_conv_fwd(const dlwpcs_conv_desc *d,
                    const void *src0, const void *src1,
                    const void *w_eq, const void *w_pol, const void *w_np,
                    const void *b_eq, const void *b_pol, const void *b_np,
                    void *y, const int32_t *table_dev,
                    void *workspace, size_t workspace_bytes, dlwpcs_stream_t stream);
int dlwpcs_conv_fwd_pool(const dlwpcs_conv_desc *d, const void *src0, const void *src1,
                         const void *w_eq, const void *w_pol, const void *w_np,
                         const void *b_eq, const void *b_pol, const void *b_np,
                         void *y, void *y_pooled, const int32_t *table_dev,
                         void *workspace, size_t workspace_bytes, dlwpcs_stream_t stream);
int dlwpcs_conv_fwd_head(const dlwpcs_conv_desc *d, const void *src0, const void *src1, const void *wpk_fwd,
                         const void *bias_pk, const dlwpcs_conv_desc *dh, const void *head_wpk_fwd,
                         const void *head_bias_pk, void *y, void *y_head, const int32_t *table_dev,
                         void *workspace, size_t workspace_bytes, int *fused, dlwpcs_stream_t stream);

int dlwpcs_conv_bwd_data(const dlwpcs_conv_desc *d,
                         const void *dy, const void *y,
                         const void *w_eq, const void *w_pol, const void *w_np,
                         void *dsrc0, void *dsrc1, const int32_t *inv_table_dev,
                         void *workspace, size_t workspace_bytes, dlwpcs_stream_t stream);

int dlwpcs_conv_bwd_data_masked(const dlwpcs_conv_desc *d, const void *dz,
                                const void *w_eq, const void *w_pol, const void *w_np,
                                void *dsrc0, void *dsrc1, const void *m0, const void *m1, float m_alpha, float m_vmax,
                                const int32_t *inv_table_dev,
                                void *workspace, size_t workspace_bytes, dlwpcs_stream_t stream);

int dlwpcs_conv_small_fwd(const dlwpcs_conv_desc *d,
                          const void *src0, const void *src1,
                          const void *w_eq, const void *w_pol, const void *w_np,
                          const void *b_eq, const void *b_pol, const void *b_np,
                          void *y, const int32_t *table_dev,
                          void *workspace, size_t workspace_bytes, dlwpcs_stream_t stream);
int dlwpcs_conv_small_bwd_data(const dlwpcs_conv_desc *d, const void *dz,
                               const void *w_eq, const void *w_pol, const void *w_np,
                               void *dsrc0, void *dsrc1, const void *m0, const void *m1, float m_alpha, float m_vmax,
                               const int32_t *inv_table_dev,
                               void *workspace, size_t workspace_bytes, dlwpcs_stream_t stream);

int dlwpcs_conv_ring_info(const dlwpcs_conv_desc *d, size_t *dxv_offset, int *channels);

int dlwpcs_conv_bwd_weights(const dlwpcs_conv_desc *d,
                            const void *src0, const void *src1, const void *dy, const void *y,
                            void *dw_eq, void *dw_pol, void *dw_np,
                            void *db_eq, void *db_pol, void *db_np,
                            const int32_t *table_dev,
                            void *workspace, size_t workspace_bytes, dlwpcs_stream_t stream);

typedef struct dlwpcs_reduce_item {
    const float *partial, *bpartial;
    float *dw_eq, *dw_pol, *dw_np, *db_eq, *db_pol, *db_np;
    int32_t ksize, Cin, Cout, CinP, CoutP, n_eq, n_4, n_5, flip_north_pole, accumulate, vec, nblocks;
    int32_t reserved[4];
} dlwpcs_reduce_item;
int dlwpcs_conv_wgrad_reduce_item(const dlwpcs_conv_desc *d,
                                  void *dw_eq, void *dw_pol, void *dw_np,
                                  void *db_eq, void *db_pol, void *db_np,
                                  void *workspace, size_t workspace_bytes, dlwpcs_reduce_item *item);
int dlwpcs_wgrad_reduce_batch(const dlwpcs_reduce_item *items_dev, const dlwpcs_reduce_item *items_host, int n_items,
                              dlwpcs_stream_t stream);

#define DLWPCS_WGRAD_BATCH_MAX 24
typedef struct dlwpcs_wgrad_item {
    dlwpcs_conv_desc d;
    const void *src0, *src1;
    const void *dz;
    const void *y;
    const int32_t *table_dev;
    void *dw_eq, *dw_pol, *dw_np;
    void *db_eq, *db_pol, *db_np;
} dlwpcs_wgrad_item;
int dlwpcs_wgrad_batch_supported(const dlwpcs_conv_desc *d);
int dlwpcs_wgrad_batch_sizes(const dlwpcs_wgrad_item *items, int n_items, size_t *plan_bytes, size_t *workspace_bytes);
int dlwpcs_wgrad_batch_plan(const dlwpcs_wgrad_item *items, int n_items, void *plan_host, size_t plan_bytes);
int dlwpcs_wgrad_batch(const dlwpcs_wgrad_item *items, int n_items, const void *plan_host, const void *plan_dev,
                       void *workspace, size_t workspace_bytes, dlwpcs_stream_t stream);
int dlwpcs_wgrad_batch_adam(const dlwpcs_wgrad_item *items, int n_items, const void *plan_host, const void *plan_dev,
                            void *workspace, size_t workspace_bytes, float *p, float *g, float *m, float *v, size_t n,
                            int32_t *state_dev, const float *hyper_dev, dlwpcs_stream_t stream);
struct dlwpcs_loss_tail;
int dlwpcs_wgrad_batch_adam_tail(const dlwpcs_wgrad_item *items, int n_items, const void *plan_host, const void *plan_dev,
                                 void *workspace, size_t workspace_bytes, float *p, float *g, float *m, float *v, size_t n,
                                 int32_t *state_dev, const float *hyper_dev, const struct dlwpcs_loss_tail *tail,
                                 const dlwpcs_pack_item *pack_items_host, dlwpcs_stream_t stream);

int dlwpcs_wgrad_batch_apply(const dlwpcs_wgrad_item *items, int n_items, const void *plan_host, const void *plan_dev,
                             float *p, float *g, float *m, float *v, size_t n, int32_t *state_dev, const float *hyper_dev,
                             const struct dlwpcs_loss_tail *tail, const dlwpcs_pack_item *pack_items_host, dlwpcs_stream_t stream);

typedef struct dlwpcs_gconv_desc {
    int32_t B, H, W, Cin, Cout;
    int32_t kh, kw, sh, sw, dh, dw;
    int32_t pad_t, pad_l;
    int32_t Ho, Wo;
    int32_t flip_north_pole;
    int32_t dtype;
} dlwpcs_gconv_desc;

int dlwpcs_gconv_fwd(const dlwpcs_gconv_desc *d, const void *x,
                     const void *w_eq, const void *w_pol, const void *w_np,
                     const void *b_eq, const void *b_pol, const void *b_np, void *y, dlwpcs_stream_t stream);
int dlwpcs_gconv_bwd_data(const dlwpcs_gconv_desc *d, const void *dy,
                          const void *w_eq, const void *w_pol, const void *w_np, void *dx, dlwpcs_stream_t stream);
int dlwpcs_gconv_bwd_weights(const dlwpcs_gconv_desc *d, const void *x, const void *dy,
                             void *dw_eq, void *dw_pol, void *dw_np, void *db_eq, void *db_pol, void *db_np,
                             dlwpcs_stream_t stream);

int dlwpcs_act_fwd(const void *x, void *y, size_t n, int act, float alpha, float vmax, int dtype,
                   dlwpcs_stream_t stream);
int dlwpcs_act_bwd(const void *dy, const void *y, void *dx, size_t n, int act, float alpha, float vmax, int dtype,
                   dlwpcs_stream_t stream);
int dlwpcs_avgpool2_fwd(const void *x, void *y, int B, int N, int C, int dtype, dlwpcs_stream_t stream);
int dlwpcs_avgpool2_bwd(const void *dy, void *dx, int B, int N, int C, int dtype, dlwpcs_stream_t stream);
int dlwpcs_avgpool2_bwd_add(const void *dy, const void *dskip, void *dx, int B, int N, int C, int dtype,
                            dlwpcs_stream_t stream);
int dlwpcs_avgpool2_bwd_masked(const void *dy, const void *dskip, const void *m, void *dx, int B, int N, int C,
                               float m_alpha, float m_vmax, int dtype, dlwpcs_stream_t stream);
int dlwpcs_avgpool2_bwd_ring(const void *dy, const void *dskip, const void *m, void *dx, int B, int N, int C,
                             float m_alpha, float m_vmax, int dtype, const void *ring, const int32_t *inv_half_dev,
                             int ring_channels, int ring_choff, dlwpcs_stream_t stream);
int dlwpcs_upsample2_fwd(const void *x, void *y, int B, int N, int C, int dtype, dlwpcs_stream_t stream);
// ... 409 lines not shown
```

Measured before the change: 50230 samples/s.

## Fold producer's deferred window/ring gradient assembly into the small-conv backward kernel

When a conv's input gradient feeds a single small halo conv, the producer's bwd-data now skips writing the final source gradient. It leaves the raw window (for upsampling layers) or ring partial in its workspace, and the next small-conv backward kernel assembles it. That kernel gathers the window, applies the activation mask and writes dz before running its own data gradient. This removes a separate src-window or ring fix-up pass and its memory round trip, at the cost of substantial plan bookkeeping and a more complex kernel. The window form is enabled by default and the ring form is off.

```diff
diff --git a/dlwp-cs_amd/DLWP/_native.py b/dlwp-cs_amd/DLWP/_native.py
--- a/dlwp-cs_amd/DLWP/_native.py
+++ b/dlwp-cs_amd/DLWP/_native.py
@@ -30,6 +30,9 @@
 CONV_DEFER_RING0 = 16
 CONV_OUT_PADDED = 32
 CONV_DGRAD_GATHER = 64
+CONV_DEFER_RING0M = 128
+CONV_DEFER_WINDOW0 = 256
+FOLD_WINDOW, FOLD_RING = 1, 2
 CONSTRAINT_MAX_NORM, CONSTRAINT_NON_NEG, CONSTRAINT_UNIT_NORM, CONSTRAINT_MIN_MAX_NORM = 1, 2, 3, 4
 PACK_FWD, PACK_BWD, PACK_BIAS = 0, 1, 2
 WGRAD_BATCH_MAX = 24
@@ -44,6 +47,12 @@
                 ('up0', ctypes.c_int32), ('flip_north_pole', ctypes.c_int32), ('act', ctypes.c_int32),
                 ('alpha', ctypes.c_float), ('vmax', ctypes.c_float), ('dtype', ctypes.c_int32),
                 ('flags', ctypes.c_int32), ('c0_valid', ctypes.c_int32)]
+
+
+class SmallFold(ctypes.Structure):
+    _fields_ = [(n, ctypes.c_int32) for n in ('form', 'channels', 'choff', 'reserved')] + \
+               [(n, ctypes.c_void_p) for n in ('partial', 'producer', 'inv_table_dev', 'm', 'dz_out')] + \
+               [('m_alpha', ctypes.c_float), ('m_vmax', ctypes.c_float)]
 
 
 class PackItem(ctypes.Structure):
@@ -206,6 +215,12 @@
                                                                                        c_void_p]),
     'dlwpcs_conv_small_bwd_data': (c_int, [ctypes.POINTER(ConvDesc)] + [c_void_p] * 4 + [c_void_p] * 4 + [c_float, c_float] +
                                    [c_void_p, c_void_p, c_size_t, c_void_p]),
+    'dlwpcs_conv_small_bwd_data_fold': (c_int, [ctypes.POINTER(ConvDesc), ctypes.POINTER(SmallFold)] + [c_void_p] * 3 +
+                                        [c_void_p, c_void_p, c_float, c_float, c_void_p, c_void_p, c_size_t, c_void_p]),
+    'dlwpcs_src_window': (c_int, [c_void_p, c_void_p, c_int, c_int, c_int, c_int, c_int, c_int, c_int, c_void_p, c_float, c_float,
+                                  c_void_p]),
+    'dlwpcs_conv_fold_info': (c_int, [ctypes.POINTER(ConvDesc), ctypes.POINTER(ConvDesc), c_int, ctypes.POINTER(c_size_t),
+                                      ctypes.POINTER(c_int)]),
     'dlwpcs_conv_bwd_weights': (c_int, [ctypes.POINTER(ConvDesc)] + [c_void_p] * 4 + [c_void_p] * 6 +
                                 [c_void_p, c_void_p, c_size_t, c_void_p]),
     'dlwpcs_conv_wgrad_reduce_item': (c_int, [ctypes.POINTER(ConvDesc)] + [c_void_p] * 6 +
diff --git a/dlwp-cs_amd/DLWP/custom.py b/dlwp-cs_amd/DLWP/custom.py
--- a/dlwp-cs_amd/DLWP/custom.py
+++ b/dlwp-cs_amd/DLWP/custom.py
@@ -203,13 +203,14 @@
         return (self._is_mfma_config() and self.kernel_size[0] == 3 and pad_width == 1 and self.activation is None)
 
     def fused_call(self, src0, src1=None, up0=False, halo=True, act=ACT_NONE, alpha=0.0, vmax=0.0, premask0=None,
-                   premask1=None, dy_premasked=False, defer_ring0=False, want_pool=False, out_padded=False, small=False):
+                   premask1=None, dy_premasked=False, defer_ring0=False, want_pool=False, out_padded=False, small=False,
+                   fold0=0):
         return ops.cs_conv(src0, self.equatorial_kernel, self.polar_kernel, self.north_pole_kernel,
                            self.equatorial_bias, self.polar_bias, self.north_pole_bias, src1=src1,
                            ksize=self.kernel_size[0], halo=halo, up0=up0, flip_north_pole=self.flip_north_pole,
                            act=act, alpha=alpha, vmax=vmax, premask0=premask0, premask1=premask1,
                            dy_premasked=dy_premasked, defer_ring0=defer_ring0, want_pool=want_pool, out_padded=out_padded,
-                           small=small)
+                           small=small, fold0=fold0)
 
     def call(self, inputs, channels_last_io=False, **kwargs):
         channels_first = self.data_format == 'channels_first' and not channels_last_io
diff --git a/dlwp-cs_amd/DLWP/keras/models.py b/dlwp-cs_amd/DLWP/keras/models.py
--- a/dlwp-cs_amd/DLWP/keras/models.py
+++ b/dlwp-cs_amd/DLWP/keras/models.py
@@ -65,6 +65,8 @@
         self.fuse_head_loss = option('fuse_head')
         self.fold_head = option('fold_head')
         self.small_conv = option('small_conv')
+        self.small_fold = option('small_fold')
+        self.small_fold_ring = option('small_fold_ring')
         self.static_batch_buffers = False
         self._ones = {}
         self._compiled = False
@@ -259,6 +261,18 @@
                     and steps[r[0]][4] != st[1] and not steps[r[0]][5]:
                 self._defer_ring.add(r[0])
 
+        producer_of = {st[1]: i for i, st in enumerate(steps) if st[0] == 'fused_conv'}
+        self._fold_small = {}
+        for i, st in enumerate(steps):
+            if st[0] != 'fused_conv' or not src_mask[i][0] or st[3] == st[4]:
+                continue
+            u = st[3]
+            c = producer_of.get(u)
+            if (c is None or u not in self._premask or u in out_uids or readers.get(u) != [i] or steps[c][4] is not None
+                    or steps[c][5] or steps[c][3] in in_uids_model or (not st[5] and st[4] is not None)):
+                continue
+            self._fold_small[i] = c
+
     def _runs_channels_last(self, lay):
         return lay.data_format == 'channels_last' or self._cf_model
 
@@ -295,6 +309,14 @@
             return None
         self._exchange_cut = (cut, int(lo_a) // 64 * 64)
         return self._exchange_cut
+
+    def _fold0(self, i, pm, cut, values):
+        c = self._fold_small.get(i)
+        if c is None or not pm or not self.small_conv or (cut is not None and c < cut <= i):
+            return 0
+        if not (self.small_fold if self._plan[i][5] else self.small_fold_ring):
+            return 0
+        return int(values[self._plan[c][3]].shape[-1])
 
     def _premask_on(self):
         return (self.compute_dtype == 'bfloat16' and torch.is_grad_enabled()
@@ -390,7 +412,7 @@
                                                  dy_premasked=out_uid in pm,
                                                  defer_ring0=bool(pm) and self.fold_ring and i in self._defer_ring,
                                                  want_pool=self.fuse_pool and i in self._pool_producers,
-                                                 small=self.small_conv)
+                                                 small=self.small_conv, fold0=self._fold0(i, pm, cut, values))
             elif st[0] == 'pool_skip':
                 _, out_uid, lay, in_uid = st
                 values[out_uid], values[in_uid] = ops.avgpool2_skip(values[in_uid],
@@ -724,10 +746,10 @@
                 ops.WGRAD_BATCH = False
                 ops.drop_deferred_reduce()
                 ops.drop_wgrad_batch()
-                if ops._pending_ring:
+                if ops._pending_ring or ops._pending_fold:
                     ops.drop_pending_rings()
                     if sys.exc_info()[0] is None:
-                        raise RuntimeError('a deferred ring fix-up was not consumed by its pooling node (plan error)')
+                        raise RuntimeError('a deferred ring fix-up / folded gradient was not consumed by the node behind it (plan error)')
                 ops.finish_loss_tail()
                 ops.join_side_stream(stats[0].device)
         if len(stats) == 1:
diff --git a/dlwp-cs_amd/DLWP/ops.py b/dlwp-cs_amd/DLWP/ops.py
--- a/dlwp-cs_amd/DLWP/ops.py
+++ b/dlwp-cs_amd/DLWP/ops.py
@@ -277,8 +277,25 @@
 _POOLED = {}
 
 
+_pending_fold = {}
+
+
 def drop_pending_rings():
     _pending_ring.clear()
+    _pending_fold.clear()
+
+
+_fold_info_cache = {}
+
+
+def small_fold_info(dp, dc, form):
+    key = tuple((d.B, d.N, d.C0, d.C1, d.Cout, d.ksize, d.halo, d.up0, d.dtype, d.c0_valid, d.flags & nat.CONV_DGRAD_GATHER)
+                for d in (dp, dc)) + (form,)
+    if key not in _fold_info_cache:
+        off, ch = ctypes.c_size_t(), ctypes.c_int()
+        ok = lib().dlwpcs_conv_fold_info(ctypes.byref(dp), ctypes.byref(dc), int(form), ctypes.byref(off), ctypes.byref(ch))
+        _fold_info_cache[key] = (off.value, ch.value) if ok else None
+    return _fold_info_cache[key]
 
 
 def _c(t):
@@ -434,7 +451,7 @@
     @staticmethod
     def forward(ctx, src0, src1, w_eq, w_pol, w_np, b_eq, b_pol, b_np, ksize, halo, up0, flip, act, alpha, vmax,
                 c0_valid=0, premask0=None, premask1=None, dy_premasked=False, defer_ring0=False, want_pool=False,
-                out_padded=False, small=False):
+                out_padded=False, small=False, fold0=0):
         require_device(src0, 'cs_conv')
         src0 = _c(src0)
         B = src0.shape[0]
@@ -501,6 +518,7 @@
         ctx.premask = (premask0, premask1)
         ctx.dy_premasked = bool(dy_premasked) and act != nat.ACT_NONE
         ctx.defer_ring0 = bool(defer_ring0)
+        ctx.fold0 = int(fold0)
         ctx.packed = packed
         ctx.desc = d
         ctx.tables = (table, inv)
@@ -549,6 +567,20 @@
                 dn.flags |= nat.CONV_DEFER_RING0
                 if not defer:
                     ws = _workspace(nbytes, dev, 'ring%d' % len(_pending_ring))
+            fold_in = _pending_fold.get(dy.data_ptr()) if ctx.dy_premasked else None
+            if fold_in is not None and not (ctx.small and dsrc0 is not None and dsrc1 is None and y is not None):
+                raise RuntimeError('cs_conv: a folded gradient reached a layer that cannot assemble it (plan error)')
+            fold_out = None
+            if ctx.fold0 and dsrc0 is not None and pm0 is not None and (d.up0 or (ctx.small and dsrc1 is None)):
+                form = nat.FOLD_WINDOW if d.up0 else nat.FOLD_RING
+                dc = _make_desc(d.B, d.N // 2 if d.up0 else d.N, ctx.fold0, 0, d.C0, 3, True, False, d.flip_north_pole, nat.ACT_NONE,
+                                0.0, 0.0, d.dtype)
+                info = small_fold_info(dn, dc, form)
+                if info is not None:
+                    fold_out = (form, info)
+                    dn.flags |= nat.CONV_DEFER_WINDOW0 if d.up0 else nat.CONV_DEFER_RING0M
+                    if not defer:
+                        ws = _workspace(nbytes, dev, 'fold%d' % len(_pending_fold))
             if dsrc0 is not None or dsrc1 is not None:
                 wq = ctx.packed[3] if ctx.packed is not None else w_eq
                 pm = pm0 if pm0 is not None else pm1
@@ -557,17 +589,35 @@
                          ptr(src0 if pm0 is not None else None), ptr(src1 if pm1 is not None else None), ma, mv, ptr(inv), ptr(ws),
                          ws.numel(), stream_ptr())
                 rc = nat.E_UNSUPPORTED
-                if ctx.small and dsrc0 is not None and dsrc1 is None:
+                if fold_in is not None:
+                    fws, foff, fch, form, finv, fpm = fold_in
+                    dz = torch.empty_like(dy)
+                    sf = nat.SmallFold(form=form, channels=fch, choff=0, reserved=0,
+                                       partial=ptr(dy) if form == nat.FOLD_RING else None, producer=fws.data_ptr() + foff,
+                                       inv_table_dev=ptr(finv), m=ptr(y), dz_out=ptr(dz), m_alpha=float(fpm[0]), m_vmax=float(fpm[1]))
+                    check(lib().dlwpcs_conv_small_bwd_data_fold(ctypes.byref(dn), ctypes.byref(sf), ptr(wq), ptr(w_pol), ptr(w_np),
+                                                                ptr(dsrc0), ptr(src0 if pm0 is not None else None), ma, mv,
+                                                                ptr(inv), ptr(ws), ws.numel(), stream_ptr()),
+                          'dlwpcs_conv_small_bwd_data_fold')
+                    del _pending_fold[dy.data_ptr()]
+                    rc = 0
+                elif ctx.small and dsrc0 is not None and dsrc1 is None:
                     rc = lib().dlwpcs_conv_small_bwd_data(*bargs)
                 if rc == nat.E_UNSUPPORTED:
+                    if fold_out is not None and fold_out[0] == nat.FOLD_RING:
+                        fold_out = None
                     rc = lib().dlwpcs_conv_bwd_data_masked(*bargs)
                 check(rc, 'dlwpcs_conv_bwd_data_masked')
                 if ring is not None:
                     _pending_ring[dsrc0.data_ptr()] = (ws, ring[0], ring[1], nat.halo_tables(d.N, 1, dev)[1])
                     dn.flags &= ~nat.CONV_DEFER_RING0
+                if fold_out is not None:
+                    _pending_fold[dsrc0.data_ptr()] = (ws, fold_out[1][0], fold_out[1][1], fold_out[0],
+                                                       inv if fold_out[0] == nat.FOLD_RING else None, pm0)
+                dn.flags &= ~(nat.CONV_DEFER_WINDOW0 | nat.CONV_DEFER_RING0M)
             dw_eq, dw_pol, dw_np, db_eq, db_pol, db_np = _weight_gradients(
                 dn, src0, src1, dz, None, ctx.params, table, ws, nbytes, direct, defer, need[2:8], has_np, has_bias, has_bnp)
-            return (dsrc0, dsrc1, dw_eq, dw_pol, dw_np, db_eq, db_pol, db_np) + (None,) * 15
+            return (dsrc0, dsrc1, dw_eq, dw_pol, dw_np, db_eq, db_pol, db_np) + (None,) * 16
         no_dgrad = dsrc0 is None and dsrc1 is None
         mask_on_load = d.ksize == 3 and (no_dgrad or d.dtype == nat.F32)
         batching = (direct and WGRAD_BATCH and d.B > 0 and not WGRAD_SIDE_STREAM and wgrad_batch_supported(d)
@@ -594,7 +644,7 @@
             batch_mask_ok=mask_on_load)
         if reuse_dz:
             run_bwd_data()
-        return (dsrc0, dsrc1, dw_eq, dw_pol, dw_np, db_eq, db_pol, db_np) + (None,) * 15
+        return (dsrc0, dsrc1, dw_eq, dw_pol, dw_np, db_eq, db_pol, db_np) + (None,) * 16
 
 
 def _small_conv_ok(d):
@@ -653,7 +703,7 @@
 
 def cs_conv(src0, w_eq, w_pol, w_np=None, b_eq=None, b_pol=None, b_np=None, src1=None, ksize=3, halo=True, up0=False,
             flip_north_pole=True, act=nat.ACT_NONE, alpha=0.0, vmax=0.0, premask0=None, premask1=None, dy_premasked=False,
-            defer_ring0=False, want_pool=False, out_padded=False, small=False):
+            defer_ring0=False, want_pool=False, out_padded=False, small=False, fold0=0):
     if (w_np is None) != (b_np is None) and b_eq is not None:
         raise ValueError('cs_conv: north-pole kernel and bias must be given together')
     c0_valid = 0
@@ -669,7 +719,7 @@
             c0_valid = cin_w
     return _CSConv.apply(src0, src1, w_eq, w_pol, w_np, b_eq, b_pol, b_np, int(ksize), bool(halo), bool(up0),
                          bool(flip_north_pole), int(act), float(alpha), float(vmax), int(c0_valid), premask0, premask1,
-                         bool(dy_premasked), bool(defer_ring0), bool(want_pool), bool(out_padded), bool(small))
+                         bool(dy_premasked), bool(defer_ring0), bool(want_pool), bool(out_padded), bool(small), int(fold0))
 
 
 def cs_conv_head_applicable(src0, src1, w_eq, head_w_eq, out_padded):
diff --git a/dlwp-cs_amd/DLWP/options.py b/dlwp-cs_amd/DLWP/options.py
--- a/dlwp-cs_amd/DLWP/options.py
+++ b/dlwp-cs_amd/DLWP/options.py
@@ -3,7 +3,7 @@
 DEFAULTS = {
     'graphs': True, 'premask': True, 'wgrad_batch': True, 'fuse_adam': True, 'fuse_pack': True, 'fuse_head': True,
     'fold_loss_tail': True, 'fuse_pool': True, 'fold_ring': True, 'cf_model': True, 'padded_io': True, 'host_staging': True, 'resident_data': True,
-    'dgrad_gather': True, 'fold_head': True, 'small_conv': True, 'check_finite': False,
+    'dgrad_gather': True, 'fold_head': True, 'small_conv': True, 'small_fold': True, 'small_fold_ring': False, 'check_finite': False,
 }
 
 
diff --git a/dlwp-cs_amd/csrc/conv_mfma.hip b/dlwp-cs_amd/csrc/conv_mfma.hip
--- a/dlwp-cs_amd/csrc/conv_mfma.hip
+++ b/dlwp-cs_amd/csrc/conv_mfma.hip
@@ -1210,7 +1210,8 @@
 static inline int cin_logical(const dlwpcs_conv_desc *d) { return (d->c0_valid > 0 ? d->c0_valid : d->C0) + d->C1; }
 
 bool conv_small_serves(int B, int N, int Cin, int Cout);
-int launch_conv_small(const ConvKParams &K, hipStream_t s);
+int launch_conv_small(const ConvKParams &K, hipStream_t s, const dlwpcs_small_fold *A = nullptr);
+bool conv_small_fold_serves(int form, int N, int C);
 static bool conv_small_layer_ok(const dlwpcs_conv_desc *d) {
     return d->dtype == DLWPCS_BF16 && d->ksize == 3 && d->halo && d->C1 == 0 && !d->up0 && d->c0_valid == 0 &&
            !(d->flags & DLWPCS_CONV_OUT_PADDED) && conv_small_serves(d->B, d->N, d->C0, d->Cout);
@@ -1615,9 +1616,24 @@
                               const void *w_eq, const void *w_pol, const void *w_np,
                               void *dsrc0, void *dsrc1, const void *m0, const void *m1, float m_alpha, float m_vmax,
                               const int32_t *inv_table_dev, void *workspace, size_t workspace_bytes, dlwpcs_stream_t stream,
-                              const char *who, int *ring_query = nullptr, bool small = false) {
+                              const char *who, int *ring_query = nullptr, bool small = false,
+                              const dlwpcs_small_fold *fold = nullptr) {
     int rc = validate(d, who);
     if (rc) return rc;
+    if (fold) {
+        const bool window = fold->form == DLWPCS_FOLD_WINDOW, ring = fold->form == DLWPCS_FOLD_RING;
+        const long pcells = window ? 6l * 4 * d->N * d->N : 6l * (d->N + 2) * (d->N + 2);
+        if (!small || (!window && !ring) || !conv_small_layer_ok(d) || !conv_small_fold_serves(fold->form, d->N, d->Cout) ||
+            fold->channels % 8 || fold->choff % 8 || fold->choff < 0 || fold->choff + d->Cout > fold->channels ||
+            pcells * fold->channels * 2 >= (1l << 31))
+            return fail(DLWPCS_E_UNSUPPORTED, "%s: assembling staging serves the small-face layers in WINDOW or RING form", who);
+        if (!fold->producer || !fold->m || !fold->dz_out || (ring && (!fold->partial || !fold->inv_table_dev)) ||
+            fold->dz_out == fold->partial)
+            return fail(DLWPCS_E_INVALID, "%s: fold description: null pointer, or dz_out is the partial dz", who);
+        if (!(fold->m_alpha >= 0.f) || !(fold->m_vmax >= 0.f))
+            return fail(DLWPCS_E_INVALID, "%s: fold mask needs negative_slope >= 0 and max_value >= 0", who);
+        if (window) dy = fold->dz_out;
+    }
     if (small && (!conv_small_layer_ok(d) || (d->act != DLWPCS_ACT_NONE && !dz_given) || dsrc1 || !dsrc0))
         return fail(DLWPCS_E_UNSUPPORTED, "%s: serves bf16 3x3 halo layers with one source on faces of <= 320 cells, channel counts multiples of 32, gradient given as dz", who);
     const bool prepacked = (d->flags & DLWPCS_CONV_PREPACKED) != 0;
@@ -1709,12 +1725,15 @@
         if (!grc) grc = dispatch_conv(d->dtype, d->ksize, 8, G, conv_work(d), s);
         if (!grc && (g_direct || !need_direct)) {
             if (small) return fail(DLWPCS_E_UNSUPPORTED, "%s: this shape is served in gather form", who);
-            if (ring_query) { *ring_query = 0; return DLWPCS_OK; }
+            const bool window0 = dsrc0 && !G.d0 && !g_usum && d->up0;
+            if (ring_query) { *ring_query = window0 ? 2 : 0; return DLWPCS_OK; }
             G.dry_run = 0;
             grc = dispatch_conv(d->dtype, d->ksize, 8, G, conv_work(d), s);
             if (grc) return grc;
             bool todo0 = m0 != nullptr && !(G.d0 && (g_mask & 1)) && !g_usum, todo1 = m1 != nullptr && !(G.d1 && (g_mask & 2));
-            if (dsrc0 && !G.d0 && !g_usum) {
+            if (window0 && (d->flags & DLWPCS_CONV_DEFER_WINDOW0)) {
+                todo0 = false;
+            } else if (dsrc0 && !G.d0 && !g_usum) {
                 int masked = 0;
                 grc = launch_src_grad(dxv, dsrc0, nullptr, d->B, d->N, Cin, 0, d->C0, d->up0, 0, d->dtype, s, m0, m_alpha, m_vmax, &masked);
                 if (grc) return grc;
@@ -1732,7 +1751,7 @@
     const bool whole = !d->halo && !d->up0 && d->C1 == 0 && dsrc0;
     if (whole) P.out = dsrc0;
     P.dry_run = ring_query ? 1 : 0;
-    rc = small ? launch_conv_small(P, s) : dispatch_conv(d->dtype, d->ksize, vec_width(d->Cout, 0, d->dtype), P, conv_work(d), s);
+    rc = small ? launch_conv_small(P, s, fold) : dispatch_conv(d->dtype, d->ksize, vec_width(d->Cout, 0, d->dtype), P, conv_work(d), s);
     if (ring_query) { *ring_query = (!rc && direct_done && P.d0 && !m0) ? 1 : 0; return rc; }
     if (rc) return rc;
     if (whole) return finish_masks(true, false);
@@ -1747,6 +1766,8 @@
     }
     if (dsrc0) {
         if (direct0 && !m0 && (d->flags & DLWPCS_CONV_DEFER_RING0)) {
+        } else if (direct0 && small && m0 && (mask_done & 1) && (d->flags & DLWPCS_CONV_DEFER_RING0M)) {
+            todo0 = false;
         } else if (direct0) {
             rc = launch_ring_fix(dxv, dsrc0, inv_table_dev, d->B, d->N, Cin, 0, d->C0, d->dtype, s, rm0, m_alpha, m_vmax);
             if (rm0) todo0 = false;
@@ -1804,6 +1825,44 @@
                                           void *workspace, size_t workspace_bytes, dlwpcs_stream_t stream) {
     return conv_bwd_data_impl(d, dz, nullptr, true, w_eq, w_pol, w_np, dsrc0, dsrc1, m0, m1, m_alpha, m_vmax, inv_table_dev, workspace,
                               workspace_bytes, stream, "conv_small_bwd_data", nullptr, true);
+}
+
+extern "C" int dlwpcs_conv_small_bwd_data_fold(const dlwpcs_conv_desc *d, const dlwpcs_small_fold *fold,
+                                               const void *w_eq, const void *w_pol, const void *w_np,
+                                               void *dsrc0, const void *m0, float m0_alpha, float m0_vmax,
+                                               const int32_t *inv_table_dev,
+                                               void *workspace, size_t workspace_bytes, dlwpcs_stream_t stream) {
+    if (!fold) return fail(DLWPCS_E_INVALID, "conv_small_bwd_data_fold: null fold description");
+    return conv_bwd_data_impl(d, fold->partial, nullptr, true, w_eq, w_pol, w_np, dsrc0, nullptr, m0, nullptr, m0_alpha, m0_vmax,
+                              inv_table_dev, workspace, workspace_bytes, stream, "conv_small_bwd_data_fold", nullptr, true, fold);
+}
+
+extern "C" int dlwpcs_conv_fold_info(const dlwpcs_conv_desc *producer, const dlwpcs_conv_desc *consumer, int form, size_t *ws_offset,
+                                     int *channels) {
+    if (validate(producer, "conv_fold_info") != DLWPCS_OK || validate(consumer, "conv_fold_info") != DLWPCS_OK || !ws_offset || !channels)
+        return 0;
+    const dlwpcs_conv_desc *d = producer;
+    if (!d->halo || d->ksize != 3 || d->B < 1 || consumer->B != d->B || consumer->Cout != d->C0) return 0;
+    if (!conv_small_layer_ok(consumer) || !conv_small_fold_serves(form, consumer->N, consumer->Cout)) return 0;
+    const WsLayout L = ws_layout(d);
+    if (form == DLWPCS_FOLD_RING) {
+        if (consumer->N != d->N || !conv_small_layer_ok(d)) return 0;
+    } else if (form == DLWPCS_FOLD_WINDOW) {
+        if (!d->up0 || d->N != 2 * consumer->N || !(d->flags & DLWPCS_CONV_DGRAD_GATHER)) return 0;
+        int q = 0;
+        char dummy = 0;
+        dlwpcs_conv_desc dd = *d;
+        dd.act = DLWPCS_ACT_NONE;
+        dd.flags |= DLWPCS_CONV_PREPACKED;
+        const int rc = conv_bwd_data_impl(&dd, &dummy, nullptr, true, &dummy, nullptr, nullptr, &dummy, d->C1 > 0 ? &dummy : nullptr, &dummy,
+                                          nullptr, 0.f, 0.f, (const int32_t *)&dummy, &dummy, L.total, nullptr, "conv_fold_info", &q);
+        if (rc || q != 2) return 0;
+    } else {
+        return 0;
+    }
+    *ws_offset = L.dxv;
+    *channels = d->C0 + d->C1;
+    return 1;
 }
 
 extern "C" int dlwpcs_conv_ring_info(const dlwpcs_conv_desc *d, size_t *dxv_offset, int *channels) {
@@ -1817,7 +1876,7 @@
     dd.flags |= DLWPCS_CONV_PREPACKED;
     const int rc = conv_bwd_data_impl(&dd, &dummy, nullptr, true, &dummy, nullptr, nullptr, &dummy, d->C1 > 0 ? &dummy : nullptr, nullptr,
                                       nullptr, 0.f, 0.f, (const int32_t *)&dummy, &dummy, L.total, nullptr, "conv_ring_info", &q);
-    if (rc || !q) return 0;
+    if (rc || q != 1) return 0;
     *dxv_offset = L.dxv;
     *channels = d->C0 + d->C1;
     return 1;
diff --git a/dlwp-cs_amd/csrc/conv_small.hip b/dlwp-cs_amd/csrc/conv_small.hip
--- a/dlwp-cs_amd/csrc/conv_small.hip
+++ b/dlwp-cs_amd/csrc/conv_small.hip
@@ -19,13 +19,32 @@
     float m_alpha;
     uint32_t m_thr1;
     int patch_base;
+    const void *a_ws;
+    const int32_t *a_inv;
+    const void *a_m;
+    void *a_out;
+    int a_CT, a_choff;
+    uint32_t magicNs;
+    float a_alpha, a_vmax;
 };
 
 constexpr int SM_THREADS = 256, SM_WAVES = 4;
 constexpr int SM_PROW = 32 * 2 + 16;
 constexpr int SM_U = 16;
-
-template <bool BWD, int MTW>
+constexpr int SM_UW = 5;
+constexpr int SM_UR = 4;
+constexpr int SM_FOLD_WINDOW = 1, SM_FOLD_RING = 2;
+
+__device__ __forceinline__ void sm_unpack(const u32x4 &q, float (&a)[8]) {
+    a[0] = bf_lo(q.x); a[1] = bf_hi(q.x); a[2] = bf_lo(q.y); a[3] = bf_hi(q.y);
+    a[4] = bf_lo(q.z); a[5] = bf_hi(q.z); a[6] = bf_lo(q.w); a[7] = bf_hi(q.w);
+}
+__device__ __forceinline__ float sm_ring_add(float partial, float ring, float g) { return __builtin_fmaf(ring, g, partial); }
+__device__ __forceinline__ uint4 sm_pack(const float (&a)[8]) {
+    return make_uint4(f2bf2(a[0], a[1]), f2bf2(a[2], a[3]), f2bf2(a[4], a[5]), f2bf2(a[6], a[7]));
+}
+
+template <bool BWD, int MTW, int FOLD = 0>
 __global__ void __launch_bounds__(SM_THREADS, 2) conv_small_kernel(const SmallParams P) {
     extern __shared__ __attribute__((aligned(16))) char smem[];
     const int tid = threadIdx.x;
@@ -51,9 +70,89 @@
     uint4 wa[9], wb[9];
     load_w(0, wa);
 
-    {
+    if constexpr (BWD && FOLD == SM_FOLD_WINDOW) {
+        const int Nf = 2 * P.Ns, spix = 6 * P.Ns * P.Ns, fpix = 6 * Nf * Nf;
+        const rsrc_t rf = make_rsrc(reinterpret_cast<const bf16_t *>(P.a_ws) + (size_t)b * fpix * P.a_CT, (uint32_t)(fpix * P.a_CT * 2));
+        const rsrc_t rm = make_rsrc(reinterpret_cast<const bf16_t *>(P.a_m) + (size_t)b * spix * P.Cin, (uint32_t)(spix * P.Cin * 2));
+        const rsrc_t ro = make_rsrc(nt == 0 ? reinterpret_cast<bf16_t *>(P.a_out) + (size_t)b * spix * P.Cin : nullptr, (uint32_t)(spix * P.Cin * 2));
+        const int nv = P.Ns * P.Ns * P.Q;
+#pragma unroll 1
+        for (int e0 = 0; e0 < nv; e0 += SM_THREADS * SM_UW) {
+            u32x4 fv[SM_UW][4], mv[SM_UW];
+#pragma unroll
+            for (int u = 0; u < SM_UW; ++u) {
+                const int e = e0 + tid + u * SM_THREADS;
+                const bool live = e < nv;
+                const int cell = __umulhi((uint32_t)e, P.magicQ), qv = e - cell * P.Q;
+                const int vy = __umulhi((uint32_t)cell, P.magicNs), vx = cell - vy * P.Ns;
+                const int fb = ((f * Nf + 2 * vy) * Nf + 2 * vx) * P.a_CT + P.a_choff + qv * 8;
+                fv[u][0] = __builtin_amdgcn_raw_buffer_load_b128(rf, live ? (uint32_t)fb * 2u : ST_SKIP, 0, 0);
+                fv[u][1] = __builtin_amdgcn_raw_buffer_load_b128(rf, live ? (uint32_t)(fb + P.a_CT) * 2u : ST_SKIP, 0, 0);
+                fv[u][2] = __builtin_amdgcn_raw_buffer_load_b128(rf, live ? (uint32_t)(fb + Nf * P.a_CT) * 2u : ST_SKIP, 0, 0);
+                fv[u][3] = __builtin_amdgcn_raw_buffer_load_b128(rf, live ? (uint32_t)(fb + (Nf + 1) * P.a_CT) * 2u : ST_SKIP, 0, 0);
+                mv[u] = __builtin_amdgcn_raw_buffer_load_b128(rm, live ? (uint32_t)((f * P.Ns * P.Ns + cell) * P.Cin + qv * 8) * 2u : ST_SKIP, 0, 0);
+            }
+            if (e0 == 0) {
+                const uint4 z4 = make_uint4(0u, 0u, 0u, 0u);
+#pragma unroll 1
+                for (int e = tid; e < nitems; e += SM_THREADS) {
+                    const int cell = __umulhi((uint32_t)e, P.magicQ), qv = e - cell * P.Q;
+                    const int ty = __umulhi((uint32_t)cell, P.magicW2), tx = cell - ty * P.W2;
+                    const bool ok = ((uint32_t)(ty - 2) < (uint32_t)P.Ns) & ((uint32_t)(tx - 2) < (uint32_t)P.Ns);
+                    if (!ok) *reinterpret_cast<uint4 *>(smem + cell * RB + qv * 16) = z4;
+                }
+            }
+#pragma unroll
+            for (int u = 0; u < SM_UW; ++u) {
+                const int e = e0 + tid + u * SM_THREADS;
+                const bool live = e < nv;
+                const int cell = __umulhi((uint32_t)e, P.magicQ), qv = e - cell * P.Q;
+                const int vy = __umulhi((uint32_t)cell, P.magicNs), vx = cell - vy * P.Ns;
+                float acc[8], t8[8], y8[8];
+#pragma unroll
+                for (int k = 0; k < 8; ++k) acc[k] = 0.f;
+#pragma unroll
+                for (int j = 0; j < 4; ++j) {
+                    sm_unpack(fv[u][j], t8);
+#pragma unroll
+                    for (int k = 0; k < 8; ++k) acc[k] += t8[k];
+                }
+                sm_unpack(mv[u], y8);
+#pragma unroll
+                for (int k = 0; k < 8; ++k) acc[k] *= act_leaky_clip_grad_from_y(y8[k], P.a_alpha, P.a_vmax);
+                const uint4 o = sm_pack(acc);
+                if (live) *reinterpret_cast<uint4 *>(smem + ((vy + 2) * P.W2 + vx + 2) * RB + qv * 16) = o;
+                bst128(o, ro, live ? (uint32_t)((f * P.Ns * P.Ns + cell) * P.Cin + qv * 8) * 2u : ST_SKIP);
+            }
+        }
+    } else {
         const int spix = 6 * P.Ns * P.Ns;
         const rsrc_t rs = make_rsrc(reinterpret_cast<const bf16_t *>(P.src) + (size_t)b * spix * P.Cin, (uint32_t)(spix * P.Cin * 2));
+        constexpr bool RING = BWD && FOLD == SM_FOLD_RING;
+        const int nbi = RING ? (4 * P.Ns - 4) * P.Q : 0;
+        const rsrc_t ro = make_rsrc(RING && nt == 0 ? reinterpret_cast<bf16_t *>(P.a_out) + (size_t)b * spix * P.Cin : nullptr, (uint32_t)(spix * P.Cin * 2));
+        u32x4 tb[RING ? SM_UR : 1];
+        auto border_item = [&](int u, int &src, int &qv, int &yy, int &xx) __attribute__((always_inline)) {
+            const int k = tid + u * SM_THREADS;
+            const int kc = __umulhi((uint32_t)k, P.magicQ);
+            qv = k - kc * P.Q;
+            const int N = P.Ns;
+            if (kc < N) { yy = 0; xx = kc; }
+            else if (kc < 2 * N) { yy = N - 1; xx = kc - N; }
+            else if (kc < 3 * N - 2) { yy = kc - 2 * N + 1; xx = 0; }
+            else { yy = kc - (3 * N - 2) + 1; xx = N - 1; }
+            src = (f * N + yy) * N + xx;
+            return k < nbi;
+        };
+        if constexpr (RING) {
+            const rsrc_t rt = make_rsrc(P.a_inv, (uint32_t)(spix * 16));
+#pragma unroll
+            for (int u = 0; u < SM_UR; ++u) {
+                int src, qv, yy, xx;
+                const bool live = border_item(u, src, qv, yy, xx);
+                tb[u] = __builtin_amdgcn_raw_buffer_load_b128(rt, live ? (uint32_t)src * 16u : ST_SKIP, 0, 0);
+            }
+        }
 #pragma unroll 1
         for (int e0 = 0; e0 < nitems; e0 += SM_THREADS * SM_U) {
             int sp[SM_U];
@@ -70,6 +169,9 @@
                     const int vy = ty - 2, vx = tx - 2;
                     const bool ok = live & ((uint32_t)vy < (uint32_t)P.Ns) & ((uint32_t)vx < (uint32_t)P.Ns);
                     sp[u] = ok ? (f * P.Ns + vy) * P.Ns + vx : -1;
+                    if constexpr (RING) {
+                        if (ok && (vy == 0 || vy == P.Ns - 1 || vx == 0 || vx == P.Ns - 1)) sp[u] = -2;
+                    }
                 }
             }
             u32x4 val[SM_U];
@@ -84,7 +186,56 @@
             for (int u = 0; u < SM_U; ++u) {
                 const int e = e0 + tid + u * SM_THREADS;
                 const int cell = __umulhi((uint32_t)e, P.magicQ), qv = e - cell * P.Q;
-                if (e < nitems) *reinterpret_cast<uint4 *>(smem + cell * RB + qv * 16) = make_uint4(val[u].x, val[u].y, val[u].z, val[u].w);
+                const uint4 o = make_uint4(val[u].x, val[u].y, val[u].z, val[u].w);
+                if constexpr (RING) {
+                    if (e < nitems && sp[u] != -2) *reinterpret_cast<uint4 *>(smem + cell * RB + qv * 16) = o;
+                    bst128(o, ro, sp[u] >= 0 ? (uint32_t)(sp[u] * P.Cin + qv * 8) * 2u : ST_SKIP);
+                } else {
+                    if (e < nitems) *reinterpret_cast<uint4 *>(smem + cell * RB + qv * 16) = o;
+                }
+            }
+        }
+        if constexpr (RING) {
+            const int M = P.Ns + 2, ppix = 6 * M * M;
+            const rsrc_t rr = make_rsrc(reinterpret_cast<const bf16_t *>(P.a_ws) + (size_t)b * ppix * P.a_CT, (uint32_t)(ppix * P.a_CT * 2));
+            const rsrc_t rm = make_rsrc(reinterpret_cast<const bf16_t *>(P.a_m) + (size_t)b * spix * P.Cin, (uint32_t)(spix * P.Cin * 2));
+            __builtin_amdgcn_sched_barrier(0);
+            u32x4 rv[SM_UR][4], mv[SM_UR], pv[SM_UR];
+#pragma unroll
+            for (int u = 0; u < SM_UR; ++u) {
+                int src, qv, yy, xx;
+                const bool live = border_item(u, src, qv, yy, xx);
+                const int cw = P.a_choff + qv * 8;
+                pv[u] = __builtin_amdgcn_raw_buffer_load_b128(rs, live ? (uint32_t)(src * P.Cin + qv * 8) * 2u : ST_SKIP, 0, 0);
+#pragma unroll
+                for (int j = 0; j < 4; ++j) {
+                    const int tj = (int)tb[u][j];
+                    rv[u][j] = __builtin_amdgcn_raw_buffer_load_b128(rr, (live && tj >= 0) ? (uint32_t)(tj * P.a_CT + cw) * 2u : ST_SKIP, 0, 0);
+                }
+                mv[u] = __builtin_amdgcn_raw_buffer_load_b128(rm, live ? (uint32_t)(src * P.Cin + qv * 8) * 2u : ST_SKIP, 0, 0);
+            }
+#pragma unroll
+            for (int u = 0; u < SM_UR; ++u) {
+                __builtin_amdgcn_sched_barrier(0);
+                int src, qv, yy, xx;
+                const bool live = border_item(u, src, qv, yy, xx);
+                float ring[8], t8[8], y8[8], d8[8];
+#pragma unroll
+                for (int k = 0; k < 8; ++k) ring[k] = 0.f;
+#pragma unroll
+                for (int j = 0; j < 4; ++j) {
+                    const bool on = (int)tb[u][j] >= 0;
+                    sm_unpack(rv[u][j], t8);
+#pragma unroll
+                    for (int k = 0; k < 8; ++k) ring[k] = on ? ring[k] + t8[k] : ring[k];
+                }
+                sm_unpack(mv[u], y8);
+                sm_unpack(pv[u], d8);
+#pragma unroll
+                for (int k = 0; k < 8; ++k) d8[k] = sm_ring_add(d8[k], ring[k], act_leaky_clip_grad_from_y(y8[k], P.a_alpha, P.a_vmax));
+                const uint4 o = sm_pack(d8);
+                if (live) *reinterpret_cast<uint4 *>(smem + ((yy + 2) * P.W2 + xx + 2) * RB + qv * 16) = o;
+                bst128(o, ro, live ? (uint32_t)(src * P.Cin + qv * 8) * 2u : ST_SKIP);
             }
         }
     }
@@ -252,7 +403,7 @@
            (size_t)(N + 4) * (N + 4) * (cmax * 2 + 16) + (size_t)SM_WAVES * 32 * SM_PROW <= 160 * 1024 && (long)B * 6 * (cmax / 32) < (1l << 16);
 }
 
-template <bool BWD>
+template <bool BWD, int FOLD = 0>
 static int launch_small_t(const SmallParams &P, int mtw, size_t lds, unsigned grid, hipStream_t s) {
     auto go = [&](auto kern) -> int {
         if (lds > 64 * 1024) {
@@ -262,13 +413,22 @@
         hipLaunchKernelGGL(kern, dim3(grid), dim3(SM_THREADS), lds, s, P);
         return check_launch("conv_small");
     };
-    if (mtw == 1) return go(conv_small_kernel<BWD, 1>);
-    if (mtw == 2) return go(conv_small_kernel<BWD, 2>);
-    return go(conv_small_kernel<BWD, 3>);
-}
-
-int launch_conv_small(const ConvKParams &K, hipStream_t s) {
+    if (mtw == 1) return go(conv_small_kernel<BWD, 1, FOLD>);
+    if (mtw == 2) return go(conv_small_kernel<BWD, 2, FOLD>);
+    return go(conv_small_kernel<BWD, 3, FOLD>);
+}
+
+bool conv_small_fold_serves(int form, int N, int C) {
+    if (form == DLWPCS_FOLD_WINDOW) return true;
+    return form == DLWPCS_FOLD_RING && (4 * N - 4) * (C / 8) <= SM_THREADS * SM_UR;
+}
+
+int launch_conv_small(const ConvKParams &K, hipStream_t s, const dlwpcs_small_fold *A) {
     const bool bwd = K.mode == MODE_ZERO;
+    if (A && (!bwd || !conv_small_fold_serves(A->form, K.Nin, K.Cin) || A->channels % 8 || A->choff % 8 || A->choff < 0 ||
+              A->choff + K.Cin > A->channels))
+        return fail(DLWPCS_E_UNSUPPORTED, "conv_small: assembling staging serves data gradients, 16-B channel windows and <= %d border vectors per face",
+                    SM_THREADS * SM_UR);
     if (K.mode != MODE_HALO && !bwd) return fail(DLWPCS_E_UNSUPPORTED, "conv_small: serves halo convolutions and their data gradients");
     const int N = K.Nin;
     if (K.C1 != 0 || K.up0 || K.ymask || K.pool_out || K.head_w || K.edge)
@@ -288,6 +448,13 @@
     P.magicNT = P.NT > 1 ? div_magic(P.NT) : 0; P.magicB = P.B > 1 ? div_magic(P.B) : 0;
     P.act = K.act; P.alpha = K.alpha; P.vmax = K.vmax;
     P.m_alpha = K.m_alpha; P.m_thr1 = K.m_thr1;
+    if (A) {
+        P.src = A->partial; P.a_ws = A->producer; P.a_inv = A->inv_table_dev; P.a_m = A->m; P.a_out = A->dz_out;
+        P.a_CT = A->channels; P.a_choff = A->choff; P.magicNs = div_magic(N);
+        P.a_alpha = A->m_alpha; P.a_vmax = mask_vmax_for(DLWPCS_BF16, A->m_vmax);
+        const long cells = A->form == DLWPCS_FOLD_WINDOW ? 6l * 4 * N * N : 6l * (N + 2) * (N + 2);
+        if (cells * A->channels * 2 >= (1l << 31)) return fail(DLWPCS_E_UNSUPPORTED, "conv_small: producer gradient beyond the 32-bit offset range");
+    }
     const size_t in_b = (size_t)P.W2 * P.W2 * (P.Cin * 2 + 16);
     P.patch_base = (int)in_b;
     const size_t lds = in_b + (size_t)SM_WAVES * 32 * SM_PROW;
@@ -300,6 +467,8 @@
     if (K.pool_done) *K.pool_done = 0;
     if (K.head_done) *K.head_done = 0;
     if (K.dry_run || K.B == 0) return DLWPCS_OK;
+    if (A) return A->form == DLWPCS_FOLD_WINDOW ? launch_small_t<true, SM_FOLD_WINDOW>(P, mtw, lds, (unsigned)nwg, s)
+                                                : launch_small_t<true, SM_FOLD_RING>(P, mtw, lds, (unsigned)nwg, s);
     return bwd ? launch_small_t<true>(P, mtw, lds, (unsigned)nwg, s) : launch_small_t<false>(P, mtw, lds, (unsigned)nwg, s);
 }
 
diff --git a/dlwp-cs_amd/csrc/elementwise.hip b/dlwp-cs_amd/csrc/elementwise.hip
--- a/dlwp-cs_amd/csrc/elementwise.hip
+++ b/dlwp-cs_amd/csrc/elementwise.hip
@@ -936,6 +936,17 @@
     }
     return check_launch("mask_inplace");
 }
+}
+
+extern "C" int dlwpcs_src_window(const void *dxv, void *dsrc, int B, int N, int CT, int choff, int CS, int up, int dtype,
+                                 const void *m, float m_alpha, float m_vmax, dlwpcs_stream_t stream) {
+    REQUIRE_DTYPE(dtype, "src_window");
+    REQUIRE(dxv && dsrc, "src_window: null pointer");
+    REQUIRE(B >= 0 && N >= 1 && CS >= 1 && choff >= 0 && choff + CS <= CT && (!up || N % 2 == 0),
+            "src_window: bad shape B=%d N=%d CT=%d choff=%d CS=%d up=%d", B, N, CT, choff, CS, up);
+    REQUIRE(!m || (m_alpha >= 0.f && m_vmax >= 0.f), "src_window: mask activation needs negative_slope >= 0 and max_value >= 0");
+    if (B == 0) return DLWPCS_OK;
+    return dlwpcs::launch_src_grad(dxv, dsrc, nullptr, B, N, CT, choff, CS, up, 0, dtype, (hipStream_t)stream, m, m_alpha, m_vmax, nullptr);
 }
 
 extern "C" int dlwpcs_act_fwd(const void *x, void *y, size_t n, int act, float alpha, float vmax, int dtype,
diff --git a/include/dlwpcs.h b/include/dlwpcs.h
--- a/include/dlwpcs.h
+++ b/include/dlwpcs.h
@@ -44,6 +44,8 @@
 #define DLWPCS_CONV_PREPACKED        2
 #define DLWPCS_CONV_REUSE_DZ         4
 #define DLWPCS_CONV_DEFER_RING0     16
+#define DLWPCS_CONV_DEFER_RING0M   128
+#define DLWPCS_CONV_DEFER_WINDOW0  256
 #define DLWPCS_CONV_DGRAD_GATHER    64
 #define DLWPCS_CONV_OUT_PADDED      32
 #define DLWPCS_CONV_DEFER_REDUCE     8
@@ -117,6 +119,31 @@
                                void *dsrc0, void *dsrc1, const void *m0, const void *m1, float m_alpha, float m_vmax,
                                const int32_t *inv_table_dev,
                                void *workspace, size_t workspace_bytes, dlwpcs_stream_t stream);
+
+#define DLWPCS_FOLD_WINDOW 1
+#define DLWPCS_FOLD_RING   2
+typedef struct dlwpcs_small_fold {
+    int32_t form;
+    int32_t channels;
+    int32_t choff;
+    int32_t reserved;
+    const void *partial;
+    const void *producer;
+    const int32_t *inv_table_dev;
+    const void *m;
+    void *dz_out;
+    float m_alpha, m_vmax;
+} dlwpcs_small_fold;
+int dlwpcs_conv_small_bwd_data_fold(const dlwpcs_conv_desc *d, const dlwpcs_small_fold *fold,
+                                    const void *w_eq, const void *w_pol, const void *w_np,
+                                    void *dsrc0, const void *m0, float m0_alpha, float m0_vmax,
+                                    const int32_t *inv_table_dev,
+                                    void *workspace, size_t workspace_bytes, dlwpcs_stream_t stream);
+int dlwpcs_conv_fold_info(const dlwpcs_conv_desc *producer, const dlwpcs_conv_desc *consumer, int form, size_t *ws_offset,
+                          int *channels);
+
+int dlwpcs_src_window(const void *dxv, void *dsrc, int B, int N, int CT, int choff, int CS, int up, int dtype,
+                      const void *m, float m_alpha, float m_vmax, dlwpcs_stream_t stream);
 
 int dlwpcs_conv_ring_info(const dlwpcs_conv_desc *d, size_t *dxv_offset, int *channels);
 
```

New measurement: 50420 samples/s, median of 6. No clear change (+0.4%).
